# aim-uofa/DiverGen

Hardware: AMD Instinct MI355X
Metric: images/sec (node) Swin-L CenterNet2 LVIS 1024px (higher is better)
Workload: dtype bf16; 1 GPU; CenterNet2 Swin-L-22k-384, 1024x1024, 2 images/GPU, 1453 classes, GPU copy-paste + fwd + bwd + fused clip/AdamW/EMA; configs/DiverGen_swinL.yaml; global_batch=2, parallelism=dp1

## Files before the change

divergen_amd/_lib.py:

```python
import ctypes
import os

import torch

_HERE = os.path.dirname(os.path.abspath(__file__))
LIB_PATH = os.environ.get("DGX_LIB", os.path.join(_HERE, "csrc", "libdgx.so"))
_lib = None

c_p, c_i, c_f, c_i64 = ctypes.c_void_p, ctypes.c_int, ctypes.c_float, ctypes.c_int64


class WgradProblem(ctypes.Structure):
    _fields_ = [("dy", c_p), ("x", c_p), ("gw", c_p), ("M", c_i), ("Nn", c_i), ("Kk", c_i), ("gb", c_p)]


class GemmEpilogue(ctypes.Structure):
    _fields_ = [("mode", c_i), ("c", c_p), ("ldc", c_i64), ("bias", c_p), ("c2", c_p), ("aux", c_p), ("ldaux", c_i64),
                ("residual", c_p), ("out", c_p), ("scale", c_p), ("residual_dtype", c_i),
                ("B", c_i), ("H", c_i), ("W", c_i), ("ws", c_i), ("shift", c_i), ("workspace", c_p), ("workspace_bytes", c_i64), ("relu", c_i)]


class ProfStats(ctypes.Structure):
    _fields_ = [("ms", ctypes.c_double), ("launches", c_i64), ("flops", ctypes.c_double), ("bytes", ctypes.c_double),
                ("captured_launches", c_i64), ("captured_flops", ctypes.c_double), ("captured_bytes", ctypes.c_double)]


class PadItem(ctypes.Structure):
    _fields_ = [("x", c_p), ("xpad", c_p), ("N", c_i), ("H", c_i), ("W", c_i)]


class ConvItem(ctypes.Structure):
    _fields_ = [("xpad", c_p), ("y", c_p), ("N", c_i), ("H", c_i), ("W", c_i)]


class ConvWgradItem(ctypes.Structure):
    _fields_ = [("dypad", c_p), ("xpad", c_p), ("N", c_i), ("H", c_i), ("W", c_i)]


class HeadLevel(ctypes.Structure):
    _fields_ = [("x", c_p), ("dx", c_p), ("scale", c_p), ("rows", c_i)]


class GnItem(ctypes.Structure):
    _fields_ = [("x", c_p), ("dy", c_p), ("out", c_p), ("mean", c_p), ("rstd", c_p), ("scratch", c_p), ("N", c_i), ("HW", c_i)]


class ColsumProblem(ctypes.Structure):
    _fields_ = [("dy", c_p), ("out", c_p), ("M", c_i), ("N", c_i)]


SIGNATURES = {
    "dgx_build_arch": (ctypes.c_char_p, []),
    "dgx_abi_version": (c_i, []),
    "dgx_host_register": (c_i, [c_p, ctypes.c_size_t]),
    "dgx_host_unregister": (c_i, [c_p]),
    "dgx_memcpy_h2d_async": (c_i, [c_p, c_p, ctypes.c_size_t, c_p]),
    "dgx_window_attention_fwd": (c_i, [c_p, c_p, c_i64, c_i64, c_p, c_p, c_p, c_i, c_i, c_i, c_i, c_f, c_p]),
    "dgx_window_attention_bwd": (c_i, [c_p] * 8 + [c_i64, c_i64, c_i, c_i, c_i, c_i, c_f, c_p]),
    "dgx_window_attention_fwd_compact": (c_i, [c_p, c_p, c_p, c_i64, c_i64, c_p, c_p, c_p, c_i, c_i, c_i, c_i, c_i, c_i, c_f, c_p]),
    "dgx_window_attention_bwd_compact": (c_i, [c_p] * 9 + [c_i64, c_i64, c_i, c_i, c_i, c_i, c_i, c_i, c_f, c_p]),
    "dgx_window_gather": (c_i, [c_p, c_p, c_i, c_i, c_i, c_i, c_i, c_i, c_i, c_p]),
    "dgx_window_scatter": (c_i, [c_p, c_p, c_i, c_i, c_i, c_i, c_i, c_i, c_i, c_p]),
    "dgx_roi_align_fwd": (c_i, [c_p, c_p, c_p, c_i, c_i, c_i, c_i, c_i, c_f, c_i, c_i, c_i, c_i, c_i, c_i, c_p]),
    "dgx_roi_align_bwd": (c_i, [c_p, c_p, c_p, c_i, c_i, c_i, c_i, c_i, c_f, c_i, c_i, c_i, c_i, c_i, c_i, c_p]),
    "dgx_roi_pooler_fwd": (c_i, [c_p, c_p, c_p, c_i, c_i, c_p, c_p, c_p, c_i, c_i, c_i, c_i, c_i, c_i, c_i, c_i, c_p]),
    "dgx_roi_pooler_bwd": (c_i, [c_p, c_p, c_p, c_p, c_i, c_i, c_p, c_i, c_i, c_i, c_i, c_i, c_i, c_i, c_i, c_p]),
    "dgx_preprocess_patches": (c_i, [c_p, c_i, c_i, c_p, c_p, c_p, c_i, c_i, c_i, c_p]),
    "dgx_stem_im2col7x7": (c_i, [c_p, c_p, c_i, c_i, c_i, c_p]),
    "dgx_affine_act_fwd": (c_i, [c_p, c_p, c_p, c_p, c_p, c_i64, c_i, c_i, c_p]),
    "dgx_affine_act_bwd": (c_i, [c_p, c_p, c_p, c_p, c_p, c_i64, c_i, c_i, c_p]),
    "dgx_maxpool3x3s2_fwd": (c_i, [c_p, c_p, c_p, c_i, c_i, c_i, c_i, c_p]),
    "dgx_maxpool3x3s2_bwd": (c_i, [c_p, c_p, c_p, c_i, c_i, c_i, c_i, c_p]),
    "dgx_mask_bce_workspace_floats": (c_i64, [c_i64]),
    "dgx_mask_bce": (c_i, [c_p, c_i64, c_i64, c_p, c_i64, c_p, c_p, c_p, c_i, c_p]),
    "dgx_prof_enable": (c_i, [c_i]),
    "dgx_prof_pause": (c_i, [c_i]),
    "dgx_prof_read": (c_i, [c_i, c_p]),
    "dgx_roi_pooler_bwd_gather": (c_i, [c_p, c_p, c_p, c_p, c_i, c_i, c_f, c_i, c_p, c_i, c_i, c_i, c_i, c_i, c_i, c_i, c_p]),
    "dgx_roi_pooler_bwd_gather_accum": (c_i, [c_p, c_p, c_p, c_p, c_i, c_i, c_f, c_i, c_p, c_i, c_i, c_i, c_i, c_i, c_i, c_i, c_f, c_i, c_p]),
    "dgx_mask_crop": (c_i, [c_p, c_p, c_p, c_p, c_i, c_i, c_i, c_i, c_i, c_p]),
    "dgx_nms_sorted": (c_i, [c_p, c_i, c_f, c_p, c_p, c_p, c_p]),
    "dgx_nms_workspace_words": (c_i64, [c_i]),
    "dgx_nms_batched_workspace_words": (c_i64, [c_i, c_i]),
    "dgx_nms_batched": (c_i, [c_p, c_p, c_p, c_i, c_i, c_f, c_i, c_p, c_p, c_i, c_p, c_p]),
    "dgx_iou_match": (c_i, [c_p, c_i, c_p, c_i, c_f, c_p, c_p, c_p, c_p]),
    "dgx_centernet_targets": (c_i, [c_p, c_p, c_i, c_p, c_p, c_p, c_i, c_f, c_f, c_p, c_p, c_p]),
    "dgx_centernet_scores": (c_i, [c_p, c_i, c_i, c_p, c_p, c_i, c_i, c_f, c_p, c_p, c_i, c_p]),
    "dgx_centernet_decode": (c_i, [c_p, c_i, c_i, c_p, c_p, c_i, c_i, c_p, c_i, c_p, c_f, c_p, c_p, c_p, c_i, c_p]),
    "dgx_centernet_head_outputs": (c_i, [c_p, c_i, c_i, c_p, c_p, c_p]),
    "dgx_centernet_head_outputs_bwd_workspace_floats": (c_i64, [c_p, c_i, c_i]),
    "dgx_centernet_head_outputs_bwd": (c_i, [c_p, c_i, c_i, c_p, c_p, c_p, c_p, c_p]),
    "dgx_set_reserved_cus": (None, [c_i]),
    "dgx_get_reserved_cus": (c_i, []),
    "dgx_dev_set": (c_i, [ctypes.c_char_p, c_i]),
    "dgx_gemm_last_form": (c_i, [ctypes.POINTER(c_i)] * 3),
    "dgx_dev_gemm_log": (c_i, [ctypes.c_char_p]),
    "dgx_gather_boxes": (c_i, [c_p, c_p, c_i, c_i, c_p, c_p]),
    "dgx_topk_index_rows": (c_i, [c_p, c_i64, c_i, c_p, c_p, c_p, c_i, c_i, c_p, c_i64, c_p]),
    "dgx_sort_rows_desc": (c_i, [c_p, c_i, c_i, c_p, c_p, c_p]),
    "dgx_centernet_finalize": (c_i, [c_p, c_p, c_p, c_p, c_i, c_i, c_i, c_p, c_p, c_p, c_p]),
    "dgx_roi_label": (c_i, [c_p, c_p, c_i, c_i, c_p, c_p, c_p, c_i, c_f, c_i, c_i, c_i, c_p, c_p, c_p, c_p, c_p, c_p]),
    "dgx_roi_gather": (c_i, [c_i, c_i, c_i, c_p, c_p, c_p, c_p, c_p, c_p, c_p, c_p, c_p, c_f] + [c_p] * 10 + [c_p]),
    "dgx_centernet_label_inds": (c_i, [c_p, c_p, c_i, c_i, c_p, c_p, c_p, c_i, c_p, c_p, c_p]),
    "dgx_copy_paste": (c_i, [c_p, c_p, c_p, c_i, c_i, c_i, c_p, c_p, c_i, c_p, c_p, c_p, c_p, c_p]),
    "dgx_copy_paste_blend": (c_i, [c_p, c_p, c_p, c_i, c_i, c_i, c_p, c_p, c_i, c_p, c_p, c_p, c_p, c_p, c_p]),
    "dgx_copy_paste_blend_ws": (c_i, [c_p, c_p, c_p, c_i, c_i, c_i, c_p, c_p, c_i, c_p, c_p, c_p, c_p, c_p, c_p, ctypes.c_size_t, c_p]),
    "dgx_poisson_blend": (c_i, [c_p, c_p, c_p, c_i, c_i, c_p, ctypes.c_size_t, c_i, c_p]),
    "dgx_poisson_work_bytes": (c_i64, [c_i, c_i, c_i64]),
    "dgx_poisson_frame_unknowns": (c_i64, [c_i, c_i]),
    "dgx_poisson_max_iter": (c_i, [c_i, c_i, c_i64]),
    "dgx_self_copy_paste": (c_i, [c_p, c_p, c_p, c_i, c_i, c_i, c_p, c_p, c_i, c_i, c_i, c_p, c_i, c_i, c_i, c_p, c_p, c_p, c_p, c_p, c_p]),
    "dgx_self_copy_paste_merged": (c_i, [c_p, c_p, c_p, c_i, c_i, c_i, c_p, c_p, c_i, c_i, c_i, c_p, c_i, c_i, c_i, c_p, c_p, c_p, c_p, c_p, c_p]),
    "dgx_self_copy_paste_all": (c_i, [c_p, c_p, c_p, c_i, c_i, c_i, c_p, c_p, c_i, c_i, c_i, c_i, c_i, c_p, c_p, c_p, c_p, c_p, c_p]),
# ... 146 lines not shown
```

divergen_amd/csrc/abi.hip:

```cpp
#include "dgx_common.h"
extern "C" const char* dgx_build_arch(void) { return "gfx950"; }
extern "C" int dgx_abi_version(void) { return 3; }

extern "C" int dgx_host_register(void* p, size_t bytes) {
    if (!p || !bytes) return DGX_ERR_BAD_ARG;
    const hipError_t e = hipHostRegister(p, bytes, hipHostRegisterDefault);
    return e == hipSuccess ? DGX_OK : -(int)e - 1000;
}
extern "C" int dgx_host_unregister(void* p) {
    if (!p) return DGX_ERR_BAD_ARG;
    const hipError_t e = hipHostUnregister(p);
    return e == hipSuccess ? DGX_OK : -(int)e - 1000;
}
extern "C" int dgx_memcpy_h2d_async(void* dst, const void* src, size_t bytes, void* stream) {
    if (!bytes) return DGX_OK;
    if (!dst || !src) return DGX_ERR_BAD_ARG;
    const hipError_t e = hipMemcpyAsync(dst, src, bytes, hipMemcpyHostToDevice, (hipStream_t)stream);
    return e == hipSuccess ? DGX_OK : -(int)e - 1000;
}
```

divergen_amd/csrc/gemm_common.h:

```cpp
#pragma once
#include "dgx_common.h"
#include "gemm_plan.h"
#include "winmap.h"
#include <type_traits>

constexpr int GBK = 64;
static constexpr uint32_t G_OOB = 0x80000000u;

namespace dgxgemm {
struct GMap { int B, H, W, ws, shift, nWh, nWw, compact; };

struct GemmP {
    const uint16_t* A;
    const uint16_t* B;
    int M, N, K, lda, ldb;
    int tiles_n, total, per_xcd;
    int splits, kt_per_split;
    float* ws;
    int mode;
    uint16_t* C;
    int ldc;
    const uint16_t* bias;
    uint16_t* C2;
    const uint16_t* aux;
    int ldaux;
    const void* res;
    void* out;
    const float* scale;
    int res_dtype;
    GMap map;
    int conv_kc, conv_wp;
    int cmap_n, cmap_h, cmap_w;
    int relu;
    int ngrp;
    struct Grp { const uint16_t* A; uint16_t* C; int M, cn, ch, cw, wp, tile0; } grp[6];
};
constexpr int GEMM_MAXG = 6;
}
using dgxgemm::GMap;
using dgxgemm::GemmP;

namespace {

__device__ __forceinline__ void g_load_lds16(uint32_t voff, u32x4 rsrc, uint32_t lds_addr, uint32_t soff) {
    asm volatile("s_mov_b32 m0, %2\n\ts_nop 0\n\tbuffer_load_dwordx4 %0, %1, %3 offen lds" ::"v"(voff), "s"(rsrc), "s"(lds_addr), "s"(soff)
                 : "memory");
}
__device__ __forceinline__ u32x4 g_rsrc(const void* base, uint32_t bytes) {
    const uint64_t a = (uint64_t)base;
    return u32x4{(uint32_t)a, (uint32_t)(a >> 32) & 0xffffu, bytes, 0x00020000u};
}
template <int N> __device__ __forceinline__ void g_vmcnt() { asm volatile("s_waitcnt vmcnt(%0)" ::"n"(N) : "memory"); }
__device__ __forceinline__ void g_lgkm0() { asm volatile("s_waitcnt lgkmcnt(0)" ::: "memory"); }
__device__ __forceinline__ void g_bar() {
    asm volatile("s_barrier" ::: "memory");
    __builtin_amdgcn_sched_barrier(0);
}

template <int MC> __device__ __forceinline__ void g_fix_mode(GemmP& P) {
    if constexpr (MC == 6) { P.mode = 3; P.res_dtype = DGX_F32; }
    else if constexpr (MC == 3) { P.mode = 3; P.res_dtype = DGX_BF16; }
    else if constexpr (MC >= 0) P.mode = MC;
}
template <class F> int g_with_mc(int mc, F&& f) {
    switch (mc) {
        case 1: return f(std::integral_constant<int, 1>{});
        case 2: return f(std::integral_constant<int, 2>{});
        case 3: return f(std::integral_constant<int, 3>{});
        case 4: return f(std::integral_constant<int, 4>{});
        case 5: return f(std::integral_constant<int, 5>{});
        case 6: return f(std::integral_constant<int, 6>{});
        default: return f(std::integral_constant<int, 0>{});
    }
}
inline int g_tail_mc(const GemmP& P) { return dgxplan::tail_mc(P.mode, P.res_dtype == DGX_BF16); }

__device__ __forceinline__ dgxgemm::GemmP::Grp g_group_of_tile(const GemmP& P, int L) {
    dgxgemm::GemmP::Grp q = P.grp[0];
#pragma unroll
    for (int k = 1; k < dgxgemm::GEMM_MAXG; ++k)
        if (k < P.ngrp && L >= P.grp[k].tile0) q = P.grp[k];
    return q;
}
__device__ __forceinline__ void g_enter_group(GemmP& P, const dgxgemm::GemmP::Grp& q) {
    P.A = q.A; P.C = q.C; P.M = q.M;
    P.cmap_n = q.cn; P.cmap_h = q.ch; P.cmap_w = q.cw; P.conv_wp = q.wp;
}
__device__ __forceinline__ uint32_t g_a_voff(const GemmP& P, int m, int lc) {
    int64_t arow = m;
    if (P.conv_kc) {
        const int hw = P.cmap_h * P.cmap_w;
        const int n = m / hw, r = m - n * hw;
        const int y = r / P.cmap_w, x = r - y * P.cmap_w;
        arow = ((int64_t)n * (P.cmap_h + 2) + y + 1) * P.conv_wp + x + 1;
    }
    return m < P.M ? (uint32_t)((arow * P.lda + lc * 8) * 2) : G_OOB;
}
__device__ __forceinline__ uint32_t g_a_soff(const GemmP& P, int kta) {
    uint32_t s = (uint32_t)kta * (GBK * 2);
    if (P.conv_kc) {
        const int tap = kta / P.conv_kc, kc = kta - tap * P.conv_kc;
        s = (uint32_t)((tap / 3) * P.conv_wp + tap % 3) * (uint32_t)(P.lda * 2) + (uint32_t)kc * (GBK * 2);
    }
    return s;
}
__device__ __forceinline__ void g_bias4(const u32x2 raw, float (&bv)[4]) {
    bv[0] = __uint_as_float(raw[0] << 16); bv[1] = __uint_as_float(raw[0] & 0xffff0000u);
    bv[2] = __uint_as_float(raw[1] << 16); bv[3] = __uint_as_float(raw[1] & 0xffff0000u);
}

constexpr float kGInvSqrt2 = 0.70710678118654752440f;
constexpr float kGInvSqrt2Pi = 0.39894228040143267794f;
__device__ __forceinline__ void g_unpack8(const u32x4 r, float (&v)[8]) {
#pragma unroll
    for (int i = 0; i < 4; ++i) { v[2 * i] = __uint_as_float(r[i] << 16); v[2 * i + 1] = __uint_as_float(r[i] & 0xffff0000u); }
}
__device__ __forceinline__ u32x4 g_pack8(const float (&v)[8]) {
    return u32x4{pack_bf2(v[0], v[1]), pack_bf2(v[2], v[3]), pack_bf2(v[4], v[5]), pack_bf2(v[6], v[7])};
}

__device__ __forceinline__ int64_t g_row_token(const GMap& m, int64_t orow, int& b) {
    if (m.ws == 0) {
        b = (int)(orow / ((int64_t)m.H * m.W));
        return orow;
    }
    if (m.compact) return wm_token_of_row(wm_geom(m.H, m.W, m.ws, m.shift), (int)orow, b);
    const int Nw = m.ws * m.ws;
    const int n = (int)(orow % Nw);
    int64_t t = orow / Nw;
    const int wc = (int)(t % m.nWw);
    t /= m.nWw;
    const int wr = (int)(t % m.nWh);
    b = (int)(t / m.nWh);
    int hh = wr * m.ws + n / m.ws + m.shift, ww = wc * m.ws + n % m.ws + m.shift;
    const int Hp = m.nWh * m.ws, Wp = m.nWw * m.ws;
    if (hh >= Hp) hh -= Hp;
    if (ww >= Wp) ww -= Wp;
    return (hh < m.H && ww < m.W) ? ((int64_t)b * m.H + hh) * m.W + ww : -1;
}
// ... 139 lines not shown
```

divergen_amd/csrc/gemm_lw.hip:

```cpp
#include "gemm_common.h"
#include "dev_clock.h"
#include <stdio.h>
#include <stdlib.h>
#include <string.h>

namespace {
constexpr int LW_LDS = 160 * 1024;
template <int BM, int BN, int NSA_, int NSB_> struct LwCfg {
    static constexpr int NSA = NSA_, NSB = NSB_;
    static_assert(NSA >= NSB && NSA - NSB <= 1 && NSB >= 2, "ring depths: NSA == NSB or NSB + 1");
    static constexpr int WMF = BM / 32;
    static constexpr int WNF = BN / 64;
    static constexpr int NLA = BM / 32;
    static constexpr int NLB = BN / 32;
    static constexpr int SA = BM * 128;
    static constexpr int SBb = BN * 128;
    static constexpr int B0 = (NSA - 1) * SA;
    static constexpr int STG0 = B0 + NSB * SBb;
    static constexpr int RING = STG0 + SA;
    static_assert(RING <= LW_LDS, "rings do not fit");
    static constexpr int SROW = BN * 2 + 16;
    static constexpr int TOK0 = LW_LDS - BM * 8;
    static constexpr int STGB = TOK0 - STG0;
    static constexpr int HALF = BM / 2;
    static constexpr int pick_hc() {
        for (int hc = HALF; hc >= 16; hc -= 16)
            if (HALF % hc == 0 && 2 * hc * SROW <= STGB) return hc;
        return 0;
    }
    static constexpr int HC = pick_hc();
    static_assert(HC >= 16, "staging area too small");
    static constexpr int CH = 2 * HC;
    static constexpr int NPASS = HALF / HC;
    static constexpr int FPP = HC / 16;
};
constexpr int LW_THREADS = 768, LW_MFMA_THREADS = 512;

__device__ __forceinline__ void lw_lgkm0() { __builtin_amdgcn_s_waitcnt(0xc07f); }
__device__ __forceinline__ uint32_t lw_sgpr(uint32_t v) { return (uint32_t)__builtin_amdgcn_readfirstlane((int)v); }
template <int PRO, int STEADY, int STEP>
__device__ __forceinline__ void lw_vmcnt_le(int n) {
    if (PRO > STEADY && n >= PRO) g_vmcnt<PRO>();
    else if (STEADY > 0 && n >= STEADY) g_vmcnt<STEADY>();
    else if (STEP > 0 && STEP < STEADY && n >= STEP) g_vmcnt<STEP>();
    else g_vmcnt<0>();
}
struct LwItem { int m0, n0, kt0, NT, split; };
}

template <int BM, int BN, int NSA, int NSB, int MC>
__global__ __launch_bounds__(LW_THREADS) void gemm_lw_kernel(GemmP P0) {
    constexpr int EC = MC == 6 ? 2 : (MC == 3 || MC == 4 || MC == 5) ? 1 : 0;
    if constexpr (MC == 0) { if (P0.mode > 1) __builtin_unreachable(); }
    else g_fix_mode<MC>(P0);
    using Cfg = LwCfg<BM, BN, NSA, NSB>;
    constexpr int WMF = Cfg::WMF, WNF = Cfg::WNF, NLA = Cfg::NLA, NLB = Cfg::NLB, SA = Cfg::SA, SBb = Cfg::SBb, B0 = Cfg::B0;
    constexpr int SROW = Cfg::SROW, STG0 = Cfg::STG0, CH = Cfg::CH, HC = Cfg::HC, NPASS = Cfg::NPASS, FPP = Cfg::FPP, HALF = Cfg::HALF;
    extern __shared__ __attribute__((aligned(1024))) unsigned char lds_raw[];
    const int nwx = (int)(gridDim.x >> 3);
    const int xcd = blockIdx.x & 7;
    const int items = P0.total * P0.splits;
    const int bound = min((xcd + 1) * P0.per_xcd, items);
    const int first = xcd * P0.per_xcd + (int)(blockIdx.x >> 3);
    if (first >= bound) return;
    const int tid = threadIdx.x, l = tid & 63;
    const int w = __builtin_amdgcn_readfirstlane(tid >> 6);
    const int grp = (w >> 2) & 1, wc = w & 3;
    const int c = l & 15, g = l >> 4;
    const int NTK = (P0.K + GBK - 1) / GBK;
    const int ktail = P0.K - (NTK - 1) * GBK;
    const uint32_t lds0 = (uint32_t)(uintptr_t)(DGX_LDS unsigned char*)lds_raw;

    auto locate_item = [&](int L0, GemmP& P, LwItem& it) {
        int L = L0 / P0.splits;
        it.split = L0 - L * P0.splits;
        if (P0.ngrp > 0) {
            L = __builtin_amdgcn_readfirstlane(L);
            const dgxgemm::GemmP::Grp q = g_group_of_tile(P0, L);
            g_enter_group(P, q);
            L -= q.tile0;
        }
        const int tm = L / P0.tiles_n, tn = L - tm * P0.tiles_n;
        it.m0 = tm * BM;
        it.n0 = tn * BN;
        it.kt0 = it.split * P0.kt_per_split;
        it.NT = min(P0.kt_per_split, NTK - it.kt0);
    };
    auto a_slot = [](int s) -> uint32_t { return s == NSA - 1 ? (uint32_t)STG0 : (uint32_t)s * SA; };

    if (w >= 8) {
        const int lw = w - 8;
        const int rsub = l >> 3;
        const int lc = (l & 7) ^ (((lw & 1) << 2) | (rsub >> 1));
        const bool kt_ok = lc * 8 < ktail;
        const uint32_t ldsq = lw_sgpr(lds0 + 1024u * lw);
        GemmP P = P0;
        LwItem it;
        uint32_t voffA[NLA], voffB[NLB];
        u32x4 rA;
        const u32x4 rB = g_rsrc(P0.B, (uint32_t)((int64_t)P0.N * P0.ldb * 2));
        auto setup = [&](int L0) {
            locate_item(L0, P, it);
#pragma unroll
            for (int s = 0; s < NLA; ++s) voffA[s] = g_a_voff(P, it.m0 + 8 * (lw + 4 * s) + rsub, lc);
#pragma unroll
            for (int s = 0; s < NLB; ++s) {
                const int n = it.n0 + 8 * (lw + 4 * s) + rsub;
                voffB[s] = n < P.N ? (uint32_t)(((int64_t)n * P.ldb + lc * 8) * 2) : G_OOB;
            }
            const u32x4 r = g_rsrc(P.A, (uint32_t)((P.conv_kc ? (int64_t)P.cmap_n * (P.cmap_h + 2) * P.conv_wp + 2 * P.conv_wp + 2 : (int64_t)P.M) * P.lda * 2));
            rA = u32x4{lw_sgpr(r[0]), lw_sgpr(r[1]), lw_sgpr(r[2]), lw_sgpr(r[3])};
        };
        auto issue_a = [&](int t) {
            if (t >= it.NT) return;
            const int kta = it.kt0 + t;
            const uint32_t soffA = g_a_soff(P, kta);
            const bool tail = (kta == NTK - 1) && (ktail != GBK) && !kt_ok;
            const uint32_t dst = ldsq + a_slot(t % NSA);
#pragma unroll
            for (int s = 0; s < NLA; ++s) g_load_lds16(tail ? G_OOB : voffA[s], rA, lw_sgpr(dst + 4096u * s), lw_sgpr(soffA));
        };
        auto issue_b = [&](int t) {
            if (t >= it.NT) return;
            const int kta = it.kt0 + t;
            const uint32_t soff = (uint32_t)kta * (GBK * 2);
            const bool tail = (kta == NTK - 1) && (ktail != GBK) && !kt_ok;
            const uint32_t dst = ldsq + B0 + (uint32_t)(t % NSB) * SBb;
#pragma unroll
            for (int s = 0; s < NLB; ++s) g_load_lds16(tail ? G_OOB : voffB[s], rB, lw_sgpr(dst + 4096u * s), lw_sgpr(soff));
        };
        constexpr int STEADY = (NSA > NSB ? NSB - 1 : NSA - 2) * NLA + (NSB - 2) * NLB;
        constexpr int PRO = (NSA - 1) * NLA + (NSB - 1) * NLB;
        static_assert(PRO < 64, "vmcnt is a 6-bit counter");
        auto wait_tile = [&](int tau, int ia, int ib) {
            const int la = min(ia, it.NT - 1), lb = min(ib, it.NT - 1);
            const int ca = max(0, la - (tau + 1) + 1), cb = max(0, lb - (tau + 1) + 1);
            lw_vmcnt_le<PRO, STEADY, NLA>(ca * NLA + cb * NLB);
        };
        auto prologue_1 = [&]() {
// ... 290 lines not shown
```

divergen_amd/csrc/gemm_nt.hip:

```cpp
#include "gemm_common.h"
#include "dev_clock.h"
#include <stdio.h>
#include <string.h>

namespace {
template <int BM, int BN, int NS_> struct GemmCfg {
    static constexpr int NS = NS_;
    static constexpr int WMF = BM / 32;
    static constexpr int WNF = BN / 64;
    static constexpr int NA = BM / 64;
    static constexpr int NB = BN / 64;
    static constexpr int SB = (BM + BN) * 128;
    static constexpr int SROW = BN * 2 + 16;
    static constexpr int EPI = BM * SROW + BM * 8;
    static constexpr int LDS = (NS * SB > EPI ? NS * SB : EPI);
};
}

template <int BM, int BN, int NS, int MINW, int MC = -1>
__global__ __launch_bounds__(512, MINW) void gemm_nt_kernel(GemmP P) {
    g_fix_mode<MC>(P);
    using Cfg = GemmCfg<BM, BN, NS>;
    constexpr int NL = Cfg::NA + Cfg::NB;
    constexpr int WMF = Cfg::WMF, WNF = Cfg::WNF, NA = Cfg::NA, NB = Cfg::NB, SB = Cfg::SB, SROW = Cfg::SROW;
    extern __shared__ __attribute__((aligned(1024))) unsigned char lds_raw[];
    const int L0 = (blockIdx.x & 7) * P.per_xcd + (blockIdx.x >> 3);
    if (L0 >= P.total * P.splits) return;
    int L = L0 / P.splits;
    const int split = L0 - L * P.splits;
    if (P.ngrp > 0) {
        L = __builtin_amdgcn_readfirstlane(L);
        dgxgemm::GemmP::Grp q = P.grp[0];
#pragma unroll
        for (int k = 1; k < dgxgemm::GEMM_MAXG; ++k)
            if (k < P.ngrp && L >= P.grp[k].tile0) q = P.grp[k];
        P.A = q.A; P.C = q.C; P.M = q.M;
        P.cmap_n = q.cn; P.cmap_h = q.ch; P.cmap_w = q.cw; P.conv_wp = q.wp;
        L -= q.tile0;
    }
    DGX_CLK(0);
    DGX_CLK_RT(5);
    const int tm = L / P.tiles_n, tn = L - tm * P.tiles_n;
    const int m0 = tm * BM, n0 = tn * BN;
    const int tid = threadIdx.x, l = tid & 63;
    const int w = __builtin_amdgcn_readfirstlane(tid >> 6);
    const int grp = w >> 2, wc = w & 3;
    const int c = l & 15, g = l >> 4;
    const int NTK = (P.K + GBK - 1) / GBK;
    const int ktail = P.K - (NTK - 1) * GBK;
    const int kt0 = split * P.kt_per_split;
    const int NT = min(P.kt_per_split, NTK - kt0);

    const int rsub = l >> 3;
    const int lc = (l & 7) ^ (((w & 1) << 2) | (rsub >> 1));
    uint32_t voffA[NA], voffB[NB];
#pragma unroll
    for (int s = 0; s < NA; ++s) voffA[s] = g_a_voff(P, m0 + 8 * (w + 8 * s) + rsub, lc);
#pragma unroll
    for (int s = 0; s < NB; ++s) {
        const int n = n0 + 8 * (w + 8 * s) + rsub;
        voffB[s] = n < P.N ? (uint32_t)(((int64_t)n * P.ldb + lc * 8) * 2) : G_OOB;
    }
    const bool kt_ok = lc * 8 < ktail;
    const u32x4 rA = g_rsrc(P.A, (uint32_t)((P.conv_kc ? (int64_t)P.cmap_n * (P.cmap_h + 2) * P.conv_wp + 2 * P.conv_wp + 2 : (int64_t)P.M) * P.lda * 2));
    const u32x4 rB = g_rsrc(P.B, (uint32_t)((int64_t)P.N * P.ldb * 2));
    const uint32_t lds0 = (uint32_t)(uintptr_t)(DGX_LDS unsigned char*)lds_raw;
    const uint32_t ldsw = __builtin_amdgcn_readfirstlane(lds0 + 1024u * w);
    auto issue_one = [&](int k, int t, int stage) {
        const int kta = kt0 + t;
        const uint32_t soff = (uint32_t)kta * (GBK * 2), soffA = g_a_soff(P, kta);
        const uint32_t dst = ldsw + (uint32_t)stage * SB;
        const bool tail = (kta == NTK - 1) && (ktail != GBK) && !kt_ok;
        if (k < NA) g_load_lds16(tail ? G_OOB : voffA[k], rA, dst + 8192u * k, soffA);
        else g_load_lds16(tail ? G_OOB : voffB[k - NA], rB, dst + BM * 128 + 8192u * (k - NA), soff);
    };

    const int swz = (c >> 1) & 7;
    const uint32_t la = (uint32_t)((grp * (BM / 2) + c) * 128 + ((g ^ swz) << 4));
    const uint32_t lb = (uint32_t)((BM + wc * (BN / 4) + c) * 128 + ((g ^ swz) << 4));
    f32x4 acc[WMF][WNF];
#pragma unroll
    for (int i = 0; i < WMF; ++i)
#pragma unroll
        for (int j = 0; j < WNF; ++j) acc[i][j] = f32x4{0.f, 0.f, 0.f, 0.f};
    bf16x8 af[WMF][2], bfr[WNF][2];
    auto load_phase = [&](int stage, int ti, int istage) {
        if (ti >= 0) {
#pragma unroll
            for (int k = 0; k < NL; ++k) issue_one(k, ti, istage);
        }
        DGX_LDS const unsigned char* sa = lds_opaque((const unsigned char*)lds_raw + stage * SB + la);
        DGX_LDS const unsigned char* sa1 = lds_opaque((const unsigned char*)lds_raw + stage * SB + (la ^ 64u));
        DGX_LDS const unsigned char* sb = lds_opaque((const unsigned char*)lds_raw + stage * SB + lb);
        DGX_LDS const unsigned char* sb1 = lds_opaque((const unsigned char*)lds_raw + stage * SB + (lb ^ 64u));
#pragma unroll
        for (int j = 0; j < WNF; ++j) {
            bfr[j][0] = *reinterpret_cast<DGX_LDS const bf16x8*>(sb + 2048 * j);
            bfr[j][1] = *reinterpret_cast<DGX_LDS const bf16x8*>(sb1 + 2048 * j);
        }
#pragma unroll
        for (int i = 0; i < WMF; ++i) {
            af[i][0] = *reinterpret_cast<DGX_LDS const bf16x8*>(sa + 2048 * i);
            af[i][1] = *reinterpret_cast<DGX_LDS const bf16x8*>(sa1 + 2048 * i);
        }
// ... 247 lines not shown
    if (bm == 192 && bn == 192 && ns == 3) return nt_launch_e<192, 192, 3, 2, -1>(P, st);
    if (bm == 128 && bn == 192 && ns == 4) return nt_launch_e<128, 192, 4, 2, -1>(P, st);
    if (bm == 192 && bn == 256 && ns == 2) return nt_launch_e<192, 256, 2, 2, -1>(P, st);
    if (bm == 128 && bn == 256 && ns == 3) return nt_launch_e<128, 256, 3, 2, -1>(P, st);
    if (bm == 256 && bn == 128 && ns == 3) return nt_launch_e<256, 128, 3, 2, -1>(P, st);
    if (bm == 128 && bn == 128 && ns == 4) return nt_launch_e<128, 128, 4, 2, -1>(P, st);
    return DGX_ERR_UNSUPPORTED;
}
}

int gemm_lw_launch(GemmP& P, int bm, int bn, hipStream_t st);
bool dgx_gemm_k192_takes(const GemmP& P);
int dgx_gemm_k192_launch(const GemmP& P, hipStream_t st);

static GemmPlan plan_and_log(const GemmP& P, int64_t ws_bytes) {
    dgxplan::GemmProblem q;
    q.M = P.M; q.N = P.N; q.K = P.K;
    q.mode = P.mode; q.res_bf16 = P.res_dtype == DGX_BF16;
    q.conv = P.conv_kc != 0; q.relu = P.relu != 0;
    q.ngrp = P.ngrp;
    int rows = P.ngrp ? 0 : P.M;
    for (int i = 0; i < P.ngrp; ++i) { q.Ms[i] = P.grp[i].M; rows += P.grp[i].M; }
    q.ws_bytes = P.ws ? ws_bytes : 0;
    q.k192_operands = dgx_gemm_k192_takes(P);
    const GemmPlan pl = dgxplan::plan_gemm(q, g_dev, dgx_get_reserved_cus() / 8);
    if (g_gemm_log) { fprintf(g_gemm_log, "%d %d %d %d %d %d\n", rows, P.N, P.K, P.conv_kc ? 9 : P.mode, pl.bm, pl.bn); fflush(g_gemm_log); }
    return pl;
}
static int launch(GemmP& P, const GemmPlan& pl, hipStream_t st) {
    P.tiles_n = pl.tiles_n; P.total = pl.total; P.per_xcd = pl.per_xcd;
    P.splits = pl.splits; P.kt_per_split = pl.kt_per_split;
    for (int i = 0; i < P.ngrp; ++i) P.grp[i].tile0 = pl.tile0[i];
    const bool k192 = pl.form == dgxplan::FORM_K192;
    const int rc = k192 ? dgx_gemm_k192_launch(P, st) : pl.form == dgxplan::FORM_LW ? gemm_lw_launch(P, pl.bm, pl.bn, st) : gemm_nt_launch(P, pl, st);
    if (rc != DGX_OK) return rc;
    if (k192) g_last = {pl.form, 32, 192, 1};
    else g_last = {pl.form, pl.bm, pl.bn, pl.splits};
    if (!k192 && pl.splits > 1) {
        const int64_t chunks = (int64_t)P.M * (P.N >> 3);
        const int grid = (int)((chunks + 255) / 256 < 4096 ? (chunks + 255) / 256 : 4096);
        hipLaunchKernelGGL(gemm_splitk_fold_kernel, dim3(grid), dim3(256), 0, st, P);
    }
    DGX_LAUNCH_CHECK();
    return DGX_OK;
}

DGX_CLK_READER(dgx_dev_gemm_nt_clocks)
extern "C" int dgx_dev_gemm_log(const char* path) {
    if (g_gemm_log) { fclose(g_gemm_log); g_gemm_log = nullptr; }
    if (path && *path && !(g_gemm_log = fopen(path, "w"))) return DGX_ERR_BAD_ARG;
    return DGX_OK;
}
extern int g_dgx_dev_wgrad_lw;
extern "C" int dgx_dev_set(const char* key, int value) {
    if (!key) return DGX_ERR_BAD_ARG;
    if (!strcmp(key, "gemm_lw")) g_dev.lw = value;
    else if (!strcmp(key, "gemm_2wg")) g_dev.two_wg = value;
    else if (!strcmp(key, "gemm_tile")) { g_dev.tile_bm = value / 1000; g_dev.tile_bn = value % 1000; }
    else if (!strcmp(key, "gemm_splitk")) g_dev.splitk = value;
    else if (!strcmp(key, "gemm_k192")) g_dev.k192 = value;
    else if (!strcmp(key, "wgrad_lw")) g_dgx_dev_wgrad_lw = value;
    else if (!strcmp(key, "reset")) { g_dev = dgxplan::DevKnobs(); g_dgx_dev_wgrad_lw = 1; }
    else return DGX_ERR_BAD_ARG;
    return DGX_OK;
}
extern "C" int dgx_gemm_last_form(int* bm, int* bn, int* splits) {
    if (bm) *bm = g_last.bm;
    if (bn) *bn = g_last.bn;
    if (splits) *splits = g_last.splits;
    return g_last.form;
}

extern "C" int dgx_gemm_bf16_nt(const void* A, const void* B, int M, int N, int K, int64_t lda, int64_t ldb,
                                const dgx_gemm_epilogue* ep, void* stream) {
    if (M <= 0 || N <= 0) return DGX_OK;
    if (!A || !B || !ep || K <= 0 || (K & 7) || (N & 7) || (lda & 7) || (ldb & 7) || lda < K || ldb < K) return DGX_ERR_BAD_ARG;
    if ((int64_t)M * lda * 2 >= (1ll << 31) || (int64_t)N * ldb * 2 >= (1ll << 31)) return DGX_ERR_UNSUPPORTED;
    GemmP P;
    memset((void*)&P, 0, sizeof(P));
    P.A = (const uint16_t*)A; P.B = (const uint16_t*)B;
    P.M = M; P.N = N; P.K = K; P.lda = (int)lda; P.ldb = (int)ldb;
    P.mode = ep->mode;
    P.C = (uint16_t*)ep->c; P.ldc = (int)ep->ldc;
    P.bias = (const uint16_t*)ep->bias;
    P.C2 = (uint16_t*)ep->c2;
    P.aux = (const uint16_t*)ep->aux; P.ldaux = (int)ep->ldaux;
    P.res = ep->residual; P.out = ep->out; P.scale = ep->scale; P.res_dtype = ep->residual_dtype;
    P.ws = (float*)ep->workspace;
    P.relu = (ep->mode <= DGX_EPI_BIAS) ? ep->relu : 0;
    switch (ep->mode) {
        case DGX_EPI_NONE: case DGX_EPI_BIAS:
            if (!ep->c || ep->ldc < N || (ep->ldc & 7)) return DGX_ERR_BAD_ARG;
            if (ep->mode == DGX_EPI_NONE) P.bias = nullptr;
            break;
        case DGX_EPI_BIAS_GELU:
            if (!ep->c || !ep->c2 || ep->ldc < N || (ep->ldc & 7)) return DGX_ERR_BAD_ARG;
            break;
        case DGX_EPI_GELU_GRAD: case DGX_EPI_RELU_GRAD:
            if (!ep->c || !ep->aux || ep->ldc < N || ep->ldaux < N || (ep->ldc & 7) || (ep->ldaux & 7)) return DGX_ERR_BAD_ARG;
            P.bias = nullptr;
            break;
        case DGX_EPI_BIAS_RESIDUAL: {
            const int aws = ep->ws < 0 ? -ep->ws : ep->ws;
            if (!ep->residual || !ep->out || ep->B <= 0 || ep->H <= 0 || ep->W <= 0 || ep->B > 4095 || ep->shift < 0 ||
                (aws > 0 && ep->shift >= aws) || (ep->residual_dtype != DGX_F32 && ep->residual_dtype != DGX_BF16) ||
                (ep->ws < 0 && !wm_compact_ok(ep->H, ep->W, aws, ep->shift)))
                return DGX_ERR_BAD_ARG;
            GMap m = {ep->B, ep->H, ep->W, aws, ep->shift, 0, 0, ep->ws < 0 ? 1 : 0};
            if (aws > 0) { m.nWh = (ep->H + aws - 1) / aws; m.nWw = (ep->W + aws - 1) / aws; }
            const int64_t rows = ep->ws > 0 ? (int64_t)ep->B * m.nWh * m.nWw * aws * aws : (int64_t)ep->B * ep->H * ep->W;
            if (rows != M) return DGX_ERR_BAD_ARG;
            P.map = m;
            break;
        }
        default: return DGX_ERR_BAD_ARG;
    }
    const double mn = (double)M * N, rsz = ep->residual_dtype == DGX_F32 ? 4.0 : 2.0;
    const double obytes = ep->mode == DGX_EPI_BIAS_RESIDUAL ? 2.0 * rsz * mn : (ep->mode >= DGX_EPI_BIAS_GELU ? 4.0 * mn : 2.0 * mn);
    DgxProfScope prof(DGX_PROF_GEMM_NT, stream, 2.0 * mn * K, 2.0 * ((double)M * K + (double)N * K) + obytes);
    return launch(P, plan_and_log(P, ep->workspace_bytes), (hipStream_t)stream);
}

extern "C" int64_t dgx_conv3x3_pad_rows(int N, int H, int W) {
    return (N <= 0 || H <= 0 || W <= 0) ? 0 : (int64_t)N * (H + 2) * (W + 2) + 2 * (int64_t)(W + 3);
}

extern "C" int dgx_conv3x3_gemm_multi(const dgx_conv_item* items, int n, const void* w, const void* bias, int Cin, int Cout, int relu,
                                      void* stream) {
    if (n <= 0) return DGX_OK;
    if (!items || !w || Cin <= 0 || Cout <= 0 || (Cin & 63) || (Cout & 7)) return DGX_ERR_BAD_ARG;
    if (n > dgxgemm::GEMM_MAXG || Cout > 256 || (int64_t)Cout * 9 * Cin * 2 >= (1ll << 31)) return DGX_ERR_UNSUPPORTED;
    GemmP P;
    memset((void*)&P, 0, sizeof(P));
    P.B = (const uint16_t*)w;
    P.N = Cout; P.K = 9 * Cin; P.lda = Cin; P.ldb = 9 * Cin;
    P.mode = bias ? DGX_EPI_BIAS : DGX_EPI_NONE;
    P.ldc = Cout;
    P.bias = (const uint16_t*)bias;
    P.conv_kc = Cin / GBK;
    P.relu = relu;
    P.ngrp = n;
    double fl = 0.0, by = 2.0 * 9.0 * Cin * Cout;
// ... 59 lines not shown
```

divergen_amd/csrc/wgrad256.hip:

```cpp
#include "dgx_common.h"
#include <type_traits>

namespace {
constexpr int T256 = 256;
constexpr int BM256 = 32;
constexpr int NB256 = 4;
constexpr int OPB256 = BM256 * T256 * 2;
constexpr int STB256 = 2 * OPB256;
constexpr int MAXP256 = 12;

struct Prob256 {
    const uint16_t* A;
    const uint16_t* B;
    float* C;
    float* gb;
    float* wsb;
    float* ws;
    int M, Nn, Kk, tiles_k, tiles, S, slab, wg0;
    int ldc;
    int64_t red0;
};
struct Params256 {
    Prob256 p[MAXP256];
    int n, total, per_xcd;
    int interleave;
    float beta;
    int nimg;
    struct Img { const uint16_t* dy; const uint16_t* x; int wp, M, slab0; } img[6];
};

__device__ __forceinline__ void buffer_load_lds16(uint32_t voff, u32x4 rsrc, uint32_t lds_wave_base, uint32_t soff) {
    asm volatile("s_mov_b32 m0, %2\n\ts_nop 0\n\tbuffer_load_dwordx4 %0, %1, %3 offen lds" ::"v"(voff), "s"(rsrc), "s"(lds_wave_base), "s"(soff)
                 : "memory");
}
__device__ __forceinline__ u32x4 make_rsrc(const void* base, uint32_t bytes) {
    const uint64_t a = (uint64_t)base;
    return u32x4{(uint32_t)a, (uint32_t)(a >> 32) & 0xffffu, bytes, 0x00020000u};
}
__device__ __forceinline__ void mfma16_agpr(f32x4& c, bf16x8 a, bf16x8 b) {
    asm("v_mfma_f32_16x16x32_bf16 %0, %1, %2, %0" : "+a"(c) : "v"(a), "v"(b));
}
__device__ __forceinline__ void mfma16_vgpr(f32x4& c, bf16x8 a, bf16x8 b) {
    asm("v_mfma_f32_16x16x32_bf16 %0, %1, %2, %0" : "+v"(c) : "v"(a), "v"(b));
}
template <int N> __device__ __forceinline__ void wait_vmcnt() { asm volatile("s_waitcnt vmcnt(%0)" ::"n"(N) : "memory"); }
}

__global__ __launch_bounds__(256) void wgrad256_partial_kernel(Params256 P) {
    extern __shared__ __attribute__((aligned(1024))) unsigned char lds_raw[];
    const int L = (blockIdx.x & 7) * P.per_xcd + (blockIdx.x >> 3);
    if (L >= P.total) return;
    int pi = 0;
    if (P.interleave) {
        pi = L % P.n;
    } else {
#pragma unroll
        for (int i = 1; i < MAXP256; ++i)
            if (i < P.n && L >= P.p[i].wg0) pi = i;
    }
    Prob256 q = P.p[pi];
    const int local = P.interleave ? L / P.n : L - q.wg0;
    const int s = local / q.tiles, tile = local - s * q.tiles;
    int s_in = s;
    if (P.nimg > 0) {
        const int su = __builtin_amdgcn_readfirstlane(s), tap = __builtin_amdgcn_readfirstlane(pi);
        Params256::Img im = P.img[0];
#pragma unroll
        for (int k = 1; k < 6; ++k)
            if (k < P.nimg && su >= P.img[k].slab0) im = P.img[k];
        q.A = im.dy + (int64_t)(im.wp + 1) * q.Nn;
        q.B = im.x + (int64_t)((tap / 3) * im.wp + tap % 3) * q.Kk;
        q.M = im.M;
        s_in = su - im.slab0;
    }
    const int n0 = (tile / q.tiles_k) * T256, k0 = (tile % q.tiles_k) * T256;
    const int m_begin = s_in * q.slab, m_end = min(q.M, m_begin + q.slab);
    const int nst = (m_end - m_begin + BM256 - 1) / BM256;
    const int tid = threadIdx.x, w = tid >> 6, l = tid & 63, g = l >> 4, c16 = l & 15;
    const int wn = (w >> 1) * 128, wk = (w & 1) * 128;

    const int rip = l >> 5;
    const int lc = (l & 31) ^ (((2 * (w & 1) + rip) & 3) << 1);
    const uint32_t OOB = 0x80000000u;
    const uint32_t vA = (n0 + 8 * lc < q.Nn) ? (uint32_t)(((2 * w + rip) * q.Nn + n0 + 8 * lc) * 2) : OOB;
    const uint32_t vB = (k0 + 8 * lc < q.Kk) ? (uint32_t)(((2 * w + rip) * q.Kk + k0 + 8 * lc) * 2) : OOB;
    const u32x4 rA = make_rsrc(q.A, (uint32_t)((int64_t)m_end * q.Nn * 2));
    const u32x4 rB = make_rsrc(q.B, (uint32_t)((int64_t)m_end * q.Kk * 2));
    const uint32_t lds0 = (uint32_t)(uintptr_t)(DGX_LDS unsigned char*)lds_raw;
    const uint32_t ldsw = __builtin_amdgcn_readfirstlane(lds0 + 1024u * w);
    auto issue1 = [&](int st, int h) {
        const uint32_t row0 = (uint32_t)(m_begin + st * BM256);
        const uint32_t dst = ldsw + (uint32_t)(st & (NB256 - 1)) * STB256;
        const int j = h & 3;
        if (h < 4) buffer_load_lds16(vA, rA, dst + 4096u * j, (row0 + 8 * j) * (uint32_t)(q.Nn * 2));
        else buffer_load_lds16(vB, rB, dst + OPB256 + 4096u * j, (row0 + 8 * j) * (uint32_t)(q.Kk * 2));
    };
    auto issue = [&](int st) {
#pragma unroll
        for (int h = 0; h < 8; ++h) issue1(st, h);
    };

    const int x = c16 >> 2, hi = (c16 >> 1) & 1, lo = c16 & 1;
    DGX_LDS const uint16_t* pfa[2][4];
    DGX_LDS const uint16_t* pfb[2][4];
#pragma unroll
    for (int b = 0; b < 4; ++b) {
        const uint32_t o = (uint32_t)((8 * g + x) * 512 + 32 * (b ^ x) + 16 * hi + 8 * lo);
#pragma unroll
        for (int h2 = 0; h2 < 2; ++h2) {
            pfa[h2][b] = lds_opaque(reinterpret_cast<const uint16_t*>(lds_raw + o + wn * 2 + h2 * 2 * STB256));
            pfb[h2][b] = lds_opaque(reinterpret_cast<const uint16_t*>(lds_raw + OPB256 + o + wk * 2 + h2 * 2 * STB256));
        }
    }

    f32x4 acc[8][8];
#pragma unroll
    for (int i = 0; i < 8; ++i)
#pragma unroll
        for (int j = 0; j < 8; ++j) acc[i][j] = f32x4{0.f, 0.f, 0.f, 0.f};
    const bool do_bias = q.gb != nullptr && (tile % q.tiles_k) == 0;
    f32x4 bacc[4];
#pragma unroll
    for (int i = 0; i < 4; ++i) bacc[i] = f32x4{0.f, 0.f, 0.f, 0.f};
    bf16x8 ones = {(short)0x3F80, (short)0x3F80, (short)0x3F80, (short)0x3F80, (short)0x3F80, (short)0x3F80, (short)0x3F80, (short)0x3F80};
    asm volatile("" : "+v"(ones));
    auto bias_mfmas = [&](const bf16x8 (&af)[8]) {
        if (do_bias) {
            if (w & 1) {
#pragma unroll
// ... 166 lines not shown
    int tiles[MAXP256], maxM = 0;
    for (int i = 0; i < n; ++i) {
        tiles[i] = ((pr[i].Nn + T256 - 1) / T256) * ((pr[i].Kk + T256 - 1) / T256);
        if (pr[i].M > maxM) maxM = pr[i].M;
    }
    int R = BM256;
    for (;; R += BM256) {
        int64_t wgs = 0;
        for (int i = 0; i < n; ++i) wgs += (int64_t)tiles[i] * ((pr[i].M + R - 1) / R);
        if (wgs <= 256 || R >= maxM) break;
    }
    for (int i = 0; i < n; ++i) {
        S[i] = (pr[i].M + R - 1) / R;
        if (S[i] < 1) S[i] = 1;
        int sl = (pr[i].M + S[i] - 1) / S[i];
        slab[i] = (sl + BM256 - 1) / BM256 * BM256;
    }
}

static int64_t ws_floats256(const dgx_wgrad_problem* pr, int n, const int* S, int64_t* off, int64_t* offb = nullptr) {
    int64_t tot = 0;
    for (int i = 0; i < n; ++i) {
        if (off) off[i] = tot;
        if (S[i] > 1) tot += (int64_t)S[i] * pr[i].Nn * pr[i].Kk;
    }
    for (int i = 0; i < n; ++i) {
        if (offb) offb[i] = tot;
        if (S[i] > 1 && pr[i].gb) tot += ((int64_t)S[i] * pr[i].Nn + 3) / 4 * 4;
    }
    return tot;
}

bool wgrad_lw_wants(const dgx_wgrad_problem* pr, int n);
int wgrad_lw_launch(const dgx_wgrad_problem* pr, int n, float beta, hipStream_t st);
constexpr int MAXP_GROUP = 32;

extern "C" int dgx_wgrad_grouped_form(const dgx_wgrad_problem* problems, int n) {
    return problems && n > 0 && n <= MAXP_GROUP && wgrad_lw_wants(problems, n) ? 1 : 0;
}

static int64_t split_workspace_bytes(const dgx_wgrad_problem* problems, int n) {
    if (!problems || n <= 0 || n > MAXP256) return 0;
    int S[MAXP256], slab[MAXP256];
    plan256(problems, n, S, slab);
    return ws_floats256(problems, n, S, nullptr) * 4;
}
extern "C" int64_t dgx_wgrad_grouped_workspace_bytes(const dgx_wgrad_problem* problems, int n) {
    if (!problems || n <= 0 || n > MAXP_GROUP) return 0;
    if (wgrad_lw_wants(problems, n) && n > MAXP256) return 0;
    return split_workspace_bytes(problems, n);
}

static int wgrad_grouped_impl(const dgx_wgrad_problem* problems, const int* ldc, int n, float beta, void* workspace, void* stream);

extern "C" int dgx_linear_wgrad_grouped(const dgx_wgrad_problem* problems, int n, float beta, void* workspace,
                                        void* stream) {
    double fl = 0.0, by = 0.0;
    if (!problems || n <= 0 || n > MAXP_GROUP) return DGX_ERR_BAD_ARG;
    for (int i = 0; i < n; ++i) {
        fl += 2.0 * problems[i].M * problems[i].Nn * problems[i].Kk;
        by += 2.0 * problems[i].M * ((double)problems[i].Nn + problems[i].Kk) + 8.0 * problems[i].Nn * problems[i].Kk;
    }
    DgxProfScope prof(DGX_PROF_WGRAD, stream, fl, by);
    if (wgrad_lw_wants(problems, n)) {
        const int rc = wgrad_lw_launch(problems, n, beta, (hipStream_t)stream);
        if (rc == DGX_OK) { DGX_LAUNCH_CHECK(); return DGX_OK; }
        if (rc != DGX_ERR_UNSUPPORTED || n > MAXP256) return rc;
    }
    return wgrad_grouped_impl(problems, nullptr, n, beta, workspace, stream);
}

extern "C" int64_t dgx_conv3x3_wgrad_workspace_bytes(int N, int H, int W, int Cin, int Cout) {
    dgx_wgrad_problem pr[9];
    const int64_t Mp = (int64_t)N * (H + 2) * (W + 2);
    for (int t = 0; t < 9; ++t) { pr[t].dy = pr[t].x = nullptr; pr[t].gw = nullptr; pr[t].gb = nullptr; pr[t].M = (int)Mp; pr[t].Nn = Cout; pr[t].Kk = Cin; }
    return split_workspace_bytes(pr, 9);
}
extern "C" int dgx_conv3x3_wgrad_bias(const void* dypad, const void* xpad, float* gw, float* gb, int N, int H, int W, int Cin, int Cout,
                                      float beta, void* workspace, void* stream);
extern "C" int dgx_conv3x3_wgrad(const void* dypad, const void* xpad, float* gw, int N, int H, int W, int Cin, int Cout, float beta,
                                 void* workspace, void* stream) {
    return dgx_conv3x3_wgrad_bias(dypad, xpad, gw, nullptr, N, H, W, Cin, Cout, beta, workspace, stream);
}
extern "C" int64_t dgx_conv3x3_wgrad_bias_workspace_bytes(int N, int H, int W, int Cin, int Cout) {
    dgx_wgrad_problem pr[9];
    const int64_t Mp = (int64_t)N * (H + 2) * (W + 2);
    float dummy;
    for (int t = 0; t < 9; ++t) { pr[t].dy = pr[t].x = nullptr; pr[t].gw = nullptr; pr[t].gb = t == 0 ? &dummy : nullptr; pr[t].M = (int)Mp; pr[t].Nn = Cout; pr[t].Kk = Cin; }
    return split_workspace_bytes(pr, 9);
}
extern "C" int dgx_conv3x3_wgrad_bias(const void* dypad, const void* xpad, float* gw, float* gb, int N, int H, int W, int Cin, int Cout,
                                      float beta, void* workspace, void* stream) {
    if (N <= 0 || H <= 0 || W <= 0) return DGX_OK;
    if (!dypad || !xpad || !gw || (Cin & 7) || (Cout & 7)) return DGX_ERR_BAD_ARG;
    const int64_t Mp = (int64_t)N * (H + 2) * (W + 2);
    const int wp = W + 2;
    dgx_wgrad_problem pr[9];
    int ldc[9];
    for (int t = 0; t < 9; ++t) {
        pr[t].dy = (const uint16_t*)dypad + (int64_t)(wp + 1) * Cout;
        pr[t].x = (const uint16_t*)xpad + (int64_t)((t / 3) * wp + t % 3) * Cin;
        pr[t].gw = gw + (int64_t)t * Cin;
        pr[t].gb = t == 0 ? gb : nullptr;
        pr[t].M = (int)Mp; pr[t].Nn = Cout; pr[t].Kk = Cin;
        ldc[t] = 9 * Cin;
    }
    DgxProfScope prof(DGX_PROF_WGRAD, stream, 2.0 * N * H * W * 9.0 * Cin * Cout, 2.0 * Mp * ((double)Cin + Cout) + 8.0 * 9.0 * Cin * Cout);
    return wgrad_grouped_impl(pr, ldc, 9, beta, workspace, stream);
}

static int wgrad_grouped_impl(const dgx_wgrad_problem* problems, const int* ldc, int n, float beta, void* workspace, void* stream) {
    if (n <= 0) return DGX_OK;
    if (!problems || n > MAXP256) return DGX_ERR_BAD_ARG;
    for (int i = 0; i < n; ++i) {
        const dgx_wgrad_problem& p = problems[i];
        if (!p.dy || !p.x || !p.gw || p.M <= 0 || p.Nn <= 0 || p.Kk <= 0 || (p.Nn & 7) || (p.Kk & 7)) return DGX_ERR_BAD_ARG;
        if ((int64_t)p.M * p.Nn * 2 >= (1ll << 31) || (int64_t)p.M * p.Kk * 2 >= (1ll << 31)) return DGX_ERR_UNSUPPORTED;
    }
    int S[MAXP256], slab[MAXP256];
    int64_t off[MAXP256], offb[MAXP256];
    plan256(problems, n, S, slab);
    if (ws_floats256(problems, n, S, off, offb) > 0 && !workspace) return DGX_ERR_BAD_ARG;
    Params256 P;
    P.n = n;
    P.beta = beta;
    P.nimg = 0;
    int wg = 0;
    int64_t red = 0;
    for (int i = 0; i < n; ++i) {
        const dgx_wgrad_problem& p = problems[i];
        Prob256& q = P.p[i];
        q.A = (const uint16_t*)p.dy;
        q.B = (const uint16_t*)p.x;
        q.C = p.gw;
        q.gb = p.gb;
        q.wsb = (float*)workspace + offb[i];
        q.ws = (float*)workspace + off[i];
        q.M = p.M; q.Nn = p.Nn; q.Kk = p.Kk;
        q.ldc = ldc ? ldc[i] : p.Kk;
        q.tiles_k = (p.Kk + T256 - 1) / T256;
        q.S = S[i];
        q.slab = slab[i];
        q.tiles = ((p.Nn + T256 - 1) / T256) * q.tiles_k;
        q.wg0 = wg;
        q.red0 = red;
        wg += q.tiles * S[i];
        if (S[i] > 1) red += (int64_t)p.Nn * p.Kk / 4;
    }
    for (int i = n; i < MAXP256; ++i) P.p[i] = P.p[0];
    hipStream_t st = (hipStream_t)stream;
    const size_t sm = (size_t)NB256 * STB256;
    static bool once = false;
    if (!once) {
        (void)hipFuncSetAttribute((const void*)wgrad256_partial_kernel, hipFuncAttributeMaxDynamicSharedMemorySize, (int)sm);
        once = true;
    }
    P.total = wg;
    P.interleave = 0;
    if (ldc && n > 1) {
        P.interleave = 1;
        for (int i = 1; i < n; ++i)
            if (P.p[i].tiles != P.p[0].tiles || P.p[i].S != P.p[0].S || P.p[i].M != P.p[0].M) P.interleave = 0;
    }
    P.per_xcd = (wg + 7) / 8;
    hipLaunchKernelGGL(wgrad256_partial_kernel, dim3(8 * P.per_xcd), dim3(256), sm, st, P);
    int bias_cb = 1, bias_blocks = 0;
    {
        int maxNn = 0;
        for (int i = 0; i < n; ++i)
            if (S[i] > 1 && problems[i].gb) maxNn = problems[i].Nn > maxNn ? problems[i].Nn : maxNn;
        if (maxNn > 0) { bias_cb = (maxNn + 255) / 256; bias_blocks = bias_cb * n; }
    }
    if (red > 0 || bias_blocks > 0) {
        int maxS = 1;
        for (int i = 0; i < n; ++i) maxS = S[i] > maxS ? S[i] : maxS;
        if (red > 0 && red <= 32768 && maxS >= 16) {
            hipLaunchKernelGGL(wgrad256_reduce_kernel<16>, dim3((int)((red * 16 + 255) / 256) + bias_blocks), dim3(256), 0, st, P, red,
                               bias_blocks, bias_cb);
        } else {
            const int grid = (int)((red + 255) / 256 < 8192 ? (red + 255) / 256 : 8192);
            hipLaunchKernelGGL(wgrad256_reduce_kernel<1>, dim3(grid + bias_blocks), dim3(256), 0, st, P, red, bias_blocks, bias_cb);
        }
    }
    DGX_LAUNCH_CHECK();
    return DGX_OK;
}

static int conv_multi_plan(const dgx_conv_wgrad_item* items, int n, int tiles, int* R_out, int* nsl, int* M) {
    int maxM = 0;
    for (int i = 0; i < n; ++i) {
        M[i] = items[i].N * (items[i].H + 2) * (items[i].W + 2);
// ... 12 lines not shown
}

extern "C" int64_t dgx_conv3x3_wgrad_bias_multi_workspace_bytes(const dgx_conv_wgrad_item* items, int n, int Cin, int Cout) {
    if (!items || n <= 0 || n > 6) return 0;
    if (n == 1) return dgx_conv3x3_wgrad_bias_workspace_bytes(items[0].N, items[0].H, items[0].W, Cin, Cout);
    int R, nsl[6], M[6];
    const int tiles = ((Cout + T256 - 1) / T256) * ((Cin + T256 - 1) / T256);
    const int S = conv_multi_plan(items, n, tiles, &R, nsl, M);
    return ((int64_t)9 * S * Cout * Cin + ((int64_t)S * Cout + 3) / 4 * 4) * 4;
}

extern "C" int dgx_conv3x3_wgrad_bias_multi(const dgx_conv_wgrad_item* items, int n, float* gw, float* gb, int Cin, int Cout, float beta,
                                            void* workspace, void* stream) {
    if (n <= 0) return DGX_OK;
    if (!items || !gw || !workspace || (Cin & 7) || (Cout & 7) || Cin <= 0 || Cout <= 0) return DGX_ERR_BAD_ARG;
    if (n > 6) return DGX_ERR_UNSUPPORTED;
    if (n == 1)
        return dgx_conv3x3_wgrad_bias(items[0].dypad, items[0].xpad, gw, gb, items[0].N, items[0].H, items[0].W, Cin, Cout, beta, workspace,
                                      stream);
    int R, nsl[6], M[6];
    const int tiles_k = (Cin + T256 - 1) / T256, tiles = ((Cout + T256 - 1) / T256) * tiles_k;
    for (int i = 0; i < n; ++i) {
        if (!items[i].dypad || !items[i].xpad || items[i].N <= 0 || items[i].H <= 0 || items[i].W <= 0) return DGX_ERR_BAD_ARG;
        const int64_t rows = (int64_t)items[i].N * (items[i].H + 2) * (items[i].W + 2) + 2 * (int64_t)(items[i].W + 3);
        if (rows * Cout * 2 >= (1ll << 31) || rows * Cin * 2 >= (1ll << 31)) return DGX_ERR_UNSUPPORTED;
    }
    const int S = conv_multi_plan(items, n, tiles, &R, nsl, M);
    Params256 P;
    P.n = 9;
    P.beta = beta;
    P.nimg = n;
    int s0 = 0;
    double fl = 0.0, by = 8.0 * 9.0 * Cin * Cout;
    for (int i = 0; i < n; ++i) {
        P.img[i].dy = (const uint16_t*)items[i].dypad; P.img[i].x = (const uint16_t*)items[i].xpad;
        P.img[i].wp = items[i].W + 2; P.img[i].M = M[i]; P.img[i].slab0 = s0;
        s0 += nsl[i];
        fl += 2.0 * items[i].N * items[i].H * items[i].W * 9.0 * Cin * Cout;
        by += 2.0 * M[i] * ((double)Cin + Cout);
    }
    for (int i = n; i < 6; ++i) P.img[i] = P.img[0];
    float* ws = (float*)workspace;
    const int64_t per = (int64_t)S * Cout * Cin;
    int wg = 0;
    int64_t red = 0;
    for (int t = 0; t < 9; ++t) {
        Prob256& q = P.p[t];
        q.A = P.img[0].dy; q.B = P.img[0].x;
        q.C = gw + (int64_t)t * Cin;
        q.gb = t == 0 ? gb : nullptr;
        q.wsb = ws + 9 * per;
        q.ws = ws + (int64_t)t * per;
        q.M = M[0]; q.Nn = Cout; q.Kk = Cin;
        q.ldc = 9 * Cin;
        q.tiles_k = tiles_k;
        q.S = S;
        q.slab = R;
        q.tiles = tiles;
        q.wg0 = wg;
        q.red0 = red;
        wg += tiles * S;
        red += (int64_t)Cout * Cin / 4;
    }
    for (int i = 9; i < MAXP256; ++i) P.p[i] = P.p[0];
    hipStream_t st = (hipStream_t)stream;
    const size_t sm = (size_t)NB256 * STB256;
    static bool once = false;
    if (!once) {
        (void)hipFuncSetAttribute((const void*)wgrad256_partial_kernel, hipFuncAttributeMaxDynamicSharedMemorySize, (int)sm);
        once = true;
    }
    P.total = wg;
    P.interleave = 1;
    P.per_xcd = (wg + 7) / 8;
    DgxProfScope prof(DGX_PROF_WGRAD, stream, fl, by);
    hipLaunchKernelGGL(wgrad256_partial_kernel, dim3(8 * P.per_xcd), dim3(256), sm, st, P);
    const int bias_cb = (Cout + 255) / 256, bias_blocks = gb ? bias_cb * 9 : 0;
    if (red <= 32768 && S >= 16) {
        hipLaunchKernelGGL(wgrad256_reduce_kernel<16>, dim3((int)((red * 16 + 255) / 256) + bias_blocks), dim3(256), 0, st, P, red, bias_blocks,
                           bias_cb);
    } else {
        const int grid = (int)((red + 255) / 256 < 8192 ? (red + 255) / 256 : 8192);
        hipLaunchKernelGGL(wgrad256_reduce_kernel<1>, dim3(grid + bias_blocks), dim3(256), 0, st, P, red, bias_blocks, bias_cb);
    }
    DGX_LAUNCH_CHECK();
    return DGX_OK;
}
```

divergen_amd/csrc/wgrad_lw.hip:

```cpp
#include "dgx_common.h"
#include <stdlib.h>
#include <string.h>
#include <type_traits>

namespace {
constexpr int WL_TN = 256, WL_TK = 192;
constexpr int WL_BM = 64;
constexpr int WL_GR = 32;
constexpr int WL_GB = WL_GR * 512;
constexpr int WL_NGA = 6, WL_NGB = 4;
constexpr int WL_B0 = WL_NGA * WL_GB;
constexpr int WL_LDS = (WL_NGA + WL_NGB) * WL_GB;
constexpr int WL_MAXP = 32;
constexpr int WL_THREADS = 768;

struct WlProb {
    const uint16_t* A;
    const uint16_t* B;
    float* C;
    float* gb;
    int M, Nn, Kk, ldc, tiles_k, item0;
};
struct WlParams {
    WlProb p[WL_MAXP];
    int item0[WL_MAXP];
    int n, total, per_xcd;
    float beta;
};

__device__ __forceinline__ void wl_load_lds16(uint32_t voff, u32x4 rsrc, uint32_t lds_addr, uint32_t soff) {
    asm volatile("s_mov_b32 m0, %2\n\ts_nop 0\n\tbuffer_load_dwordx4 %0, %1, %3 offen lds" ::"v"(voff), "s"(rsrc), "s"(lds_addr), "s"(soff)
                 : "memory");
}
__device__ __forceinline__ u32x4 wl_rsrc(const void* base, uint32_t bytes) {
    const uint64_t a = (uint64_t)base;
    return u32x4{(uint32_t)__builtin_amdgcn_readfirstlane((int)(uint32_t)a), (uint32_t)__builtin_amdgcn_readfirstlane((int)((uint32_t)(a >> 32) & 0xffffu)),
                 (uint32_t)__builtin_amdgcn_readfirstlane((int)bytes), 0x00020000u};
}
template <int N> __device__ __forceinline__ void wl_vmcnt() { asm volatile("s_waitcnt vmcnt(%0)" ::"n"(N) : "memory"); }
__device__ __forceinline__ void wl_bar() {
    asm volatile("s_barrier" ::: "memory");
    __builtin_amdgcn_sched_barrier(0);
}
__device__ __forceinline__ void wl_lgkm0() { __builtin_amdgcn_s_waitcnt(0xc07f); }
__device__ __forceinline__ uint32_t wl_sgpr(uint32_t v) { return (uint32_t)__builtin_amdgcn_readfirstlane((int)v); }
template <int N> using wl_ic = std::integral_constant<int, N>;
template <int N, int I = 0, typename F> __device__ __forceinline__ void wl_static_for(F&& f) {
    if constexpr (I < N) { f(wl_ic<I>{}); wl_static_for<N, I + 1>(f); }
}
}

__global__ __launch_bounds__(WL_THREADS) void wgrad_lw_kernel(WlParams P) {
    extern __shared__ __attribute__((aligned(1024))) unsigned char lds_raw[];
    const int nwx = (int)(gridDim.x >> 3);
    const int xcd = blockIdx.x & 7;
    const int bound = min((xcd + 1) * P.per_xcd, P.total);
    const int first = xcd * P.per_xcd + (int)(blockIdx.x >> 3);
    if (first >= bound) return;
    const int tid = threadIdx.x, l = tid & 63;
    const int w = __builtin_amdgcn_readfirstlane(tid >> 6);
    const uint32_t lds0 = (uint32_t)(uintptr_t)(DGX_LDS unsigned char*)lds_raw;

    typedef const __attribute__((address_space(4))) WlProb* TabPtr;
    const TabPtr tab = (TabPtr)__builtin_amdgcn_kernarg_segment_ptr();
    auto locate = [&](int L, WlProb& q, int& n0, int& k0) {
        L = __builtin_amdgcn_readfirstlane(L);
        int idx = 0;
#pragma unroll
        for (int i = 1; i < WL_MAXP; ++i)
            if (L >= P.item0[i]) idx = i;
        q.A = tab[idx].A; q.B = tab[idx].B; q.C = tab[idx].C; q.gb = tab[idx].gb;
        q.M = tab[idx].M; q.Nn = tab[idx].Nn; q.Kk = tab[idx].Kk; q.ldc = tab[idx].ldc; q.tiles_k = tab[idx].tiles_k; q.item0 = tab[idx].item0;
        const int t = L - q.item0;
        const int tn = t / q.tiles_k;
        n0 = tn * WL_TN;
        k0 = ((t - tn * q.tiles_k + tn + (tn >> 3)) % q.tiles_k) * WL_TK;
    };
    if (w >= 8) {
        const int lw = w - 8;
        const int rip = l >> 5;
        const int lc0 = (l & 31) ^ (((2 * (lw & 1) + rip) & 3) << 1), lc1 = lc0 ^ 8;
        const uint32_t ldsq = wl_sgpr(lds0 + 1024u * lw);
        const uint32_t OOB = 0x80000000u;
        WlProb q;
        int n0, k0, NH = 0;
        uint32_t va[4], vb[4];
        uint32_t stepA = 0, stepB = 0, sa = 0, sb = 0;
        u32x4 rA, rB;
        auto setup = [&](int L) {
            locate(L, q, n0, k0);
            NH = 2 * ((q.M + WL_BM - 1) / WL_BM);
#pragma unroll
            for (int s = 0; s < 4; ++s) {
                const int lc = (s & 1) ? lc1 : lc0, row = 8 * s + 2 * lw + rip;
                va[s] = (n0 + 8 * lc < q.Nn) ? (uint32_t)((row * q.Nn + n0 + 8 * lc) * 2) : OOB;
                vb[s] = (8 * lc < WL_TK && k0 + 8 * lc < q.Kk) ? (uint32_t)((row * q.Kk + k0 + 8 * lc) * 2) : OOB;
            }
            stepA = (uint32_t)(WL_GR * q.Nn * 2); stepB = (uint32_t)(WL_GR * q.Kk * 2);
            sa = 0; sb = 0;
            rA = wl_rsrc(q.A, (uint32_t)((int64_t)q.M * q.Nn * 2));
            rB = wl_rsrc(q.B, (uint32_t)((int64_t)q.M * q.Kk * 2));
        };
        auto issue_a1 = [&](int s) { wl_load_lds16(va[s], rA, wl_sgpr(ldsq + sa + 4096u * s), 0u); va[s] += stepA; };
        auto issue_b1 = [&](int s) { wl_load_lds16(vb[s], rB, wl_sgpr(ldsq + WL_B0 + sb + 4096u * s), 0u); vb[s] += stepB; };
        auto next_a = [&]() { sa = sa + WL_GB == WL_NGA * WL_GB ? 0u : sa + WL_GB; };
        auto next_b = [&]() { sb = (sb + WL_GB) & (WL_NGB * WL_GB - 1); };
        auto issue_a = [&]() {
#pragma unroll
            for (int s = 0; s < 4; ++s) issue_a1(s);
            next_a();
        };
        auto issue_b = [&]() {
#pragma unroll
            for (int s = 0; s < 4; ++s) issue_b1(s);
            next_b();
        };
        const int g = l >> 4, c16 = l & 15, x = c16 >> 2;
        DGX_LDS const uint16_t* pf[4];
#pragma unroll
        for (int f = 0; f < 4; ++f)
            pf[f] = lds_opaque(reinterpret_cast<const uint16_t*>(lds_raw + (8 * g + x) * 512 + 16 * ((c16 >> 1) & 1) + 8 * (c16 & 1) + 32 * ((4 * lw + f) ^ x ^ ((g & 1) << 2))));
        const bf16x8 ones = {(short)0x3F80, (short)0x3F80, (short)0x3F80, (short)0x3F80, (short)0x3F80, (short)0x3F80, (short)0x3F80, (short)0x3F80};
        f32x4 bacc[4];
        bf16x8 bfrag[4];
#pragma unroll
        for (int f = 0; f < 4; ++f) bacc[f] = f32x4{0.f, 0.f, 0.f, 0.f};
        uint32_t sbias = 0;
        auto bias_read = [&]() {
#pragma unroll
            for (int f = 0; f < 4; ++f) {
                DGX_LDS const uint16_t* p = pf[f] + sbias;
                asm volatile("" : "+v"(p));
                bfrag[f] = tr_frag(p, 0, 4 * 256);
            }
            sbias = sbias + WL_GB / 2 == WL_NGA * WL_GB / 2 ? 0u : sbias + WL_GB / 2;
        };
        auto bias_fold = [&](int f) { bacc[f] = mfma16(ones, bfrag[f], bacc[f]); };
        setup(first);
        for (int L = first; L < bound; L += nwx) {
            const bool do_bias = q.gb != nullptr && k0 == 0;
            issue_a(); issue_b(); issue_a(); issue_b(); issue_a(); issue_b(); issue_a(); issue_b(); issue_a();
            wl_vmcnt<28>();
            wl_bar();
            sbias = 0;
            if (do_bias) bias_read();
            for (int h = 0; h < NH; ++h) {
                if (h < 3) wl_vmcnt<20>(); else wl_vmcnt<16>();
                wl_bar();
                if (do_bias) {
#pragma unroll
                    for (int s = 0; s < 4; ++s) { issue_a1(s); bias_fold(s); }
                    issue_b();
                    next_a();
                    bias_read();
                } else {
                    issue_a();
                    issue_b();
                }
            }
            wl_bar();
            if (do_bias) {
#pragma unroll
                for (int f = 0; f < 4; ++f) {
                    const int n = n0 + 64 * lw + 16 * f + c16;
                    if (g == 0 && n < q.Nn) q.gb[n] = P.beta != 0.f ? P.beta * q.gb[n] + bacc[f][0] : bacc[f][0];
                    bacc[f] = f32x4{0.f, 0.f, 0.f, 0.f};
                }
            }
            if (L + nwx < bound) setup(L + nwx);
        }
        return;
    }

    const int grp = (w >> 2) & 1, wc = w & 3;
    const int g = l >> 4, c16 = l & 15;
    const int x = c16 >> 2, hi = (c16 >> 1) & 1, lo = c16 & 1;
    const uint32_t rowb = (uint32_t)((8 * g + x) * 512 + 16 * hi + 8 * lo);
    const int gb = g & 1;
    DGX_LDS const uint16_t* pa[2][4];
    DGX_LDS const uint16_t* pb[3];
#pragma unroll
    for (int b = 0; b < 4; ++b) {
        const uint32_t o = rowb + 32u * (uint32_t)(b ^ x) + 128u * (uint32_t)(grp ^ gb);
        pa[0][b] = lds_opaque(reinterpret_cast<const uint16_t*>(lds_raw + o));
        pa[1][b] = lds_opaque(reinterpret_cast<const uint16_t*>(lds_raw + o + 4 * WL_GB));
    }
#pragma unroll
    for (int j = 0; j < 3; ++j) pb[j] = lds_opaque(reinterpret_cast<const uint16_t*>(lds_raw + WL_B0 + rowb + 32u * (uint32_t)((3 * wc + j) ^ x ^ (gb << 2))));
    for (int L = first; L < bound; L += nwx) {
        WlProb q;
        int n0, k0;
        locate(L, q, n0, k0);
        const int NH = 2 * ((q.M + WL_BM - 1) / WL_BM);
        f32x4 acc[8][3];
#pragma unroll
        for (int i = 0; i < 8; ++i)
#pragma unroll
            for (int j = 0; j < 3; ++j) acc[i][j] = f32x4{0.f, 0.f, 0.f, 0.f};
        bf16x8 b0[3], b1[3], afr[4];
        constexpr int PRE = 3;
        auto fragA = [&](auto S, auto I) -> bf16x8 {
            constexpr int s_ = decltype(S)::value, i_ = decltype(I)::value;
            constexpr int off = (s_ & 3) * (WL_GB / 2) + 128 * (i_ >> 2);
            return tr_frag(pa[s_ >> 2][i_ & 3], off, off + 4 * 256);
        };
        auto fragB = [&](auto S, auto J) -> bf16x8 {
            constexpr int off = decltype(S)::value * (WL_GB / 2);
            return tr_frag(pb[decltype(J)::value], off, off + 4 * 256);
        };
        auto half = [&](auto U, const bf16x8 (&bc)[3], bf16x8 (&bn)[3]) {
            constexpr int u = decltype(U)::value, sa = u % WL_NGA, sa1 = (u + 1) % WL_NGA, sb1 = (u + 1) % WL_NGB;
            wl_bar();
            __builtin_amdgcn_s_setprio(1);
            wl_static_for<8>([&](auto I) {
                constexpr int i = decltype(I)::value, ip = i + PRE;
                if constexpr (ip < 8) afr[ip & 3] = fragA(wl_ic<sa>{}, wl_ic<ip>{});
                else afr[ip & 3] = fragA(wl_ic<sa1>{}, wl_ic<ip - 8>{});
                if constexpr (i < 3) bn[i] = fragB(wl_ic<sb1>{}, wl_ic<i>{});
#pragma unroll
                for (int j = 0; j < 3; ++j) acc[i][j] = mfma16(bc[j], afr[i & 3], acc[i][j]);
            });
            __builtin_amdgcn_sched_group_barrier(0x100, 4, 0); __builtin_amdgcn_sched_group_barrier(0x008, 3, 0);
            __builtin_amdgcn_sched_group_barrier(0x100, 4, 0); __builtin_amdgcn_sched_group_barrier(0x008, 3, 0);
            __builtin_amdgcn_sched_group_barrier(0x100, 4, 0); __builtin_amdgcn_sched_group_barrier(0x008, 3, 0);
            __builtin_amdgcn_sched_group_barrier(0x100, 2, 0); __builtin_amdgcn_sched_group_barrier(0x008, 3, 0);
            __builtin_amdgcn_sched_group_barrier(0x100, 2, 0); __builtin_amdgcn_sched_group_barrier(0x008, 3, 0);
            __builtin_amdgcn_sched_group_barrier(0x100, 2, 0); __builtin_amdgcn_sched_group_barrier(0x008, 3, 0);
            __builtin_amdgcn_sched_group_barrier(0x100, 2, 0); __builtin_amdgcn_sched_group_barrier(0x008, 3, 0);
            __builtin_amdgcn_sched_group_barrier(0x100, 2, 0); __builtin_amdgcn_sched_group_barrier(0x008, 3, 0);
            __builtin_amdgcn_s_setprio(0);
        };
        wl_bar();
        wl_static_for<3>([&](auto J) { b0[decltype(J)::value] = fragB(wl_ic<0>{}, J); });
        wl_static_for<PRE>([&](auto I) { afr[decltype(I)::value] = fragA(wl_ic<0>{}, I); });
        for (int h = 0; h < NH; h += 12) {
            half(wl_ic<0>{}, b0, b1); half(wl_ic<1>{}, b1, b0);
            if (h + 2 >= NH) break;
            half(wl_ic<2>{}, b0, b1); half(wl_ic<3>{}, b1, b0);
            if (h + 4 >= NH) break;
            half(wl_ic<4>{}, b0, b1); half(wl_ic<5>{}, b1, b0);
            if (h + 6 >= NH) break;
            half(wl_ic<6>{}, b0, b1); half(wl_ic<7>{}, b1, b0);
            if (h + 8 >= NH) break;
            half(wl_ic<8>{}, b0, b1); half(wl_ic<9>{}, b1, b0);
            if (h + 10 >= NH) break;
            half(wl_ic<10>{}, b0, b1); half(wl_ic<11>{}, b1, b0);
        }
        wl_bar();
        const float beta = P.beta;
#pragma unroll
        for (int i = 0; i < 8; ++i) {
            const int n = n0 + 128 * (i >> 2) + 64 * grp + 16 * (i & 3) + c16;
#pragma unroll
            for (int j = 0; j < 3; ++j) {
                const int k = k0 + wc * 48 + 16 * j + 4 * g;
                if (n < q.Nn && k < q.Kk) {
                    f32x4* o = reinterpret_cast<f32x4*>(q.C + (int64_t)n * q.ldc + k);
                    f32x4 v = acc[i][j];
                    if (beta != 0.f) { const f32x4 c = *o; v[0] += beta * c[0]; v[1] += beta * c[1]; v[2] += beta * c[2]; v[3] += beta * c[3]; }
                    *o = v;
                }
            }
        }
    }
}

int wgrad_lw_launch(const dgx_wgrad_problem* pr, int n, float beta, hipStream_t st) {
    if (n <= 0 || n > WL_MAXP) return DGX_ERR_UNSUPPORTED;
    WlParams P;
    memset((void*)&P, 0, sizeof(P));
    int items = 0;
    for (int i = 0; i < n; ++i) {
        const dgx_wgrad_problem& p = pr[i];
        if (!p.dy || !p.x || !p.gw || p.M <= 0 || (p.Nn & 7) || (p.Kk & 7)) return DGX_ERR_BAD_ARG;
        if ((int64_t)p.M * p.Nn * 2 >= (1ll << 31) || (int64_t)p.M * p.Kk * 2 >= (1ll << 31)) return DGX_ERR_UNSUPPORTED;
        WlProb& q = P.p[i];
        q.A = (const uint16_t*)p.dy; q.B = (const uint16_t*)p.x; q.C = p.gw; q.gb = p.gb;
        q.M = p.M; q.Nn = p.Nn; q.Kk = p.Kk; q.ldc = p.Kk;
        q.tiles_k = (p.Kk + WL_TK - 1) / WL_TK;
        q.item0 = items;
        items += ((p.Nn + WL_TN - 1) / WL_TN) * q.tiles_k;
    }
    for (int i = 0; i < WL_MAXP; ++i) P.item0[i] = i < n ? P.p[i].item0 : 0x7fffffff;
    P.n = n; P.total = items; P.beta = beta;
    P.per_xcd = (items + 7) / 8;
    static bool once = false;
    if (!once) {
        if (hipFuncSetAttribute((const void*)wgrad_lw_kernel, hipFuncAttributeMaxDynamicSharedMemorySize, WL_LDS) != hipSuccess) return DGX_ERR_UNSUPPORTED;
        once = true;
    }
    extern int dgx_get_reserved_cus(void);
    const int avail = 32 - dgx_get_reserved_cus() / 8;
    const int wgx = P.per_xcd < avail ? P.per_xcd : avail;
    hipLaunchKernelGGL(wgrad_lw_kernel, dim3(8 * wgx), dim3(WL_THREADS), WL_LDS, st, P);
    return DGX_OK;
}

int g_dgx_dev_wgrad_lw = 1;
bool wgrad_lw_wants(const dgx_wgrad_problem* pr, int n) {
    const int mode = g_dgx_dev_wgrad_lw;
    if (!mode || n <= 0 || n > WL_MAXP) return false;
    int items = 0;
    for (int i = 0; i < n; ++i) {
        if (pr[i].M < 1024) return false;
        items += ((pr[i].Nn + WL_TN - 1) / WL_TN) * ((pr[i].Kk + WL_TK - 1) / WL_TK);
    }
    if (mode == 2) return true;
    if (items < 192) return false;
    const int rounds = (items + 255) / 256;
    return (double)items / (256.0 * rounds) >= 0.74;
}
```

divergen_amd/csrc/window_attention.hip:

```cpp
#include "dgx_common.h"
#include <type_traits>
#include <map>
#include <mutex>
#include <utility>
#include "winmap.h"
#if defined(__HIP_DEVICE_COMPILE__) && !defined(__gfx950__)
#error "window_attention.hip orders the bias-gradient slot hand-over by store COMPLETION (sc1 stores acknowledged at the device coherence point; see flush_head): verified for gfx950 only"
#endif
typedef float wa_f32x2 __attribute__((ext_vector_type(2)));

template <int WS> struct WinCfg;
template <> struct WinCfg<12> { static constexpr int N = 144, NT = 9, NTK = 10, RS = 168, TBL = 529; };
template <> struct WinCfg<7>  { static constexpr int N = 49,  NT = 4, NTK = 4,  RS = 72,  TBL = 169; };

__device__ __forceinline__ bf16x8 ld_frag_global(const uint16_t* p, bool ok) {
    bf16x8 z = {0, 0, 0, 0, 0, 0, 0, 0};
    return ok ? *reinterpret_cast<const bf16x8*>(p) : z;
}

template <int N, int NP, int RS>
__device__ __forceinline__ void stage_transposed(uint16_t* T, const uint16_t* src, int64_t row_stride,
                                                 int tid, int nthreads) {
    constexpr int HALF = NP / 2;
    for (int u = tid; u < HALF * 4; u += nthreads) {
        const int c = u / HALF, m = u - c * HALF;
        const int r0 = 2 * m, r1 = r0 + 1;
        bf16x8 v0 = ld_frag_global(src + (int64_t)r0 * row_stride + 8 * c, r0 < N);
        bf16x8 v1 = ld_frag_global(src + (int64_t)r1 * row_stride + 8 * c, r1 < N);
#pragma unroll
        for (int i = 0; i < 8; ++i) {
            uint32_t w = (uint32_t)(uint16_t)v0[i] | ((uint32_t)(uint16_t)v1[i] << 16);
            *reinterpret_cast<uint32_t*>(&T[(8 * c + i) * RS + r0]) = w;
        }
    }
}

template <int RS>
__device__ __forceinline__ bf16x8 ld_frag_T(const uint16_t* T, int row, int t, int g) {
    const uint2 a = *reinterpret_cast<const uint2*>(&T[row * RS + 32 * t + 4 * g]);
    const uint2 b = *reinterpret_cast<const uint2*>(&T[row * RS + 32 * t + 16 + 4 * g]);
    u32x4 v = {a.x, a.y, b.x, b.y};
    return __builtin_bit_cast(bf16x8, v);
}

template <int N, int NP, int RR>
__device__ __forceinline__ void stage_rows(uint16_t* img, const uint16_t* src, int64_t row_stride, int tid, int nthreads) {
    for (int u = tid; u < NP * 4; u += nthreads) {
        const int r = u >> 2, c = u & 3;
        *reinterpret_cast<bf16x8*>(&img[r * RR + 8 * c]) = ld_frag_global(src + (int64_t)r * row_stride + 8 * c, r < N);
    }
}

__device__ __forceinline__ void block_to_window_head(int bid, int nH, int& b, int& h) {
    const int xcd = bid & 7, slot = bid >> 3;
    b = (slot / nH) * 8 + xcd;
    h = slot % nH;
}

struct AttnGeom {
    int H, W, shift;
    int T, P;
    const uint16_t* bias;
    const uint16_t* zeros;
};
template <int WS>
__device__ __forceinline__ int attn_row(const AttnGeom& G, const WmGeom& g, const WmWindow& w, int img, int wr, int wc, int n) {
    const int i = n / WS, j = n - i * WS;
    int before;
    const bool real = wm_token_real(g, w, wr, wc, i, j, before);
    const int wi = wr * g.nWw + wc;
    return real ? img * (G.H * G.W) + w.base + before : -(1 + img * G.P + (wi * (WS * WS) - w.base) + (n - before));
}

#define DGX_LOG2E 1.4426950408889634f
#define DGX_LN2 0.6931471805599453f
template <int WS, bool MASKED, bool COMPACT = false>
__global__ __launch_bounds__(WinCfg<WS>::NT * 64) void win_attn_fwd_kernel(
    const uint16_t* __restrict__ qkv, const float* __restrict__ table, const int8_t* __restrict__ region,
    uint16_t* __restrict__ out, float* __restrict__ lse, int B_, int nW, int nH, float scale, int64_t t_sh, int64_t t_si,
    AttnGeom G = AttnGeom{0, 0, 0, 0, 0, nullptr, nullptr}) {
    using Cf = WinCfg<WS>;
    constexpr int N = Cf::N, NT = Cf::NT, NTK = Cf::NTK, NP = NTK * 16, RS = Cf::RS, TBL = Cf::TBL;
    constexpr int RR = WS == 12 ? 48 : 40;
    __shared__ __attribute__((aligned(16))) uint16_t Vs[NP * RR];
    __shared__ __attribute__((aligned(16))) uint16_t Ks[NP * RR];
    __shared__ float tbl[TBL];
    __shared__ __attribute__((aligned(16))) int koff_s[NP];
    __shared__ __attribute__((aligned(16))) int kreg_s[NP];
    static_assert(TBL <= NT * 64 && NP <= NT * 64 && NP * 4 <= 2 * NT * 64, "one prologue load per thread and array");

    int b, h;
    block_to_window_head(blockIdx.x, nH, b, h);
    if (b >= B_) return;
    const int C = nH * 32;
    const int64_t rowst = 3 * (int64_t)C;
    const uint16_t* base = qkv + (int64_t)b * N * rowst + h * 32;
    const int tid = threadIdx.x, nthreads = NT * 64;
    const int w = tid >> 6, l = tid & 63, g = l >> 4, c16 = l & 15;
    const int qi = 16 * w + c16;
    const bool qok = qi < N;
    WmGeom wg;
    WmWindow ww;
    int img = 0, wr = 0, wc = 0;
    if (COMPACT) {
        wg = wm_geom(G.H, G.W, WS, G.shift);
        img = b / nW;
        const int wi = b - img * nW;
        wr = wi / wg.nWw;
        wc = wi - wr * wg.nWw;
        ww = wm_window(wg, wr, wc);
    }
    const bool wfull = COMPACT && ww.rh == WS && ww.rw == WS;
    auto row_of = [&](int n) -> int {
        if (wfull) return img * (G.H * G.W) + ww.base + n;
        return attn_row<WS>(G, wg, ww, img, wr, wc, n);
    };
    auto row_ptr = [&](int n) -> const uint16_t* {
        if (!COMPACT) return base + (int64_t)n * rowst;
        const int row = row_of(n < N ? n : 0);
        return (row >= 0 ? qkv + (int64_t)row * rowst : G.bias) + h * 32;
    };

    const int8_t* reg = region + (int64_t)(b % nW) * N;
    const float tv = tid < TBL ? table[h * t_sh + tid * t_si] : 0.f;
    const int kr_in = (MASKED && tid < N) ? (int)reg[tid] : -1;
    const int rq = (MASKED && qok) ? (int)reg[qi] : 0;
    const int u0 = tid, u1 = tid + nthreads;
    const uint16_t* r0 = row_ptr(u0 >> 2);
    const uint16_t* r1 = row_ptr(u1 >> 2);
    const bf16x8 k0 = ld_frag_global(r0 + C + 8 * (u0 & 3), (u0 >> 2) < N);
    const bf16x8 v0 = ld_frag_global(r0 + 2 * C + 8 * (u0 & 3), (u0 >> 2) < N);
    const bool two = u1 < NP * 4;
    const bf16x8 k1 = ld_frag_global(r1 + C + 8 * (u1 & 3), two && (u1 >> 2) < N);
    const bf16x8 v1 = ld_frag_global(r1 + 2 * C + 8 * (u1 & 3), two && (u1 >> 2) < N);
    const int q_row = COMPACT ? row_of(qok ? qi : 0) : 0;
    const bf16x8 qf = ld_frag_global(COMPACT ? (q_row >= 0 ? qkv + (int64_t)q_row * rowst : G.bias) + h * 32 + 8 * g : base + (int64_t)qi * rowst + 8 * g, qok);
    if (tid < TBL) tbl[tid] = tv * DGX_LOG2E;
    if (tid < NP) {
        const int yk = tid / WS;
        koff_s[tid] = tid < N ? yk * (2 * WS - 1) + (tid - yk * WS) : 0;
        kreg_s[tid] = kr_in;
    }
    if (u0 < NP * 4) {
        *reinterpret_cast<bf16x8*>(&Ks[(u0 >> 2) * RR + 8 * (u0 & 3)]) = k0;
        *reinterpret_cast<bf16x8*>(&Vs[(u0 >> 2) * RR + 8 * (u0 & 3)]) = v0;
    }
    if (two) {
        *reinterpret_cast<bf16x8*>(&Ks[(u1 >> 2) * RR + 8 * (u1 & 3)]) = k1;
        *reinterpret_cast<bf16x8*>(&Vs[(u1 >> 2) * RR + 8 * (u1 & 3)]) = v1;
    }
    __syncthreads();

    const int yq = qi / WS, xq = qi - yq * WS;
    const int base_q = qok ? (yq + WS - 1) * (2 * WS - 1) + (xq + WS - 1) : (WS - 1) * (2 * WS - 1) + (WS - 1);
    const float scale2 = scale * DGX_LOG2E;
    DGX_LDS const float* tbl_q = lds_opaque(tbl + base_q);
    DGX_LDS const int* koff_g = lds_opaque(koff_s + 4 * g);
    DGX_LDS const int* kreg_g = lds_opaque(kreg_s + 4 * g);

    float p[NTK][4];
    float mx = -INFINITY;
#pragma unroll
    for (int kt = 0; kt < NTK; ++kt) {
        const bf16x8 kf = *reinterpret_cast<const bf16x8*>(&Ks[(16 * kt + c16) * RR + 8 * g]);
        f32x4 z = {0.f, 0.f, 0.f, 0.f};
        const f32x4 acc = mfma16(kf, qf, z);
        const i32x4 ko = *reinterpret_cast<DGX_LDS const i32x4*>(koff_g + 16 * kt);
        i32x4 kr4 = {0, 0, 0, 0};
        if (MASKED) kr4 = *reinterpret_cast<DGX_LDS const i32x4*>(kreg_g + 16 * kt);
#pragma unroll
        for (int r = 0; r < 4; ++r) {
            float s = __builtin_fmaf(acc[r], scale2, tbl_q[-ko[r]]);
            if (MASKED) s += kr4[r] != rq ? -100.0f * DGX_LOG2E : 0.0f;
            if (NP != N && 16 * kt + 4 * g + r >= N) s = -INFINITY;
            p[kt][r] = s;
// ... 119 lines not shown
    DGX_LDS const int* reg_g = reinterpret_cast<DGX_LDS const int*>(lse_g) + 3 * NP;
    DGX_LDS uint16_t* ds_w = lds_opaque(dSt + key * RD + 4 * g);

    const uint32_t st_qk_c = (uint32_t)(srow * (int)rowst + 8 * sc);
    const uint32_t st_o_c = (uint32_t)(srow * C + 8 * sc);
    const uint32_t row4_c = (uint32_t)((kok ? key : 0) * (int)rowst + 4 * g);
    auto compact_row = [&](int b, int n) -> int {
        const WmGeom wg = wm_geom(G.H, G.W, WS, G.shift);
        const int img = b / nW, wi = b - img * nW, wr = wi / wg.nWw, wc = wi - wr * wg.nWw;
        const WmWindow ww = wm_window(wg, wr, wc);
        if (ww.rh == WS && ww.rw == WS) return img * (G.H * G.W) + ww.base + n;
        return attn_row<WS>(G, wg, ww, img, wr, wc, n);
    };
    auto issue = [&](int b, int h, BwdPrefetch& P) {
        if (COMPACT) {
            const int row = compact_row(b, stager ? srow : 0);
            const uint16_t* qp = (row >= 0 ? qkv + (int64_t)row * rowst : G.bias) + h * 32 + 8 * sc;
            const uint16_t* dp = row >= 0 ? dout + (int64_t)row * C + h * 32 + 8 * sc : G.zeros + 8 * sc;
            const uint16_t* op = row >= 0 ? out + (int64_t)row * C + h * 32 + 8 * sc : G.zeros + 8 * sc;
            if (stager) {
                P.q = *reinterpret_cast<const bf16x8*>(qp);
                P.k = *reinterpret_cast<const bf16x8*>(qp + C);
                P.v = *reinterpret_cast<const bf16x8*>(qp + 2 * C);
                P.d = *reinterpret_cast<const bf16x8*>(dp);
                P.o = *reinterpret_cast<const bf16x8*>(op);
                P.lse = (lse + ((int64_t)b * nH + h) * N)[(uint32_t)srow];
                P.reg = (int)(region + (MASKED ? (int64_t)(b % nW) * N : 0))[(uint32_t)srow];
            }
            return;
        }
        const uint16_t* base = qkv + (int64_t)b * N * rowst + h * 32;
        const uint16_t* dob = dout + (int64_t)b * N * C + h * 32;
        const uint16_t* ob = out + (int64_t)b * N * C + h * 32;
        uint32_t st_qk = st_qk_c, st_o = st_o_c;
        asm volatile("" : "+v"(st_qk), "+v"(st_o));
        if (stager) {
            P.q = *reinterpret_cast<const bf16x8*>(base + st_qk);
            P.k = *reinterpret_cast<const bf16x8*>(base + C + st_qk);
            P.v = *reinterpret_cast<const bf16x8*>(base + 2 * C + st_qk);
            P.d = *reinterpret_cast<const bf16x8*>(dob + st_o);
            P.o = *reinterpret_cast<const bf16x8*>(ob + st_o);
            P.lse = (lse + ((int64_t)b * nH + h) * N)[(uint32_t)srow];
            P.reg = (int)(region + (int64_t)(b % nW) * N)[(uint32_t)srow];
        }
    };

    BwdPrefetch P;
    {
        const bf16x8 z = {0, 0, 0, 0, 0, 0, 0, 0};
        P.q = P.d = P.o = P.k = P.v = z;
        P.lse = INFINITY;
        P.reg = 0;
    }
    if (count > 0) issue(b, h, P);
    auto load_head = [&](int hh) {
        constexpr int NTHR = (NT + (HELP ? 3 : 0)) * 64, KT = (TBL + NTHR - 1) / NTHR;
        float tv[KT];
#pragma unroll
        for (int k = 0; k < KT; ++k) {
            const int i = tid + k * NTHR;
            tv[k] = table[hh * dt_sh + (i < TBL ? i : 0) * dt_si];
        }
#pragma unroll
        for (int k = 0; k < KT; ++k) {
            const int i = tid + k * NTHR;
            if (i < TBL) { tbl[i] = tv[k] * DGX_LOG2E; tblacc[i] = 0.f; }
        }
        if (PK) {
            __syncthreads();
            for (int i = tid; i < 4 * TBLS; i += nthreads) {
                const int sft = i / TBLS, j = i - sft * TBLS + sft;
                tbl4[i] = j < TBL ? tbl[j] : 0.f;
            }
        }
    };
    load_head(h);
    auto zero_pads = [&]() {
        for (int i = tid; i < (NP - N) * RR; i += nthreads) { Qs[N * RR + i] = 0; dOs[N * RR + i] = 0; Ks[N * RR + i] = 0; Vs[N * RR + i] = 0; }
        for (int i = tid; i < (NP - N) * RD; i += nthreads) dSt[N * RD + i] = 0;
    };
    zero_pads();
    for (int i = tid; i < NP; i += nthreads) {
        const int yq = i / WS;
        qoff_s[i] = i < N ? yq * (2 * WS - 1) + (i - yq * WS) : 0;
        if (i >= N) {
            if (PK) { lse_s[2 * i] = -INFINITY; lse_s[2 * i + 1] = 0.f; }
            else { lse_s[i] = -INFINITY; delta_s[i] = 0.f; }
            reg_s[i] = 0;
        }
    }
    const int yk = key / WS, xk = key - yk * WS;
    const int kbase = kok ? (WS - 1) * (2 * WS - 1) + (WS - 1) - (yk * (2 * WS - 1) + xk) : 0;
    const float kneg = kok ? 0.0f : -INFINITY;
    const float scale2 = scale * DGX_LOG2E, inv_scale = 1.0f / scale;
    DGX_LDS const float* tbl_k = lds_opaque(tbl + kbase);
    DGX_LDS const float* bptr[NT];
#pragma unroll
    for (int qt = 0; qt < NT; ++qt) {
        const int q0 = 16 * qt + 4 * g, y0 = q0 / WS;
        const int idx0 = kbase + y0 * (2 * WS - 1) + (q0 - y0 * WS);
        bptr[qt] = lds_opaque(tbl4 + (idx0 & 3) * TBLS + (idx0 & ~3));
    }
    float dbias[NT][4];
#pragma unroll
    for (int i = 0; i < NT; ++i)
#pragma unroll
        for (int r = 0; r < 4; ++r) dbias[i][r] = 0.f;
// ... 37 lines not shown
                for (int r = 0; r < 4; ++r) {
                    const int q = 16 * qt + 4 * g + r;
                    if (q < N) M[krow + 16 * qt + r] = dbias[qt][r];
                    dbias[qt][r] = 0.f;
                }
            }
        }
        __syncthreads();
        const int lrun0 = left > 0 ? (hh * left) / upl : 0;
        const int nlrun = left > 0 ? ((hh + 1) * left - 1) / upl - lrun0 + 1 : 0;
        const int slot = (int)blockIdx.x < main_wgs ? (int)blockIdx.x / nH : q_runs + ((int)blockIdx.x - main_wgs - lrun0);
        float* mine = part_ws + ((int64_t)hh * slots_per_head + slot) * TBLP;
        for (int i = tid; i < TBL; i += nthreads) {
            const int iy = i / (2 * WS - 1), dy = iy - (WS - 1), dx = i - iy * (2 * WS - 1) - (WS - 1);
            const int yk0 = dy < 0 ? -dy : 0, yk1 = dy > 0 ? WS - dy : WS, xk0 = dx < 0 ? -dx : 0, xk1 = dx > 0 ? WS - dx : WS;
            float sum = 0.f;
            for (int yk = yk0; yk < yk1; ++yk) {
                DGX_LDS const float* row = M + (yk * WS) * LDM + (yk + dy) * WS + dx;
                for (int xk = xk0; xk < xk1; ++xk) sum += row[xk * (LDM + 1)];
            }
            __hip_atomic_store(mine + i, sum, __ATOMIC_RELAXED, __HIP_MEMORY_SCOPE_AGENT);
        }
        asm volatile("s_waitcnt vmcnt(0)" ::: "memory");
        __syncthreads();
        if (tid == 0) last_s = __hip_atomic_fetch_add(&head_cnt[hh], 1, __ATOMIC_RELAXED, __HIP_MEMORY_SCOPE_AGENT) == q_runs + nlrun - 1;
        __syncthreads();
        if (last_s) {
            const float* p0 = part_ws + (int64_t)hh * slots_per_head * TBLP;
            const int ns = q_runs + nlrun;
            for (int i = tid; i < TBL; i += nthreads) {
                float sum = dtable[hh * dt_sh + i * dt_si];
                for (int s0 = 0; s0 < ns; s0 += 16) {
                    float v[16];
#pragma unroll
                    for (int k = 0; k < 16; ++k)
                        v[k] = __hip_atomic_load(p0 + (s0 + k < ns ? s0 + k : s0) * TBLP + i, __ATOMIC_RELAXED, __HIP_MEMORY_SCOPE_AGENT);
#pragma unroll
                    for (int k = 0; k < 16; ++k) sum += s0 + k < ns ? v[k] : 0.f;
                }
                dtable[hh * dt_sh + i * dt_si] = sum;
            }
            if (tid == 0) __hip_atomic_store(&head_cnt[hh], 0, __ATOMIC_RELAXED, __HIP_MEMORY_SCOPE_AGENT);
        }
    };
    if (count > 0) stage();
    int done = 0;
    while (done < count) {
    const int seg = min(count - done, hi - b);
    for (int u = 0; u < seg; ++u) {
        const bool more = done + u + 1 < count;
        const bool wrap = u + 1 == seg;
        const int bn = b + 1 == hi ? lo : b + 1, hn = b + 1 == hi ? h + 1 : h;
        __syncthreads();
        if (more) issue(bn, hn, P);
        const bf16x8 kf = *reinterpret_cast<const bf16x8*>(&Ks[(kok ? key : 0) * RR + 8 * g]);
        const bf16x8 vf = *reinterpret_cast<const bf16x8*>(&Vs[(kok ? key : 0) * RR + 8 * g]);
        const int rk = MASKED ? reg_s[kok ? key : 0] : 0;

        f32x4 dV[2] = {{0.f, 0.f, 0.f, 0.f}, {0.f, 0.f, 0.f, 0.f}};
        f32x4 dK[2] = {{0.f, 0.f, 0.f, 0.f}, {0.f, 0.f, 0.f, 0.f}};
        constexpr int TSPLIT = 3;
        bool mixed = false;
        if (MASKED) {
            const int r0 = reg_s[0];
            bool diff = false;
            for (int i = l; i < N; i += 64) diff = diff || reg_s[i] != r0;
            mixed = __builtin_amdgcn_readfirstlane((int)(__ballot(diff) != 0ull)) != 0;
        }
        const bool MK = MASKED && mixed;
#pragma unroll
        for (int t = 0; t < NTK / 2; ++t) {
            if (HELP && (t < TSPLIT ? helper : shared)) continue;
            uint32_t ppk[2][2], dpk[2][2];
#pragma unroll
            for (int hh = 0; hh < 2; ++hh) {
                const int qt = 2 * t + hh;
                float pv[4] = {0.f, 0.f, 0.f, 0.f}, dsv[4] = {0.f, 0.f, 0.f, 0.f};
                if (qt < NT) {
                    const bf16x8 qa = *reinterpret_cast<DGX_LDS const bf16x8*>(q_row + 16 * qt * RR);
                    const bf16x8 da = *reinterpret_cast<DGX_LDS const bf16x8*>(do_row + 16 * qt * RR);
                    f32x4 lv, dl, bv = {0.f, 0.f, 0.f, 0.f};
                    i32x4 ov = {0, 0, 0, 0}, rv = {0, 0, 0, 0};
                    if constexpr (PK) {
                        const wa_f32x2 ld = *reinterpret_cast<DGX_LDS const wa_f32x2*>(ld_lane + 32 * qt);
                        lv = f32x4{quad_bcast<0>(ld.x), quad_bcast<1>(ld.x), quad_bcast<2>(ld.x), quad_bcast<3>(ld.x)};
                        dl = f32x4{quad_bcast<0>(ld.y), quad_bcast<1>(ld.y), quad_bcast<2>(ld.y), quad_bcast<3>(ld.y)};
                        bv = *reinterpret_cast<DGX_LDS const f32x4*>(bptr[qt]);
                        if (MK) {
                            const int rq1 = reg_lane[16 * qt];
                            rv = i32x4{quad_bcast<0>(rq1), quad_bcast<1>(rq1), quad_bcast<2>(rq1), quad_bcast<3>(rq1)};
                        }
                    } else {
                        lv = *reinterpret_cast<DGX_LDS const f32x4*>(lse_g + 16 * qt);
                        dl = *reinterpret_cast<DGX_LDS const f32x4*>(delta_g + 16 * qt);
                        ov = *reinterpret_cast<DGX_LDS const i32x4*>(qoff_g + 16 * qt);
                        if (MK) rv = *reinterpret_cast<DGX_LDS const i32x4*>(reg_g + 16 * qt);
                    }
                    const f32x4 s = mfma16(qa, kf, lv);
                    const f32x4 dp = mfma16(da, vf, dl);
#pragma unroll
                    for (int r = 0; r < 4; ++r) {
                        float sv = __builtin_fmaf(s[r], scale2, PK ? bv[r] : tbl_k[ov[r]]);
                        if (N % 16 != 0) sv += kneg;
                        if (MK) sv += rv[r] != rk ? -100.0f * DGX_LOG2E : 0.0f;
                        pv[r] = __builtin_amdgcn_exp2f(sv);
                        dsv[r] = pv[r] * dp[r];
                        dbias[qt < NT ? qt : 0][r] += dsv[r];
// ... 93 lines not shown
    std::lock_guard<std::mutex> lock(mu);
    int device = 0;
    if (hipGetDevice(&device) != hipSuccess) return nullptr;
    BwdTableWs& w = pool[std::make_pair(device, st)];
    hipStreamCaptureStatus cap = hipStreamCaptureStatusNone;
    const bool capturing = hipStreamIsCapturing(st, &cap) == hipSuccess && cap != hipStreamCaptureStatusNone;
    if (w.part && w.floats >= floats && w.heads >= heads) {
        if (w.dirty || capturing) {
            if (hipMemsetAsync(w.cnt, 0, (size_t)w.heads * 4, st) != hipSuccess) return nullptr;
            if (!capturing) w.dirty = false;
        }
        return &w;
    }
    if (w.part && capturing) return nullptr;
    hipStreamCaptureMode mode = hipStreamCaptureModeRelaxed;
    if (capturing && hipThreadExchangeStreamCaptureMode(&mode) != hipSuccess) return nullptr;
    if (w.part) { (void)hipStreamSynchronize(st); (void)hipFree(w.part); (void)hipFree(w.cnt); w.part = nullptr; w.cnt = nullptr; }
    const int64_t nf = floats > (int64_t)300 * 532 ? floats : (int64_t)300 * 532;
    const int nh = heads > 64 ? heads : 64;
    bool ok = hipMalloc((void**)&w.part, (size_t)nf * 4) == hipSuccess;
    if (!ok) w.part = nullptr;
    if (ok && hipMalloc((void**)&w.cnt, (size_t)nh * 4) != hipSuccess) { (void)hipFree(w.part); w.part = nullptr; w.cnt = nullptr; ok = false; }
    if (capturing) (void)hipThreadExchangeStreamCaptureMode(&mode);
    if (!ok) return nullptr;
    if (hipMemsetAsync(w.cnt, 0, (size_t)nh * 4, st) != hipSuccess) return nullptr;
    w.floats = nf; w.heads = nh;
    w.dirty = capturing;
    return &w;
}

static const int8_t* zero_region() {
    static int8_t* z = nullptr;
    if (!z) {
        if (hipMalloc((void**)&z, 256) != hipSuccess) return nullptr;
        (void)hipMemset(z, 0, 256);
    }
    return z;
}

static int attn_geom(AttnGeom& G, int B_, int& nW, int ws, int B, int H, int W, int shift, const void* qkv_bias, int nH) {
    if (B <= 0 || H <= 0 || W <= 0 || shift < 0 || shift >= ws || !qkv_bias || !wm_compact_ok(H, W, ws, shift)) return DGX_ERR_BAD_ARG;
    const WmGeom g = wm_geom(H, W, ws, shift);
    nW = g.nWh * g.nWw;
    if ((int64_t)B * nW != B_) return DGX_ERR_BAD_ARG;
    const int64_t Tw = (int64_t)B_ * ws * ws;
    if (Tw * 3 * nH * 32 >= ((int64_t)1 << 32)) return DGX_ERR_UNSUPPORTED;
    G.H = H; G.W = W; G.shift = shift;
    G.T = B * H * W;
    G.P = nW * ws * ws - H * W;
    G.bias = (const uint16_t*)qkv_bias;
    return DGX_OK;
}

static int attn_fwd_launch(const void* qkv, const float* table, int64_t table_stride_head, int64_t table_stride_index, const int8_t* region,
                           void* out, float* lse, int B_, int nW, int nH, int ws, float scale, const AttnGeom* geom, void* stream) {
    if (B_ <= 0) return DGX_OK;
    if (!qkv || !table || !out || !lse || nH <= 0 || nW <= 0 || (region && B_ % nW)) return DGX_ERR_BAD_ARG;
    hipStream_t st = (hipStream_t)stream;
    const bool masked = region != nullptr;
    if (!region) { region = zero_region(); if (!geom) nW = 1; if (!region) return DGX_ERR_BAD_ARG; }
    const int grid = ((B_ + 7) / 8) * 8 * nH;
    const double heads = (double)B_ * nH, ntok = (double)ws * ws;
    DgxProfScope prof(DGX_PROF_ATTN_FWD, stream, heads * 2.0 * 2.0 * ntok * ntok * 32.0, heads * ntok * (32.0 * 2.0 * 4.0 + 4.0));
    AttnGeom G = geom ? *geom : AttnGeom{0, 0, 0, 0, 0, nullptr, nullptr};
#define FWD_LAUNCH(WSV, MK, CP) hipLaunchKernelGGL((win_attn_fwd_kernel<WSV, MK, CP>), dim3(grid), dim3(WinCfg<WSV>::NT * 64), 0, st, \
                                                  (const uint16_t*)qkv, table, region, (uint16_t*)out, lse, B_, nW, nH, scale, \
                                                  table_stride_head, table_stride_index, G)
#define FWD_LAUNCH_C(WSV, MK) do { if (geom) FWD_LAUNCH(WSV, MK, true); else FWD_LAUNCH(WSV, MK, false); } while (0)
    if (ws == 12) { if (masked) FWD_LAUNCH_C(12, true); else FWD_LAUNCH_C(12, false); }
    else if (ws == 7) { if (masked) FWD_LAUNCH_C(7, true); else FWD_LAUNCH_C(7, false); }
#undef FWD_LAUNCH_C
#undef FWD_LAUNCH
    else
        return DGX_ERR_UNSUPPORTED;
    DGX_LAUNCH_CHECK();
    return DGX_OK;
}

extern "C" int dgx_window_attention_fwd(const void* qkv, const float* table, int64_t table_stride_head,
                                        int64_t table_stride_index, const int8_t* region, void* out, float* lse, int B_,
                                        int nW, int nH, int ws, float scale, void* stream) {
    return attn_fwd_launch(qkv, table, table_stride_head, table_stride_index, region, out, lse, B_, nW, nH, ws, scale, nullptr, stream);
}

extern "C" int dgx_window_attention_fwd_compact(const void* qkv, const void* qkv_bias, const float* table, int64_t table_stride_head,
                                                int64_t table_stride_index, const int8_t* region, void* out, float* lse, int B, int H, int W,
                                                int nH, int ws, int shift, float scale, void* stream) {
    if (ws != 12 && ws != 7) return DGX_ERR_UNSUPPORTED;
    AttnGeom G = {0, 0, 0, 0, 0, nullptr, nullptr};
    int nW = 0;
    const int nWh = (H + ws - 1) / ws, nWw = (W + ws - 1) / ws;
    const int B_ = B * nWh * nWw;
    if (int rc = attn_geom(G, B_, nW, ws, B, H, W, shift, qkv_bias, nH)) return rc;
    return attn_fwd_launch(qkv, table, table_stride_head, table_stride_index, region, out, lse, B_, nW, nH, ws, scale, &G, stream);
}

static int attn_bwd_launch(const void* qkv, const float* table, const int8_t* region, const void* out,
                           const float* lse, const void* dout, void* dqkv, float* dtable,
                           int64_t dtable_stride_head, int64_t dtable_stride_index, int B_, int nW, int nH,
                           int ws, float scale, const AttnGeom* geom, void* stream) {
    if (B_ <= 0) return DGX_OK;
    if (!qkv || !table || !out || !lse || !dout || !dqkv || !dtable || nH <= 0 || nW <= 0 || (region && B_ % nW))
        return DGX_ERR_BAD_ARG;
    hipStream_t st = (hipStream_t)stream;
    const bool masked = region != nullptr;
    if (!region) { region = zero_region(); if (!geom) nW = 1; if (!region) return DGX_ERR_BAD_ARG; }
    AttnGeom G = geom ? *geom : AttnGeom{0, 0, 0, 0, 0, nullptr, nullptr};
    if (geom) { G.zeros = (const uint16_t*)zero_region(); if (!G.zeros) return DGX_ERR_BAD_ARG; }
    extern int dgx_get_reserved_cus(void);
    const int cus = 256 - dgx_get_reserved_cus();
    const int64_t total = (int64_t)B_ * nH;
    if (total > 0x7fffffff) return DGX_ERR_UNSUPPORTED;
    int upw = (int)((total + cus - 1) / cus);
    if (upw > B_) upw = B_;
    const int left = B_ % upw, main_wgs = (B_ / upw) * nH;
    int upl = upw;
    if (left > 0 && cus > main_wgs) {
        upl = (nH * left + (cus - main_wgs) - 1) / (cus - main_wgs);
        if (upl > upw) upl = upw;
    }
    const int grid = main_wgs + (nH * left + upl - 1) / upl;
    const double heads = (double)B_ * nH, ntok = (double)ws * ws;
    DgxProfScope prof(DGX_PROF_ATTN_BWD, stream, heads * 5.0 * 2.0 * ntok * ntok * 32.0, heads * ntok * (32.0 * 2.0 * 8.0 + 4.0));
    const int64_t tblp = ((2 * ws - 1) * (2 * ws - 1) + 3) / 4 * 4;
    BwdTableWs* tw = bwd_table_ws(st, (int64_t)nH * (B_ / upw + (left > 0 ? (left + upl - 1) / upl + 1 : 0)) * tblp, nH);
    if (!tw) return DGX_ERR_UNSUPPORTED;
#define BWD_ARGS (const uint16_t*)qkv, table, region, (const uint16_t*)out, lse, (const uint16_t*)dout, (uint16_t*)dqkv, dtable, B_, nW, nH, \
                 scale, upw, upl, tw->part, tw->cnt, dtable_stride_head, dtable_stride_index, G
    if (ws == 12) {
        static bool once = false;
        const size_t sm = bwd_smem_bytes<12>(true);
        if (!once) {
            (void)hipFuncSetAttribute((const void*)win_attn_bwd_kernel<12, true, true>, hipFuncAttributeMaxDynamicSharedMemorySize, (int)sm);
            (void)hipFuncSetAttribute((const void*)win_attn_bwd_kernel<12, false, true>, hipFuncAttributeMaxDynamicSharedMemorySize, (int)sm);
            (void)hipFuncSetAttribute((const void*)win_attn_bwd_kernel<12, true, true, true>, hipFuncAttributeMaxDynamicSharedMemorySize, (int)sm);
            (void)hipFuncSetAttribute((const void*)win_attn_bwd_kernel<12, false, true, true>, hipFuncAttributeMaxDynamicSharedMemorySize, (int)sm);
            once = true;
        }
#define BWD12(MK, CP) hipLaunchKernelGGL((win_attn_bwd_kernel<12, MK, true, CP>), dim3(grid), dim3((WinCfg<12>::NT + 3) * 64), sm, st, BWD_ARGS)
        if (masked) { if (geom) BWD12(true, true); else BWD12(true, false); }
        else { if (geom) BWD12(false, true); else BWD12(false, false); }
#undef BWD12
    } else if (ws == 7) {
        const size_t sm = bwd_smem_bytes<7>();
#define BWD7(MK, CP) hipLaunchKernelGGL((win_attn_bwd_kernel<7, MK, false, CP>), dim3(grid), dim3(WinCfg<7>::NT * 64), sm, st, BWD_ARGS)
        if (masked) { if (geom) BWD7(true, true); else BWD7(true, false); }
        else { if (geom) BWD7(false, true); else BWD7(false, false); }
#undef BWD7
    } else {
        return DGX_ERR_UNSUPPORTED;
    }
#undef BWD_ARGS
    if (hipError_t e = hipGetLastError(); e != hipSuccess) {
        tw->dirty = true;
        return -(int)e - 1000;
    }
    return DGX_OK;
}

extern "C" int dgx_window_attention_bwd(const void* qkv, const float* table, const int8_t* region, const void* out,
                                        const float* lse, const void* dout, void* dqkv, float* dtable,
                                        int64_t dtable_stride_head, int64_t dtable_stride_index, int B_, int nW, int nH,
                                        int ws, float scale, void* stream) {
    return attn_bwd_launch(qkv, table, region, out, lse, dout, dqkv, dtable, dtable_stride_head, dtable_stride_index, B_, nW, nH, ws, scale,
                           nullptr, stream);
}

extern "C" int dgx_window_attention_bwd_compact(const void* qkv, const void* qkv_bias, const float* table, const int8_t* region, const void* out,
                                                const float* lse, const void* dout, void* dqkv, float* dtable, int64_t dtable_stride_head,
                                                int64_t dtable_stride_index, int B, int H, int W, int nH, int ws, int shift, float scale,
                                                void* stream) {
    if (ws != 12 && ws != 7) return DGX_ERR_UNSUPPORTED;
    AttnGeom G = {0, 0, 0, 0, 0, nullptr, nullptr};
    int nW = 0;
    const int nWh = (H + ws - 1) / ws, nWw = (W + ws - 1) / ws;
    const int B_ = B * nWh * nWw;
    if (int rc = attn_geom(G, B_, nW, ws, B, H, W, shift, qkv_bias, nH)) return rc;
    return attn_bwd_launch(qkv, table, region, out, lse, dout, dqkv, dtable, dtable_stride_head, dtable_stride_index, B_, nW, nH, ws, scale,
                           &G, stream);
}
```

divergen_amd/layers/gemm_ops.py:

```python
import ctypes

import torch

from .. import _lib as L

BF16 = torch.bfloat16
EPI_NONE, EPI_BIAS, EPI_BIAS_GELU, EPI_BIAS_RESIDUAL, EPI_GELU_GRAD, EPI_RELU_GRAD = 0, 1, 2, 3, 4, 5


def _check2(a, b):
    if a.dtype != BF16 or b.dtype != BF16:
        raise L.DgxError("dgx_gemm_bf16_nt takes bfloat16 operands")
    if a.dim() != 2 or b.dim() != 2 or a.shape[1] != b.shape[1]:
        raise L.DgxError("gemm_nt: a (M, K) x b (N, K): got %s, %s" % (tuple(a.shape), tuple(b.shape)))
    if a.stride(1) != 1 or b.stride(1) != 1:
        raise L.DgxError("gemm_nt: operands must be K-contiguous")


_WS = {}
WS_BYTES = 64 << 20


def _workspace(dev):
    key = (dev, L.stream())
    ws = _WS.get(key)
    if ws is None:
        ws = _WS[key] = torch.empty(WS_BYTES, dtype=torch.uint8, device=dev)
    return ws


def _launch(a, b, ep):
    M, K = a.shape
    N = b.shape[0]
    if M * N * 8 <= WS_BYTES:
        ws = _workspace(a.device)
        ep.workspace, ep.workspace_bytes = ws.data_ptr(), WS_BYTES
    L.check(L.lib().dgx_gemm_bf16_nt(a.data_ptr(), b.data_ptr(), M, N, K, a.stride(0), b.stride(0), ctypes.byref(ep), L.stream()),
            "dgx_gemm_bf16_nt")


def _dev_ptr(t):
    if t is None:
        return None
    if not t.is_cuda:
        raise L.DgxError("libdgx ops need GPU (ROCm) tensors; got a %s tensor -- no CPU fallback exists" % t.device)
    return t.data_ptr()


def gemm_nt(a, b, bias=None, out=None):
    _check2(a, b)
    _dev_ptr(a), _dev_ptr(b)
    M, N = a.shape[0], b.shape[0]
    c = out if out is not None else torch.empty(M, N, dtype=BF16, device=a.device)
    ep = L.GemmEpilogue()
    ep.mode = EPI_BIAS if bias is not None else EPI_NONE
    ep.c, ep.ldc, ep.bias = c.data_ptr(), c.stride(0), _dev_ptr(bias)
    _launch(a, b, ep)
    return c


def gemm_nt_act(a, b, bias=None, relu=False):
    _check2(a, b)
    M, N = a.shape[0], b.shape[0]
    c = torch.empty(M, N, dtype=BF16, device=a.device)
    ep = L.GemmEpilogue()
    ep.mode = EPI_BIAS if bias is not None else EPI_NONE
    ep.c, ep.ldc, ep.bias, ep.relu = c.data_ptr(), N, _dev_ptr(bias), int(bool(relu))
    _launch(a, b, ep)
    return c


def gemm_bias_gelu(a, b, bias):
    _check2(a, b)
    M, N = a.shape[0], b.shape[0]
    f1 = torch.empty(M, N, dtype=BF16, device=a.device)
    act = torch.empty(M, N, dtype=BF16, device=a.device)
    ep = L.GemmEpilogue()
    ep.mode = EPI_BIAS_GELU
    ep.c, ep.ldc, ep.bias, ep.c2 = f1.data_ptr(), N, _dev_ptr(bias), act.data_ptr()
    _launch(a, b, ep)
    return f1, act


def gemm_gelu_grad(a, b, f1):
    _check2(a, b)
    M, N = a.shape[0], b.shape[0]
    assert f1.shape == (M, N) and f1.dtype == BF16 and f1.is_contiguous()
    c = torch.empty(M, N, dtype=BF16, device=a.device)
    ep = L.GemmEpilogue()
    ep.mode = EPI_GELU_GRAD
    ep.c, ep.ldc, ep.aux, ep.ldaux = c.data_ptr(), N, f1.data_ptr(), N
    _launch(a, b, ep)
    return c


def gemm_relu_grad(a, b, act):
    _check2(a, b)
    M, N = a.shape[0], b.shape[0]
    assert act.shape == (M, N) and act.dtype == BF16 and act.is_contiguous()
    c = torch.empty(M, N, dtype=BF16, device=a.device)
    ep = L.GemmEpilogue()
    ep.mode = EPI_RELU_GRAD
    ep.c, ep.ldc, ep.aux, ep.ldaux = c.data_ptr(), N, act.data_ptr(), N
    _launch(a, b, ep)
    return c


def gemm_bias_residual(a, b, bias, res, scale, B, H, W, ws, shift):
    _check2(a, b)
    N = b.shape[0]
    res = res.contiguous()
    assert res.shape[-1] == N and res.numel() == B * H * W * N
    out = torch.empty_like(res)
    ep = L.GemmEpilogue()
    ep.mode = EPI_BIAS_RESIDUAL
    ep.bias, ep.residual, ep.out, ep.scale = _dev_ptr(bias), res.data_ptr(), out.data_ptr(), _dev_ptr(scale)
    ep.residual_dtype = L.dtype_code(res)
    ep.B, ep.H, ep.W, ep.ws, ep.shift = B, H, W, ws, shift
    _launch(a, b, ep)
    return out


def dev_time_us(a, b, bias=None, iters=30, mode=None):
    _check2(a, b)
    M, N = a.shape[0], b.shape[0]
    c = torch.empty(M, N, dtype=BF16, device=a.device)
    ep = L.GemmEpilogue()
    ep.mode = (EPI_BIAS if bias is not None else EPI_NONE) if mode is None else mode
    ep.c, ep.ldc, ep.bias = c.data_ptr(), N, _dev_ptr(bias)
    if mode in (EPI_BIAS_GELU, EPI_GELU_GRAD):
        extra = torch.randn(M, N, device=a.device).to(BF16)
        ep.c2, ep.aux, ep.ldaux = extra.data_ptr(), extra.data_ptr(), N
    fn = L.lib().dgx_dev_gemm_time_us
    fn.restype = ctypes.c_float
    fn.argtypes = [L.c_p, L.c_p, L.c_i, L.c_i, L.c_i, L.c_i64, L.c_i64, ctypes.POINTER(L.GemmEpilogue), L.c_i, L.c_p]
    return float(fn(a.data_ptr(), b.data_ptr(), M, N, a.shape[1], a.stride(0), b.stride(0), ctypes.byref(ep), iters, L.stream()))
```

divergen_amd/layers/linear_ops.py:

```python
import torch
import torch.nn as nn

from .. import _lib as L

BF16 = torch.bfloat16


def pad8(n):
    return (n + 7) // 8 * 8


def wgrad_into(g2, dy2, x2, beta=1.0, gb=None):
    M, Nn = dy2.shape
    Kk = x2.shape[1]
    if not (dy2.is_cuda and Nn % 8 == 0 and Kk % 8 == 0 and g2.is_contiguous() and dy2.dtype == BF16 and x2.dtype == BF16
            and M * max(Nn, Kk) * 2 < (1 << 31)):
        raise L.DgxError("wgrad_into: dy %s %s x %s %s -- libdgx takes bf16 GPU operands with widths that are multiples of 8"
                         % (tuple(dy2.shape), dy2.dtype, tuple(x2.shape), x2.dtype))
    wgrad_grouped([(g2, dy2.contiguous(), x2.contiguous(), gb)], beta)


def _wgrad_array(problems):
    n = len(problems)
    arr = (L.WgradProblem * n)()
    for i, pr in enumerate(problems):
        g2, dy2, x2 = pr[:3]
        gb = pr[3] if len(pr) > 3 else None
        assert g2.is_contiguous() and dy2.is_contiguous() and x2.is_contiguous()
        assert dy2.dtype == BF16 and x2.dtype == BF16 and g2.dtype == torch.float32
        assert gb is None or (gb.dtype == torch.float32 and gb.is_contiguous() and gb.numel() == dy2.shape[1])
        arr[i].dy, arr[i].x, arr[i].gw = dy2.data_ptr(), x2.data_ptr(), g2.data_ptr()
        arr[i].gb = gb.data_ptr() if gb is not None else None
        arr[i].M, arr[i].Nn, arr[i].Kk = dy2.shape[0], dy2.shape[1], x2.shape[1]
    return arr


def wgrad_group_form(problems):
    n = len(problems)
    return 0 if n == 0 or n > 32 else int(L.lib().dgx_wgrad_grouped_form(_wgrad_array(problems), n))


def wgrad_grouped(problems, beta=1.0):
    n = len(problems)
    arr = _wgrad_array(problems)
    lib = L.lib()
    nbytes = int(lib.dgx_wgrad_grouped_workspace_bytes(arr, n))
    ws = torch.empty(max(nbytes, 16), dtype=torch.uint8, device=problems[0][1].device)
    L.check(lib.dgx_linear_wgrad_grouped(arr, n, float(beta), L.ptr(ws), L.stream()), "dgx_linear_wgrad_grouped")


_READY_SUSPENDED = [False]
SEGMENT_MODES = {}


class suspend_ready:

    def __enter__(self):
        self.prev = _READY_SUSPENDED[0]
        _READY_SUSPENDED[0] = True

    def __exit__(self, *a):
        _READY_SUSPENDED[0] = self.prev


def notify_ready(p):
    r = getattr(p, "_dgx_ready", None)
    if r is not None and not _READY_SUSPENDED[0] and not (p.is_cuda and torch.cuda.is_current_stream_capturing()):
        r()


def shadow(p):
    s = getattr(p, "_dgx16", None)
    return s if s is not None else p.detach().to(BF16)


def shadow_t(p):
    s = getattr(p, "_dgx16t", None)
    if s is not None:
        return s
    w = shadow(p)
    return w.reshape(w.shape[0], -1).t().contiguous()


def shadow_padded(p):
    s = getattr(p, "_dgx16g", None)
    if s is None:
# ... 193 lines not shown
```

divergen_amd/layers/swin_block.py:

```python
import torch

from .. import _lib as L
from . import gemm_ops as G
from .linear_ops import BF16, notify_ready, shadow, shadow_t, wgrad_group_form, wgrad_grouped


def arena_resident(params):
    return all(p.is_leaf and getattr(p, "_dgx16", None) is not None and p.grad is not None
               and p.grad.dtype == torch.float32 for p in params)


def _ready(*params):
    for p in params:
        notify_ready(p)


def colsum_into(gb, dy2, beta=1.0):
    M, N = dy2.shape
    lib = L.lib()
    ws = torch.empty(max(int(lib.dgx_colsum_workspace_bytes(M, N)), 4), dtype=torch.uint8, device=dy2.device)
    L.check(lib.dgx_colsum_bf16(L.ptr(dy2), L.ptr(gb), M, N, float(beta), L.ptr(ws), L.stream()), "dgx_colsum_bf16")


def colsum_grouped(problems, beta=1.0):
    n = len(problems)
    arr = (L.ColsumProblem * n)()
    for i, (gb, dy2) in enumerate(problems):
        arr[i].dy, arr[i].out, arr[i].M, arr[i].N = dy2.data_ptr(), gb.data_ptr(), dy2.shape[0], dy2.shape[1]
    lib = L.lib()
    ws = torch.empty(max(int(lib.dgx_colsum_grouped_workspace_bytes(arr, n)), 4), dtype=torch.uint8, device=problems[0][1].device)
    L.check(lib.dgx_colsum_grouped(arr, n, float(beta), L.ptr(ws), L.stream()), "dgx_colsum_grouped")


import os
_PAIR = 3
_PENDING = []
_PENDING_LW = []
_CB_QUEUED = [False]
_ROUND, _MAXP = 256, 12
_LW_MIN_M = 4096
_LW_ITEMS, _LW_MAXP = 1000, 32


def _lw_items(g):
    return (-(-g.shape[0] // 256)) * (-(-g.shape[1] // 192))


def _tiles(g):
    return (-(-g.shape[0] // 256)) * (-(-g.shape[1] // 256))


def _launch(items):
    members = [q for (g, d, x_, b, w), _ in items for q in ((w,) if b is None else (w, b))]
    slot = getattr(members[0], "_dgx_arena_slot", None)
    first = slot is not None and all(getattr(q, "_dgx_arena_slot", (None,))[0] is slot[0] for q in members) and slot[0].claim_first_write(members)
    wgrad_grouped([(g, d, x_, b.grad if b is not None else None) for (g, d, x_, b, w), _ in items], beta=0.0 if first else 1.0)
    for (g, d, x_, b, w), _ in items:
        _ready(w) if b is None else _ready(w, b)


def flush_wgrads(final=True):
    if final:
        _CB_QUEUED[0] = False
        _flush_ln()
        _flush_lw()
    while _PENDING:
        if not final and sum(t for _, t in _PENDING) < _ROUND:
            break
        pick, rest, s = [], [], 0
        for it in _PENDING:
            if len(pick) < _MAXP and (s + it[1] <= _ROUND or not pick):
                pick.append(it)
                s += it[1]
            else:
                rest.append(it)
        _PENDING[:] = rest
        _launch(pick)


def reset_pending():
    if _PENDING or _PENDING_LW or _PENDING_LN:
        import warnings
        warnings.warn("divergen_amd: %d pending weight gradients dropped (LayerNorm parameter folds included; an earlier backward pass did not finish)"
                      % (len(_PENDING) + len(_PENDING_LW) + len(_PENDING_LN)))
        del _PENDING[:]
        del _PENDING_LW[:]
        del _PENDING_LN[:]
    _CB_QUEUED[0] = False


_PENDING_LN = []
_PENDING_LN_KEY = [None]


def _flush_ln():
    if not _PENDING_LN:
        return
    import ctypes
    n = len(_PENDING_LN)
    T, C = _PENDING_LN_KEY[0]
    arr = lambda vals: (ctypes.c_void_p * n)(*vals)
    L.check(L.lib().dgx_layernorm_param_reduce_n(arr([p.data_ptr() for p, _, _ in _PENDING_LN]), arr([w.grad.data_ptr() for _, w, _ in _PENDING_LN]),
                                                 arr([b.grad.data_ptr() for _, _, b in _PENDING_LN]), n, T, C, L.stream()),
            "dgx_layernorm_param_reduce_n")
    for _, w, b in _PENDING_LN:
        _ready(w, b)
    del _PENDING_LN[:]


def _defer_ln_reduce(part, norms, T, C):
    n2w, n2b, n1w, n1b = norms
    if _PENDING_LN and _PENDING_LN_KEY[0] != (T, C):
        _flush_ln()
    if any(w is n2w or w is n1w for _, w, _ in _PENDING_LN):
        _flush_ln()
    _PENDING_LN_KEY[0] = (T, C)
    _PENDING_LN.append((part[0], n2w, n2b))
    _PENDING_LN.append((part[1], n1w, n1b))
    if len(_PENDING_LN) >= 16:
        _flush_ln()


def _flush_lw():
    if not _PENDING_LW:
        return
    items = [[p, _tiles(p[0])] for p in _PENDING_LW]
    del _PENDING_LW[:]
    if wgrad_group_form([(g, d, x_, b.grad if b is not None else None) for (g, d, x_, b, w), _ in items]):
        _launch(items)
    else:
        _flush_all()
        _PENDING.extend(items)
        _flush_all()


def _queue_callback():
    if (_PENDING or _PENDING_LW or _PENDING_LN) and not _CB_QUEUED[0]:
        _CB_QUEUED[0] = True
        torch.autograd.Variable._execution_engine.queue_callback(flush_wgrads)


def _defer_wgrads(wgrads, params):
    blk = sum(_tiles(p[0]) for p in wgrads)
    M = wgrads[0][1].shape[0]
    if _PENDING_LW and _PENDING_LW[0][1].shape[0] != M:
        _flush_lw()
    if _LW_MIN_M and min(p[1].shape[0] for p in wgrads) >= _LW_MIN_M and sum(_lw_items(p[0]) for p in wgrads) >= 128 and wgrads[0][1].is_cuda:
        if len(_PENDING_LW) + len(wgrads) > _LW_MAXP:
            _flush_lw()
        _PENDING_LW.extend(wgrads)
        if sum(_lw_items(p[0]) for p in _PENDING_LW) >= _LW_ITEMS or len(_PENDING_LW) + len(wgrads) > _LW_MAXP:
            _flush_lw()
        _queue_callback()
        return
    if _PENDING and _PENDING[0][0][1].shape[0] != M:
        _flush_all()
    if _PAIR >= 3 and 2 * blk <= _ROUND:
        _PENDING.extend([p, _tiles(p[0])] for p in wgrads)
        flush_wgrads(final=False)
    else:
        _PENDING.extend([p, 0] for p in wgrads)
        if len(_PENDING) // 4 >= min(_PAIR, 2):
            _flush_all()
    _queue_callback()


def _flush_all():
    while _PENDING:
        items = _PENDING[:_MAXP]
        del _PENDING[:_MAXP]
        _launch(items)


def _linear_bwd(dy2, x2, weight, bias, wgrads, gelu_of=None):
    wgrads.append((weight.grad.view(weight.shape[0], -1), dy2, x2, bias, weight))
    wt = shadow_t(weight)
    return G.gemm_gelu_grad(dy2, wt, gelu_of) if gelu_of is not None else G.gemm_nt(dy2, wt)


_HANDOVER = [None]


def _take_handover(g, s2):
    h, _HANDOVER[0] = _HANDOVER[0], None
    if h is None or h[0].data_ptr() != g.data_ptr() or h[0].shape != g.shape or h[0].dtype != g.dtype:
        return None
    same_scale = (h[1] is None and s2 is None) or (h[1] is not None and s2 is not None and h[1].data_ptr() == s2.data_ptr())
    return h[2] if same_scale else None


COMPACT = True


def compact_ok(H, W, ws, shift):
    nWh, nWw = -(-H // ws), -(-W // ws)
    return COMPACT and (nWh * ws != H or nWw * ws != W) and H >= shift and W >= shift


class _SwinBlockFn(torch.autograd.Function):
    @staticmethod
    def forward(ctx, x, region, s1, s2, cfg, prev_scale, n1w, n1b, qw, qb, table, pw, pb, n2w, n2b, w1, b1, w2, b2):
        ctx.prev_scale = prev_scale
        B, H, W, ws, shift, nH, scale, eps1, eps2 = cfg
        lib, st, dev = L.lib(), L.stream(), x.device
        x = x.contiguous()
        C = x.shape[-1]
        T = B * H * W
        code = L.dtype_code(x)
        nW = (-(-H // ws)) * (-(-W // ws))
        B_, N = B * nW, ws * ws
        Tw = B_ * N
        f32 = torch.float32
        compact = compact_ok(H, W, ws, shift)
        wsm = -ws if compact else ws
        Tr = T if compact else Tw
        xw = torch.empty(Tw, C, dtype=BF16, device=dev)
        mean1 = torch.empty(T, dtype=f32, device=dev)
        rstd1 = torch.empty(T, dtype=f32, device=dev)
        L.check(lib.dgx_layernorm_fwd(x.data_ptr(), n1w.data_ptr(), n1b.data_ptr(), xw.data_ptr(), mean1.data_ptr(),
                                      rstd1.data_ptr(), T, C, eps1, B, H, W, wsm, shift, code, st), "dgx_layernorm_fwd")
        qkv = G.gemm_nt(xw[:Tr], shadow(qw), shadow(qb))
        tbl = table.detach()
        o = torch.empty(Tr, C, dtype=BF16, device=dev)
        lse = torch.empty(B_, nH, N, dtype=f32, device=dev)
        if compact:
            L.check(lib.dgx_window_attention_fwd_compact(qkv.data_ptr(), shadow(qb).data_ptr(), tbl.data_ptr(), tbl.stride(1), tbl.stride(0),
                                                         L.ptr(region), o.data_ptr(), lse.data_ptr(), B, H, W, nH, ws, shift, scale, st),
                    "dgx_window_attention_fwd_compact")
        else:
            L.check(lib.dgx_window_attention_fwd(qkv.data_ptr(), tbl.data_ptr(), tbl.stride(1), tbl.stride(0), L.ptr(region),
                                                 o.data_ptr(), lse.data_ptr(), B_, nW, nH, ws, scale, st), "dgx_window_attention_fwd")
        x1 = G.gemm_bias_residual(o, shadow(pw), shadow(pb), x.view(B, H * W, C), s1, B, H, W, wsm, shift).view(x.shape)
        h2 = torch.empty(T, C, dtype=BF16, device=dev)
        mean2 = torch.empty(T, dtype=f32, device=dev)
        rstd2 = torch.empty(T, dtype=f32, device=dev)
        L.check(lib.dgx_layernorm_fwd(x1.data_ptr(), n2w.data_ptr(), n2b.data_ptr(), h2.data_ptr(), mean2.data_ptr(),
                                      rstd2.data_ptr(), T, C, eps2, 0, 0, 0, 0, 0, code, st), "dgx_layernorm_fwd")
        f1, a = G.gemm_bias_gelu(h2, shadow(w1), shadow(b1))
        out = G.gemm_bias_residual(a, shadow(w2), shadow(b2), x1.view(B, H * W, C), s2, B, H, W, 0, 0).view(x.shape)
        ctx.save_for_backward(x, mean1, rstd1, xw, qkv, region, o, lse, x1, mean2, rstd2, h2, f1, a, s1, s2)
        ctx.params = (n1w, n1b, qw, qb, table, pw, pb, n2w, n2b, w1, b1, w2, b2)
        ctx.cfg = cfg
        return out

    @staticmethod
    def backward(ctx, g):
        x, mean1, rstd1, xw, qkv, region, o, lse, x1, mean2, rstd2, h2, f1, a, s1, s2 = ctx.saved_tensors
        n1w, n1b, qw, qb, table, pw, pb, n2w, n2b, w1, b1, w2, b2 = ctx.params
        B, H, W, ws, shift, nH, scale, eps1, eps2 = ctx.cfg
        lib, st, dev = L.lib(), L.stream(), g.device
        g = g.contiguous()
        C = x.shape[-1]
        T = B * H * W
        code = L.dtype_code(x)
        nW = (-(-H // ws)) * (-(-W // ws))
        B_, N = B * nW, ws * ws
        Tw = B_ * N
        df2 = _take_handover(g, s2)
        if df2 is None:
            if s2 is None and g.dtype == BF16:
                df2 = g.view(T, C)
            else:
                df2 = torch.empty(T, C, dtype=BF16, device=dev)
                L.check(lib.dgx_residual_bwd(g.data_ptr(), L.ptr(s2), df2.data_ptr(), B, H, W, C, 0, 0, code, st), "dgx_residual_bwd")
        wgrads = []
        df1 = _linear_bwd(df2, a, w2, b2, wgrads, gelu_of=f1)
        dh2 = _linear_bwd(df1, h2, w1, b1, wgrads)
        nblk = lib.dgx_layernorm_bwd_blocks(T)
        part = torch.empty(2, nblk * 2 * C, dtype=torch.float32, device=dev)
        compact = compact_ok(H, W, ws, shift)
        wsm = -ws if compact else ws
        Tr = T if compact else Tw
        dx1 = torch.empty_like(x)
        dpr = torch.empty(Tr, C, dtype=BF16, device=dev)
        L.check(lib.dgx_layernorm_bwd_emit(dh2.data_ptr(), x1.data_ptr(), mean2.data_ptr(), rstd2.data_ptr(), n2w.data_ptr(),
                                           g.data_ptr(), dx1.data_ptr(), None, None, part[0].data_ptr(),
                                           T, C, 0, 0, 0, 0, 0, code, dpr.data_ptr(), L.ptr(s1), B, H, W, wsm, shift, st),
                "dgx_layernorm_bwd_emit")
        do = _linear_bwd(dpr, o, pw, pb, wgrads)
        dqkv = torch.empty(Tw, qkv.shape[1], dtype=BF16, device=dev)
        assert table.grad.stride() == table.stride()
        if compact:
            L.check(lib.dgx_window_attention_bwd_compact(qkv.data_ptr(), shadow(qb).data_ptr(), table.data_ptr(), L.ptr(region), o.data_ptr(),
                                                         lse.data_ptr(), do.data_ptr(), dqkv.data_ptr(), table.grad.data_ptr(), table.stride(1),
                                                         table.stride(0), B, H, W, nH, ws, shift, scale, st), "dgx_window_attention_bwd_compact")
            _ready(table)
            wgrads.append((qw.grad.view(qw.shape[0], -1), dqkv, xw, qb, qw))
            dxw = G.gemm_nt(dqkv[:T], shadow_t(qw))
        else:
            L.check(lib.dgx_window_attention_bwd(qkv.data_ptr(), table.data_ptr(), L.ptr(region), o.data_ptr(), lse.data_ptr(),
                                                 do.data_ptr(), dqkv.data_ptr(), table.grad.data_ptr(), table.stride(1), table.stride(0),
                                                 B_, nW, nH, ws, scale, st), "dgx_window_attention_bwd")
            _ready(table)
            dxw = _linear_bwd(dqkv, xw, qw, qb, wgrads)
        prev = ctx.prev_scale
        if prev and (prev[0] is not None or dx1.dtype != BF16):
            scaled = torch.empty(T, C, dtype=BF16, device=dev)
            L.check(lib.dgx_layernorm_bwd_emit(dxw.data_ptr(), x.data_ptr(), mean1.data_ptr(), rstd1.data_ptr(), n1w.data_ptr(),
                                               dx1.data_ptr(), dx1.data_ptr(), None, None, part[1].data_ptr(),
                                               T, C, B, H, W, wsm, shift, code, scaled.data_ptr(), L.ptr(prev[0]), B, H, W, 0, 0, st),
                    "dgx_layernorm_bwd_emit")
            _HANDOVER[0] = (dx1, prev[0], scaled)
        else:
            L.check(lib.dgx_layernorm_bwd(dxw.data_ptr(), x.data_ptr(), mean1.data_ptr(), rstd1.data_ptr(), n1w.data_ptr(),
                                          dx1.data_ptr(), dx1.data_ptr(), None, None, part[1].data_ptr(),
                                          T, C, B, H, W, wsm, shift, code, st), "dgx_layernorm_bwd")
        _defer_ln_reduce(part, (n2w, n2b, n1w, n1b), T, C)
        _defer_wgrads(wgrads, (w2, w1, pw, qw, b2, b1, pb, qb))
        return (dx1,) + (None,) * 18


def swin_block(x, region, s1, s2, cfg, params):
    prev = getattr(x, "_dgx_next_scale", None)
    with torch.autocast("cuda", enabled=False):
        out = _SwinBlockFn.apply(x, region, s1, s2, cfg, prev, *params)
    out._dgx_next_scale = (s2,)
    return out
```

include/divergen_hip.h:

```cpp
#ifndef DIVERGEN_HIP_H
#define DIVERGEN_HIP_H

#include <stddef.h>
#include <stdint.h>

#ifdef __cplusplus
extern "C" {
#endif

#define DGX_OK 0
#define DGX_ERR_BAD_ARG (-1)
#define DGX_ERR_UNSUPPORTED (-2)
#define DGX_F32 0
#define DGX_BF16 1

const char* dgx_build_arch(void);
int dgx_abi_version(void);

int dgx_host_register(void* p, size_t bytes);
int dgx_host_unregister(void* p);
int dgx_memcpy_h2d_async(void* dst, const void* src, size_t bytes, void* stream);

int dgx_window_attention_fwd(const void* qkv, const float* table, int64_t table_stride_head,
                             int64_t table_stride_index, const int8_t* region, void* out, float* lse, int B_,
                             int nW, int nH, int ws, float scale, void* stream);

int dgx_window_attention_bwd(const void* qkv, const float* table, const int8_t* region,
                             const void* out, const float* lse, const void* dout,
                             void* dqkv, float* dtable, int64_t dtable_stride_head,
                             int64_t dtable_stride_index, int B_, int nW, int nH, int ws, float scale,
                             void* stream);

int dgx_window_attention_fwd_compact(const void* qkv, const void* qkv_bias, const float* table, int64_t table_stride_head,
                                     int64_t table_stride_index, const int8_t* region, void* out, float* lse, int B, int H,
                                     int W, int nH, int ws, int shift, float scale, void* stream);
int dgx_window_attention_bwd_compact(const void* qkv, const void* qkv_bias, const float* table, const int8_t* region,
                                     const void* out, const float* lse, const void* dout, void* dqkv, float* dtable,
                                     int64_t dtable_stride_head, int64_t dtable_stride_index, int B, int H, int W, int nH,
                                     int ws, int shift, float scale, void* stream);

int dgx_window_gather(const void* x, void* xw, int B, int H, int W, int C, int ws, int shift,
                      int dtype, void* stream);
int dgx_window_scatter(const void* xw, void* x, int B, int H, int W, int C, int ws, int shift,
                       int dtype, void* stream);

int dgx_roi_align_fwd(const void* feat, const float* rois, void* out, int N, int H, int W, int C,
                      int R, float spatial_scale, int ph, int pw, int sampling_ratio, int aligned,
                      int out_nhwc, int dtype, void* stream);
int dgx_roi_align_bwd(const void* grad_out, const float* rois, float* grad_feat, int N, int H,
                      int W, int C, int R, float spatial_scale, int ph, int pw, int sampling_ratio,
                      int aligned, int out_nhwc, int dtype, void* stream);

int dgx_roi_pooler_fwd(const void* const* feats, const int* Hs, const int* Ws, int num_levels,
                       int min_level, const float* rois, void* out, int32_t* levels_out, int N,
                       int C, int R, int ph, int pw, int sampling_ratio, int out_nhwc, int dtype,
                       void* stream);
int dgx_roi_pooler_bwd(const void* grad_out, float* const* grad_feats, const int* Hs, const int* Ws,
                       int num_levels, int min_level, const float* rois, int N, int C, int R, int ph,
                       int pw, int sampling_ratio, int out_nhwc, int dtype, void* stream);

int dgx_roi_pooler_bwd_gather(const void* grad_out, void* const* grad_feats, const int* Hs, const int* Ws,
                              int num_levels, int min_level, float spatial_scale, int aligned, const float* rois,
                              int N, int C, int R, int ph, int pw, int sampling_ratio, int dtype, void* stream);
int dgx_roi_pooler_bwd_gather_accum(const void* grad_out, void* const* grad_feats, const int* Hs, const int* Ws,
                                    int num_levels, int min_level, float spatial_scale, int aligned, const float* rois,
                                    int N, int C, int R, int ph, int pw, int sampling_ratio, int accumulate, float grad_scale,
                                    int dtype, void* stream);

int dgx_mask_crop(const uint8_t* masks, const float* boxes, const int32_t* mask_idx, uint8_t* out,
                  int M, int H, int W, int R, int S, void* stream);

int dgx_nms_sorted(const float* boxes, int n, float iou_thr, uint64_t* mask, uint8_t* keep,
                   int32_t* num_keep, void* stream);
int64_t dgx_nms_workspace_words(int n);

int64_t dgx_nms_batched_workspace_words(int B, int K);
int dgx_nms_batched(const float* boxes, const float* scores, const int32_t* n_valid, int B, int K,
                    float iou_thr, int max_keep, uint64_t* mask, int32_t* keep_idx, int cap,
                    int32_t* num_keep, void* stream);

int dgx_iou_match(const float* gt, int M, const float* props, int N, float thr,
                  int64_t* matched_idx, int8_t* matched_label, float* max_iou, void* stream);

int dgx_centernet_scores(const void* const* hm_levels, int hm_pixel_stride, int hm_channel, const int32_t* level_hw,
                         const int32_t* strides, int L, int B, float thr, float* scores, int32_t* n_valid, int dtype, void* stream);
int dgx_centernet_decode(const void* const* reg_levels, int reg_pixel_stride, int reg_channel, const int32_t* level_hw,
                         const int32_t* strides, int L, int B, const int64_t* cand_idx, int Kc, const float* scores, float thr,
                         float* boxes, float* out_scores, int32_t* n_valid, int dtype, void* stream);
int dgx_gather_boxes(const float* boxes, const int64_t* order, int B, int K, float* out, void* stream);
int dgx_topk_index_rows(const float* scores, int64_t row_stride, int B, const int32_t* level_off, const int32_t* level_n,
                        const int32_t* level_n_host, int nlev, int k, int64_t* out, int64_t out_row_stride, void* stream);
int dgx_sort_rows_desc(const float* in, int B, int K, float* out_vals, int64_t* out_order, void* stream);
// ... 84 lines not shown
int dgx_im2col3x3(const void* x, void* col, int N, int H, int W, int C, int stride, int dtype,
                  void* stream);
int dgx_col2im3x3(const void* dcol, void* dx, int N, int H, int W, int C, int stride, int dtype,
                  void* stream);

int64_t dgx_wgrad_workspace_bytes(int M, int Nn, int Kk);
int dgx_linear_wgrad(const void* dy, const void* x, float* gw, int M, int Nn, int Kk, float beta,
                     void* workspace, void* stream);

int dgx_layernorm_fwd(const void* x, const float* gamma, const float* beta, void* y_bf16, float* mean,
                      float* rstd, int64_t T, int C, float eps, int B, int H, int W, int ws, int shift,
                      int x_dtype, void* stream);
int dgx_layernorm_bwd_blocks(int64_t T);
int dgx_layernorm_bwd(const void* dy_bf16, const void* x, const float* mean, const float* rstd,
                      const float* gamma, const void* dres, void* dx, float* dgamma, float* dbeta, float* part,
                      int64_t T, int C, int B, int H, int W, int ws, int shift, int x_dtype, void* stream);
int dgx_layernorm_bwd_emit(const void* dy_bf16, const void* x, const float* mean, const float* rstd, const float* gamma,
                           const void* dres, void* dx, float* dgamma, float* dbeta, float* part, int64_t T, int C, int B, int H,
                           int W, int ws, int shift, int x_dtype, void* emit_bf16, const float* emit_scale, int eB, int eH,
                           int eW, int ews, int eshift, void* stream);
int dgx_layernorm_param_reduce2(const float* part_a, float* dgamma_a, float* dbeta_a, const float* part_b, float* dgamma_b,
                                float* dbeta_b, int64_t T, int C, void* stream);
int dgx_layernorm_param_reduce_n(const float* const* parts, float* const* dgammas, float* const* dbetas, int n, int64_t T, int C,
                                 void* stream);
int dgx_layernorm_f32out_fwd(const void* x, const float* gamma, const float* beta, float* y, float* mean,
                             float* rstd, int64_t T, int C, float eps, int x_dtype, void* stream);
int dgx_layernorm_f32out_bwd(const float* dy, const void* x, const float* mean, const float* rstd,
                             const float* gamma, void* dx, float* dgamma, float* dbeta, float* part, int64_t T,
                             int C, int x_dtype, void* stream);
int dgx_patch_merge_ln_fwd(const void* x, const float* gamma, const float* beta, void* y_bf16, float* mean,
                           float* rstd, int B, int H, int W, int C0, float eps, int x_dtype, void* stream);
int dgx_patch_merge_ln_bwd(const void* dy_bf16, const void* x, const float* mean, const float* rstd,
                           const float* gamma, void* dx, float* dgamma, float* dbeta, float* part, int B, int H,
                           int W, int C0, int x_dtype, void* stream);

int dgx_l2norm_rows_fwd(const void* x, void* y_bf16, float* rnorm, int64_t R, int D, float t, int x_dtype, void* stream);
int dgx_l2norm_rows_bwd(const void* g_bf16, const void* x, const float* rnorm, void* dx_bf16, int64_t R, int D, float t,
                        int x_dtype, void* stream);

int dgx_residual_fwd(const void* x, const void* y_bf16, const float* scale, void* out, int B, int H, int W,
                     int C, int ws, int shift, int x_dtype, void* stream);
int dgx_residual_bwd(const void* g, const float* scale, void* dy_bf16, int B, int H, int W, int C, int ws,
                     int shift, int g_dtype, void* stream);

int dgx_upsample2x_add_fwd(const void* lat, const void* top, void* out, int N, int H, int W, int C, int dtype, void* stream);
int dgx_upsample2x_add_bwd(const void* g, void* gtop, int N, int H, int W, int C, int dtype, void* stream);

typedef struct dgx_wgrad_problem {
    const void* dy;
    const void* x;
    float* gw;
    int M, Nn, Kk;
    float* gb;
} dgx_wgrad_problem;
int64_t dgx_wgrad_grouped_workspace_bytes(const dgx_wgrad_problem* problems, int n);
int dgx_linear_wgrad_grouped(const dgx_wgrad_problem* problems, int n, float beta, void* workspace,
                             void* stream);
int dgx_wgrad_grouped_form(const dgx_wgrad_problem* problems, int n);

int64_t dgx_colsum_workspace_bytes(int M, int N);
int dgx_colsum_bf16(const void* dy_bf16, float* out, int M, int N, float beta, void* workspace, void* stream);
typedef struct dgx_colsum_problem {
    const void* dy;
    float* out;
    int M, N;
} dgx_colsum_problem;
int64_t dgx_colsum_grouped_workspace_bytes(const dgx_colsum_problem* problems, int n);
int dgx_colsum_grouped(const dgx_colsum_problem* problems, int n, float beta, void* workspace, void* stream);

int64_t dgx_groupnorm_scratch_floats(int N, int HW, int G);
int dgx_groupnorm_fwd(const void* x, const float* gamma, const float* beta, void* y, float* mean, float* rstd,
                      float* scratch, int N, int HW, int C, int G, float eps, int relu, void* stream);
int dgx_groupnorm_bwd(const void* x, const void* dy, const float* mean, const float* rstd, const float* gamma,
                      const float* beta, void* dx, float* dgamma, float* dbeta, float* part, int N, int HW,
                      int C, int G, int relu, void* stream);
typedef struct dgx_gn_item {
    const void* x;
    const void* dy;
    void* out;
    float* mean;
    float* rstd;
    float* scratch;
    int N, HW;
} dgx_gn_item;
int dgx_groupnorm_fwd_multi(const dgx_gn_item* items, int n, const float* gamma, const float* beta, int C, int G, float eps, int relu,
                            void* stream);
int dgx_groupnorm_bwd_multi(const dgx_gn_item* items, int n, const float* gamma, const float* beta, float* dgamma, float* dbeta, int C,
                            int G, int relu, void* stream);

int dgx_detic_losses(const void* logits, const void* deltas, const int64_t* gt_classes, const float* class_w,
                     const float* prop, const float* gtb, const int64_t* src, int R, int C, float wx, float wy,
                     float ww, float wh, void* dlogits, float* dsign, float* out16, float* part, int dtype,
                     void* stream);
int dgx_detic_losses_strided(const void* logits, int64_t ld_logits, const void* deltas, int64_t ld_deltas,
                             const int64_t* gt_classes, const float* class_w, const float* prop, const float* gtb,
                             const int64_t* src, int R, int C, float wx, float wy, float ww, float wh, void* dlogits,
                             int64_t ld_dlogits, int grad_cols, float* dsign, float* out16, float* part, int dtype,
                             void* stream);
int dgx_detic_grad_scale(void* dy, int64_t ld, int rows, int C, const float* out16, const float* g_cls, const float* g_box,
                         int dtype, void* stream);

int dgx_fed_class_mask(const int64_t* gt_classes, int R, const float* prob, const float* expo, int C, int K, uint8_t* mask,
                       void* stream);

int dgx_cascade_refine(const float* prop, const void* deltas, const uint8_t* valid_in, int B, const int* row0,
                       const int* gt0, const float* img_h, const float* img_w, const float* gt_boxes,
                       const int64_t* gt_classes, const int64_t* gt_src, float iou_thr, int num_classes, float wx,
                       float wy, float ww, float wh, float scale_clamp, float* boxes, uint8_t* valid_out,
                       int64_t* out_cls, float* out_gtb, int64_t* out_src, int32_t* num_fg, int dtype, void* stream);

int dgx_gelu_fwd(const void* x, void* y, int64_t n, void* stream);
int64_t dgx_gelu_bwd_workspace_bytes(int M, int N);
int dgx_gelu_bwd_colsum(const void* dy, const void* x, void* dx, float* bias_grad, int M, int N, float beta,
                        void* workspace, void* stream);

int dgx_centernet_losses_blocks(int M);
int dgx_centernet_losses(const float* reg_pred, const float* reg_targets, const float* hms, const float* logit,
                         const int64_t* pos_idx, const uint8_t* pos_cared, int M, int C, int P, int not_norm_reg,
                         float beta, float gamma, float sigmoid_clamp, float ignore_high_fp, float pos_mul,
                         float neg_mul, float* g_reg, float* g_neg, float* g_pos, float* out8, float* part,
                         void* stream);

int dgx_paste_masks(const float* masks, const float* boxes, uint8_t* out, int N, int S, int H, int W,
                    float threshold, void* stream);
int dgx_paste_rle(const float* masks, const float* boxes, int32_t* counts, int32_t* nruns, int N, int S, int H,
                  int W, float threshold, int cap, void* stream);
int dgx_rle_encode(const uint8_t* bits, int32_t* counts, int32_t* nruns, int N, int H, int W, int cap, void* stream);
int64_t dgx_rle_to_string(const int32_t* counts, int64_t n, char* out, int64_t cap);

int dgx_grad_bank_update(float* bank, const float* grad, int64_t n, float a, float b, void* stream);
int64_t dgx_grad_sim_workspace_bytes(int64_t n);
int dgx_grad_sim(const float* g1, const float* g2, int64_t n, double* out3, float* out4, void* workspace,
                 void* stream);


#define DGX_EPI_NONE 0
#define DGX_EPI_BIAS 1
#define DGX_EPI_BIAS_GELU 2
#define DGX_EPI_BIAS_RESIDUAL 3
#define DGX_EPI_GELU_GRAD 4
#define DGX_EPI_RELU_GRAD 5
typedef struct dgx_gemm_epilogue {
    int mode;
    void* c;
    int64_t ldc;
    const void* bias;
    void* c2;
    const void* aux;
    int64_t ldaux;
    const void* residual;
    void* out;
    const float* scale;
    int residual_dtype;
    int B, H, W, ws, shift;
    void* workspace;
    int64_t workspace_bytes;
    int relu;
} dgx_gemm_epilogue;
int dgx_gemm_bf16_nt(const void* A, const void* B, int M, int N, int K, int64_t lda, int64_t ldb,
                     const dgx_gemm_epilogue* epilogue, void* stream);
void dgx_set_reserved_cus(int n);
int dgx_get_reserved_cus(void);
int dgx_dev_set(const char* key, int value);
int dgx_gemm_last_form(int* bm, int* bn, int* splits);
int dgx_dev_gemm_log(const char* path);


int dgx_transpose_bf16_grouped(const void* src, void* dst, const void* jobs, int njobs, int64_t total_tiles, void* stream);


int64_t dgx_conv3x3_pad_rows(int N, int H, int W);
int dgx_conv3x3_pad(const void* x, void* xpad, int N, int H, int W, int C, void* stream);
typedef struct dgx_pad_item { const void* x; void* xpad; int N, H, W; } dgx_pad_item;
int dgx_conv3x3_pad_multi(const dgx_pad_item* items, int n, int C, void* stream);
int dgx_deconv2x2_shuffle(const void* y2, void* out, int N, int H, int W, int Cout, void* stream);
int dgx_deconv2x2_unshuffle_relu_grad(const void* gy, const void* yout, void* g2, int N, int H, int W, int Cout, void* stream);
typedef struct dgx_conv_item { const void* xpad; void* y; int N, H, W; } dgx_conv_item;
int dgx_conv3x3_gemm_multi(const dgx_conv_item* items, int n, const void* w, const void* bias, int Cin, int Cout, int relu, void* stream);
typedef struct dgx_conv_wgrad_item { const void* dypad; const void* xpad; int N, H, W; } dgx_conv_wgrad_item;
int64_t dgx_conv3x3_wgrad_bias_multi_workspace_bytes(const dgx_conv_wgrad_item* items, int n, int Cin, int Cout);
int dgx_conv3x3_wgrad_bias_multi(const dgx_conv_wgrad_item* items, int n, float* gw, float* gb, int Cin, int Cout, float beta,
                                 void* workspace, void* stream);
int dgx_conv3x3_pad_relu_grad(const void* g, const void* y, void* gpad, int N, int H, int W, int C, void* stream);
int dgx_conv3x3_gemm(const void* xpad, const void* w, const void* bias, void* y, int N, int H, int W, int Cin, int Cout,
                     int relu, void* workspace, int64_t workspace_bytes, void* stream);
int64_t dgx_conv3x3_wgrad_workspace_bytes(int N, int H, int W, int Cin, int Cout);
int dgx_conv3x3_wgrad(const void* dypad, const void* xpad, float* gw, int N, int H, int W, int Cin, int Cout, float beta,
                      void* workspace, void* stream);
int64_t dgx_conv3x3_wgrad_bias_workspace_bytes(int N, int H, int W, int Cin, int Cout);
int dgx_conv3x3_wgrad_bias(const void* dypad, const void* xpad, float* gw, float* gb, int N, int H, int W, int Cin, int Cout,
                           float beta, void* workspace, void* stream);


int dgx_preprocess_patches(const uint8_t* img, int h, int w, const float* mean, const float* stdv, void* rows, int Hp, int Wp,
                           int patch, void* stream);

int dgx_stem_im2col7x7(const float* x_nchw, void* rows_bf16, int N, int H, int W, void* stream);
int dgx_affine_act_fwd(const void* x, const float* scale, const float* shift, const void* residual, void* y, int64_t rows, int C,
                       int relu, void* stream);
int dgx_affine_act_bwd(const void* dy, const void* y, const float* scale, void* dx, void* dres, int64_t rows, int C, int relu,
                       void* stream);
int dgx_maxpool3x3s2_fwd(const void* x, void* y, void* idx_u8, int N, int H, int W, int C, void* stream);
int dgx_maxpool3x3s2_bwd(const void* dy, const void* idx_u8, void* dx, int N, int H, int W, int C, void* stream);

int64_t dgx_mask_bce_workspace_floats(int64_t n);
int dgx_mask_bce(const void* logits, int64_t row_stride, int64_t inner, const uint8_t* gt, int64_t n, void* grad, float* out,
                 float* workspace, int dtype, void* stream);

#define DGX_PROF_GEMM_NT 0
#define DGX_PROF_WGRAD 1
// ... 19 lines not shown
```

Before: 80.44 images/s.

## Skip GEMM, attention and wgrad work for drop-path-zeroed samples in Swin blocks

Threads the per-sample stochastic-depth scale (s1/s2) through as a row gate into the window-attention forward and backward kernels, the bf16 NT GEMM (both the regular and LW variants) and the grouped wgrad kernels. Output tiles and reduction ranges whose rows belong to a sample with zero scale are skipped, since that branch is multiplied by zero anyway. The GEMM also reorders M-panels so kept and dropped images are interleaved, to balance work across CUs. This adds ABI changes, extra per-tile gate checks, and correctness risk if gating is applied where the zero-scale assumption does not hold.

```diff
diff --git a/divergen_amd/_lib.py b/divergen_amd/_lib.py
--- a/divergen_amd/_lib.py
+++ b/divergen_amd/_lib.py
@@ -11,13 +11,15 @@
 
 
 class WgradProblem(ctypes.Structure):
-    _fields_ = [("dy", c_p), ("x", c_p), ("gw", c_p), ("M", c_i), ("Nn", c_i), ("Kk", c_i), ("gb", c_p)]
+    _fields_ = [("dy", c_p), ("x", c_p), ("gw", c_p), ("M", c_i), ("Nn", c_i), ("Kk", c_i), ("gb", c_p),
+                ("gate", c_p), ("gate_rows", c_i), ("gate_n", c_i)]
 
 
 class GemmEpilogue(ctypes.Structure):
     _fields_ = [("mode", c_i), ("c", c_p), ("ldc", c_i64), ("bias", c_p), ("c2", c_p), ("aux", c_p), ("ldaux", c_i64),
                 ("residual", c_p), ("out", c_p), ("scale", c_p), ("residual_dtype", c_i),
-                ("B", c_i), ("H", c_i), ("W", c_i), ("ws", c_i), ("shift", c_i), ("workspace", c_p), ("workspace_bytes", c_i64), ("relu", c_i)]
+                ("B", c_i), ("H", c_i), ("W", c_i), ("ws", c_i), ("shift", c_i), ("workspace", c_p), ("workspace_bytes", c_i64), ("relu", c_i),
+                ("gate", c_p), ("gate_rows", c_i), ("gate_n", c_i)]
 
 
 class ProfStats(ctypes.Structure):
@@ -59,6 +61,10 @@
     "dgx_window_attention_bwd": (c_i, [c_p] * 8 + [c_i64, c_i64, c_i, c_i, c_i, c_i, c_f, c_p]),
     "dgx_window_attention_fwd_compact": (c_i, [c_p, c_p, c_p, c_i64, c_i64, c_p, c_p, c_p, c_i, c_i, c_i, c_i, c_i, c_i, c_f, c_p]),
     "dgx_window_attention_bwd_compact": (c_i, [c_p] * 9 + [c_i64, c_i64, c_i, c_i, c_i, c_i, c_i, c_i, c_f, c_p]),
+    "dgx_window_attention_fwd_gated": (c_i, [c_p, c_p, c_i64, c_i64, c_p, c_p, c_p, c_i, c_i, c_i, c_i, c_f, c_p, c_p]),
+    "dgx_window_attention_bwd_gated": (c_i, [c_p] * 8 + [c_i64, c_i64, c_i, c_i, c_i, c_i, c_f, c_p, c_p]),
+    "dgx_window_attention_fwd_compact_gated": (c_i, [c_p, c_p, c_p, c_i64, c_i64, c_p, c_p, c_p, c_i, c_i, c_i, c_i, c_i, c_i, c_f, c_p, c_p]),
+    "dgx_window_attention_bwd_compact_gated": (c_i, [c_p] * 9 + [c_i64, c_i64, c_i, c_i, c_i, c_i, c_i, c_i, c_f, c_p, c_p]),
     "dgx_window_gather": (c_i, [c_p, c_p, c_i, c_i, c_i, c_i, c_i, c_i, c_i, c_p]),
     "dgx_window_scatter": (c_i, [c_p, c_p, c_i, c_i, c_i, c_i, c_i, c_i, c_i, c_p]),
     "dgx_roi_align_fwd": (c_i, [c_p, c_p, c_p, c_i, c_i, c_i, c_i, c_i, c_f, c_i, c_i, c_i, c_i, c_i, c_i, c_p]),
diff --git a/divergen_amd/csrc/abi.hip b/divergen_amd/csrc/abi.hip
--- a/divergen_amd/csrc/abi.hip
+++ b/divergen_amd/csrc/abi.hip
@@ -1,6 +1,6 @@
 #include "dgx_common.h"
 extern "C" const char* dgx_build_arch(void) { return "gfx950"; }
-extern "C" int dgx_abi_version(void) { return 3; }
+extern "C" int dgx_abi_version(void) { return 4; }
 
 extern "C" int dgx_host_register(void* p, size_t bytes) {
     if (!p || !bytes) return DGX_ERR_BAD_ARG;
diff --git a/divergen_amd/csrc/gemm_common.h b/divergen_amd/csrc/gemm_common.h
--- a/divergen_amd/csrc/gemm_common.h
+++ b/divergen_amd/csrc/gemm_common.h
@@ -34,6 +34,8 @@
     int relu;
     int ngrp;
     struct Grp { const uint16_t* A; uint16_t* C; int M, cn, ch, cw, wp, tile0; } grp[6];
+    const float* gate;
+    int gate_rows, gate_n;
 };
 constexpr int GEMM_MAXG = 6;
 }
@@ -85,6 +87,48 @@
 __device__ __forceinline__ void g_enter_group(GemmP& P, const dgxgemm::GemmP::Grp& q) {
     P.A = q.A; P.C = q.C; P.M = q.M;
     P.cmap_n = q.cn; P.cmap_h = q.ch; P.cmap_w = q.cw; P.conv_wp = q.wp;
+}
+__device__ __forceinline__ bool g_tile_gated(const GemmP& P, int m0, int bm) {
+    if (!P.gate) return false;
+    const int m1 = min(m0 + bm, P.M) - 1;
+    const int i0 = __builtin_amdgcn_readfirstlane(m0 / P.gate_rows), i1 = __builtin_amdgcn_readfirstlane(m1 / P.gate_rows);
+    if (i0 != i1 || i0 >= P.gate_n) return false;
+    return P.gate[i0] == 0.0f;
+}
+struct GGateOrder { uint32_t kept; int lp8, lr, n; };
+__device__ __forceinline__ GGateOrder g_gate_order(const GemmP& P, int bm) {
+    GGateOrder o = {0u, 0, 0, 0};
+    if (!P.gate) return o;
+    const int tiles_m = P.total / P.tiles_n, n = P.gate_n;
+    const int P8 = tiles_m >> 3, R = P.gate_rows / bm;
+    if (n > 8 || (tiles_m & 7) || P.gate_rows % bm || n * P.gate_rows != P.M || (P8 & (P8 - 1)) || (R & (R - 1))) return o;
+    uint32_t m = 0;
+#pragma unroll
+    for (int i = 0; i < 8; ++i)
+        if (i < n && P.gate[i] != 0.0f) m |= 1u << i;
+    if (m == 0 || m == (1u << n) - 1u) return o;
+    o.kept = (uint32_t)__builtin_amdgcn_readfirstlane((int)m);
+    o.lp8 = __builtin_amdgcn_readfirstlane(__builtin_ctz((unsigned)P8));
+    o.lr = __builtin_amdgcn_readfirstlane(__builtin_ctz((unsigned)R));
+    o.n = __builtin_amdgcn_readfirstlane(n);
+    return o;
+}
+__device__ __forceinline__ int g_gate_panel(const GGateOrder& o, int tm) {
+    if (!o.kept) return tm;
+    tm = __builtin_amdgcn_readfirstlane(tm);
+    const int x = tm >> o.lp8, q = ((tm & ((1 << o.lp8) - 1)) << 3) + x;
+    const int slot = q >> o.lr, r = q & ((1 << o.lr) - 1);
+    const int nk = __builtin_popcount(o.kept);
+    int img = 0, kk = 0, dd = nk;
+#pragma unroll
+    for (int i = 0; i < 8; ++i)
+        if (i < o.n) {
+            const int kept = (int)((o.kept >> i) & 1u);
+            if ((kept ? kk : dd) == slot) img = i;
+            kk += kept;
+            dd += 1 - kept;
+        }
+    return (img << o.lr) + r;
 }
 __device__ __forceinline__ uint32_t g_a_voff(const GemmP& P, int m, int lc) {
     int64_t arow = m;
diff --git a/divergen_amd/csrc/gemm_lw.hip b/divergen_amd/csrc/gemm_lw.hip
--- a/divergen_amd/csrc/gemm_lw.hip
+++ b/divergen_amd/csrc/gemm_lw.hip
@@ -71,6 +71,7 @@
     const int ktail = P0.K - (NTK - 1) * GBK;
     const uint32_t lds0 = (uint32_t)(uintptr_t)(DGX_LDS unsigned char*)lds_raw;
 
+    const GGateOrder gorder = g_gate_order(P0, BM);
     auto locate_item = [&](int L0, GemmP& P, LwItem& it) {
         int L = L0 / P0.splits;
         it.split = L0 - L * P0.splits;
@@ -81,10 +82,10 @@
             L -= q.tile0;
         }
         const int tm = L / P0.tiles_n, tn = L - tm * P0.tiles_n;
-        it.m0 = tm * BM;
+        it.m0 = g_gate_panel(gorder, tm) * BM;
         it.n0 = tn * BN;
         it.kt0 = it.split * P0.kt_per_split;
-        it.NT = min(P0.kt_per_split, NTK - it.kt0);
+        it.NT = g_tile_gated(P, __builtin_amdgcn_readfirstlane(it.m0), BM) ? 0 : min(P0.kt_per_split, NTK - it.kt0);
     };
     auto a_slot = [](int s) -> uint32_t { return s == NSA - 1 ? (uint32_t)STG0 : (uint32_t)s * SA; };
 
diff --git a/divergen_amd/csrc/gemm_nt.hip b/divergen_amd/csrc/gemm_nt.hip
--- a/divergen_amd/csrc/gemm_nt.hip
+++ b/divergen_amd/csrc/gemm_nt.hip
@@ -41,7 +41,7 @@
     DGX_CLK(0);
     DGX_CLK_RT(5);
     const int tm = L / P.tiles_n, tn = L - tm * P.tiles_n;
-    const int m0 = tm * BM, n0 = tn * BN;
+    const int m0 = g_gate_panel(g_gate_order(P, BM), tm) * BM, n0 = tn * BN;
     const int tid = threadIdx.x, l = tid & 63;
     const int w = __builtin_amdgcn_readfirstlane(tid >> 6);
     const int grp = w >> 2, wc = w & 3;
@@ -49,7 +49,7 @@
     const int NTK = (P.K + GBK - 1) / GBK;
     const int ktail = P.K - (NTK - 1) * GBK;
     const int kt0 = split * P.kt_per_split;
-    const int NT = min(P.kt_per_split, NTK - kt0);
+    const int NT = g_tile_gated(P, __builtin_amdgcn_readfirstlane(m0), BM) ? 0 : min(P.kt_per_split, NTK - kt0);
 
     const int rsub = l >> 3;
     const int lc = (l & 7) ^ (((w & 1) << 2) | (rsub >> 1));
@@ -403,6 +403,7 @@
     return DGX_OK;
 }
 extern int g_dgx_dev_wgrad_lw;
+int g_dgx_dev_row_gate = 1;
 extern "C" int dgx_dev_set(const char* key, int value) {
     if (!key) return DGX_ERR_BAD_ARG;
     if (!strcmp(key, "gemm_lw")) g_dev.lw = value;
@@ -411,7 +412,8 @@
     else if (!strcmp(key, "gemm_splitk")) g_dev.splitk = value;
     else if (!strcmp(key, "gemm_k192")) g_dev.k192 = value;
     else if (!strcmp(key, "wgrad_lw")) g_dgx_dev_wgrad_lw = value;
-    else if (!strcmp(key, "reset")) { g_dev = dgxplan::DevKnobs(); g_dgx_dev_wgrad_lw = 1; }
+    else if (!strcmp(key, "row_gate")) g_dgx_dev_row_gate = value;
+    else if (!strcmp(key, "reset")) { g_dev = dgxplan::DevKnobs(); g_dgx_dev_wgrad_lw = 1; g_dgx_dev_row_gate = 1; }
     else return DGX_ERR_BAD_ARG;
     return DGX_OK;
 }
@@ -439,6 +441,10 @@
     P.res = ep->residual; P.out = ep->out; P.scale = ep->scale; P.res_dtype = ep->residual_dtype;
     P.ws = (float*)ep->workspace;
     P.relu = (ep->mode <= DGX_EPI_BIAS) ? ep->relu : 0;
+    if (ep->gate) {
+        if (ep->gate_rows <= 0 || ep->gate_n <= 0) return DGX_ERR_BAD_ARG;
+        if (g_dgx_dev_row_gate) { P.gate = ep->gate; P.gate_rows = ep->gate_rows; P.gate_n = ep->gate_n; }
+    }
     switch (ep->mode) {
         case DGX_EPI_NONE: case DGX_EPI_BIAS:
             if (!ep->c || ep->ldc < N || (ep->ldc & 7)) return DGX_ERR_BAD_ARG;
diff --git a/divergen_amd/csrc/wgrad256.hip b/divergen_amd/csrc/wgrad256.hip
--- a/divergen_amd/csrc/wgrad256.hip
+++ b/divergen_amd/csrc/wgrad256.hip
@@ -19,6 +19,8 @@
     int M, Nn, Kk, tiles_k, tiles, S, slab, wg0;
     int ldc;
     int64_t red0;
+    const float* gate;
+    int gate_rows, gate_n;
 };
 struct Params256 {
     Prob256 p[MAXP256];
@@ -74,7 +76,26 @@
         s_in = su - im.slab0;
     }
     const int n0 = (tile / q.tiles_k) * T256, k0 = (tile % q.tiles_k) * T256;
-    const int m_begin = s_in * q.slab, m_end = min(q.M, m_begin + q.slab);
+    int m_begin = s_in * q.slab, m_end = min(q.M, m_begin + q.slab);
+    if (q.gate) {
+        const int rows = q.gate_rows, lim = q.gate_n * rows;
+        for (int guard = 0; guard < 64 && m_begin < m_end && m_begin < lim; ++guard) {
+            const int i = __builtin_amdgcn_readfirstlane(m_begin / rows);
+            if (q.gate[i] != 0.0f) break;
+            const int skip = ((i + 1) * rows - m_begin) / BM256;
+            if (skip <= 0) break;
+            m_begin = min(m_end, m_begin + skip * BM256);
+        }
+        for (int guard = 0; guard < 64 && m_begin < m_end && m_end <= lim; ++guard) {
+            const int i = __builtin_amdgcn_readfirstlane((m_end - 1) / rows);
+            if (q.gate[i] != 0.0f) break;
+            const int first = max(i * rows, m_begin), a = m_begin + (first - m_begin + BM256 - 1) / BM256 * BM256;
+            if (a >= m_end) break;
+            m_end = a;
+        }
+        m_begin = __builtin_amdgcn_readfirstlane(m_begin);
+        m_end = __builtin_amdgcn_readfirstlane(m_end);
+    }
     const int nst = (m_end - m_begin + BM256 - 1) / BM256;
     const int tid = threadIdx.x, w = tid >> 6, l = tid & 63, g = l >> 4, c16 = l & 15;
     const int wn = (w >> 1) * 128, wk = (w & 1) * 128;
@@ -347,6 +368,7 @@
 }
 
 static int wgrad_grouped_impl(const dgx_wgrad_problem* problems, const int* ldc, int n, float beta, void* workspace, void* stream);
+extern int g_dgx_dev_row_gate;
 
 extern "C" int dgx_linear_wgrad_grouped(const dgx_wgrad_problem* problems, int n, float beta, void* workspace,
                                         void* stream) {
@@ -366,7 +388,7 @@
 }
 
 extern "C" int64_t dgx_conv3x3_wgrad_workspace_bytes(int N, int H, int W, int Cin, int Cout) {
-    dgx_wgrad_problem pr[9];
+    dgx_wgrad_problem pr[9] = {};
     const int64_t Mp = (int64_t)N * (H + 2) * (W + 2);
     for (int t = 0; t < 9; ++t) { pr[t].dy = pr[t].x = nullptr; pr[t].gw = nullptr; pr[t].gb = nullptr; pr[t].M = (int)Mp; pr[t].Nn = Cout; pr[t].Kk = Cin; }
     return split_workspace_bytes(pr, 9);
@@ -378,7 +400,7 @@
     return dgx_conv3x3_wgrad_bias(dypad, xpad, gw, nullptr, N, H, W, Cin, Cout, beta, workspace, stream);
 }
 extern "C" int64_t dgx_conv3x3_wgrad_bias_workspace_bytes(int N, int H, int W, int Cin, int Cout) {
-    dgx_wgrad_problem pr[9];
+    dgx_wgrad_problem pr[9] = {};
     const int64_t Mp = (int64_t)N * (H + 2) * (W + 2);
     float dummy;
     for (int t = 0; t < 9; ++t) { pr[t].dy = pr[t].x = nullptr; pr[t].gw = nullptr; pr[t].gb = t == 0 ? &dummy : nullptr; pr[t].M = (int)Mp; pr[t].Nn = Cout; pr[t].Kk = Cin; }
@@ -390,7 +412,7 @@
     if (!dypad || !xpad || !gw || (Cin & 7) || (Cout & 7)) return DGX_ERR_BAD_ARG;
     const int64_t Mp = (int64_t)N * (H + 2) * (W + 2);
     const int wp = W + 2;
-    dgx_wgrad_problem pr[9];
+    dgx_wgrad_problem pr[9] = {};
     int ldc[9];
     for (int t = 0; t < 9; ++t) {
         pr[t].dy = (const uint16_t*)dypad + (int64_t)(wp + 1) * Cout;
@@ -432,6 +454,11 @@
         q.wsb = (float*)workspace + offb[i];
         q.ws = (float*)workspace + off[i];
         q.M = p.M; q.Nn = p.Nn; q.Kk = p.Kk;
+        q.gate = nullptr; q.gate_rows = 0; q.gate_n = 0;
+        if (p.gate && !ldc) {
+            if (p.gate_rows <= 0 || p.gate_n <= 0 || (int64_t)p.gate_rows * p.gate_n > p.M) return DGX_ERR_BAD_ARG;
+            if (g_dgx_dev_row_gate) { q.gate = p.gate; q.gate_rows = p.gate_rows; q.gate_n = p.gate_n; }
+        }
         q.ldc = ldc ? ldc[i] : p.Kk;
         q.tiles_k = (p.Kk + T256 - 1) / T256;
         q.S = S[i];
@@ -550,6 +577,7 @@
         q.wsb = ws + 9 * per;
         q.ws = ws + (int64_t)t * per;
         q.M = M[0]; q.Nn = Cout; q.Kk = Cin;
+        q.gate = nullptr; q.gate_rows = 0; q.gate_n = 0;
         q.ldc = 9 * Cin;
         q.tiles_k = tiles_k;
         q.S = S;
diff --git a/divergen_amd/csrc/wgrad_lw.hip b/divergen_amd/csrc/wgrad_lw.hip
--- a/divergen_amd/csrc/wgrad_lw.hip
+++ b/divergen_amd/csrc/wgrad_lw.hip
@@ -20,7 +20,11 @@
     float* C;
     float* gb;
     int M, Nn, Kk, ldc, tiles_k, item0;
+    const float* gate;
+    int gate_rows, gate_n;
 };
+struct WlSpan { int lo, hi, hole_at, hole_rows, NH; };
+constexpr int WL_GATE_SCAN = 64;
 struct WlParams {
     WlProb p[WL_MAXP];
     int item0[WL_MAXP];
@@ -73,8 +77,37 @@
         q.M = tab[idx].M; q.Nn = tab[idx].Nn; q.Kk = tab[idx].Kk; q.ldc = tab[idx].ldc; q.tiles_k = tab[idx].tiles_k; q.item0 = tab[idx].item0;
         const int t = L - q.item0;
         const int tn = t / q.tiles_k;
+        q.gate = tab[idx].gate; q.gate_rows = tab[idx].gate_rows; q.gate_n = tab[idx].gate_n;
         n0 = tn * WL_TN;
         k0 = ((t - tn * q.tiles_k + tn + (tn >> 3)) % q.tiles_k) * WL_TK;
+    };
+    auto span_of = [&](const WlProb& q, WlSpan& sp) {
+        sp.lo = 0; sp.hi = q.M; sp.hole_at = -1; sp.hole_rows = 0;
+        if (q.gate) {
+            const int rows = q.gate_rows, n = min(q.gate_n, WL_GATE_SCAN);
+            const bool all = n == q.gate_n && n * rows == q.M;
+            int i = 0, j = n;
+            while (i < n && q.gate[i] == 0.0f) ++i;
+            if (all) {
+                while (j > i && q.gate[j - 1] == 0.0f) --j;
+                sp.hi = min(q.M, (j * rows + WL_BM - 1) / WL_BM * WL_BM);
+            }
+            sp.lo = (i * rows) / WL_BM * WL_BM;
+            if (all && i >= j) sp.lo = sp.hi = 0;
+            int k = i + 1;
+            while (k < j && q.gate[k] != 0.0f) ++k;
+            if (k < j) {
+                int e = k;
+                while (e < j && q.gate[e] == 0.0f) ++e;
+                const int hs = (k * rows + WL_BM - 1) / WL_BM * WL_BM, he = (e * rows) / WL_BM * WL_BM;
+                if (he > hs) { sp.hole_at = 2 * ((hs - sp.lo) / WL_BM); sp.hole_rows = he - hs; }
+            }
+        }
+        const int len = sp.hi - sp.lo - sp.hole_rows;
+        sp.NH = len > 0 ? 2 * ((len + WL_BM - 1) / WL_BM) : 0;
+        sp.lo = __builtin_amdgcn_readfirstlane(sp.lo); sp.hi = __builtin_amdgcn_readfirstlane(sp.hi);
+        sp.hole_at = __builtin_amdgcn_readfirstlane(sp.hole_at); sp.hole_rows = __builtin_amdgcn_readfirstlane(sp.hole_rows);
+        sp.NH = __builtin_amdgcn_readfirstlane(sp.NH);
     };
     if (w >= 8) {
         const int lw = w - 8;
@@ -84,27 +117,45 @@
         const uint32_t OOB = 0x80000000u;
         WlProb q;
         int n0, k0, NH = 0;
+        int ga = 0, gb_ = 0, hole_at = -1;
+        uint32_t jumpA = 0, jumpB = 0;
         uint32_t va[4], vb[4];
         uint32_t stepA = 0, stepB = 0, sa = 0, sb = 0;
         u32x4 rA, rB;
         auto setup = [&](int L) {
             locate(L, q, n0, k0);
-            NH = 2 * ((q.M + WL_BM - 1) / WL_BM);
+            WlSpan sp;
+            span_of(q, sp);
+            NH = sp.NH;
+            ga = 0; gb_ = 0; hole_at = sp.hole_at;
+            jumpA = (uint32_t)(sp.hole_rows * q.Nn * 2); jumpB = (uint32_t)(sp.hole_rows * q.Kk * 2);
 #pragma unroll
             for (int s = 0; s < 4; ++s) {
-                const int lc = (s & 1) ? lc1 : lc0, row = 8 * s + 2 * lw + rip;
+                const int lc = (s & 1) ? lc1 : lc0, row = sp.lo + 8 * s + 2 * lw + rip;
                 va[s] = (n0 + 8 * lc < q.Nn) ? (uint32_t)((row * q.Nn + n0 + 8 * lc) * 2) : OOB;
                 vb[s] = (8 * lc < WL_TK && k0 + 8 * lc < q.Kk) ? (uint32_t)((row * q.Kk + k0 + 8 * lc) * 2) : OOB;
             }
             stepA = (uint32_t)(WL_GR * q.Nn * 2); stepB = (uint32_t)(WL_GR * q.Kk * 2);
             sa = 0; sb = 0;
-            rA = wl_rsrc(q.A, (uint32_t)((int64_t)q.M * q.Nn * 2));
-            rB = wl_rsrc(q.B, (uint32_t)((int64_t)q.M * q.Kk * 2));
+            rA = wl_rsrc(q.A, (uint32_t)((int64_t)sp.hi * q.Nn * 2));
+            rB = wl_rsrc(q.B, (uint32_t)((int64_t)sp.hi * q.Kk * 2));
         };
         auto issue_a1 = [&](int s) { wl_load_lds16(va[s], rA, wl_sgpr(ldsq + sa + 4096u * s), 0u); va[s] += stepA; };
         auto issue_b1 = [&](int s) { wl_load_lds16(vb[s], rB, wl_sgpr(ldsq + WL_B0 + sb + 4096u * s), 0u); vb[s] += stepB; };
-        auto next_a = [&]() { sa = sa + WL_GB == WL_NGA * WL_GB ? 0u : sa + WL_GB; };
-        auto next_b = [&]() { sb = (sb + WL_GB) & (WL_NGB * WL_GB - 1); };
+        auto next_a = [&]() {
+            sa = sa + WL_GB == WL_NGA * WL_GB ? 0u : sa + WL_GB;
+            if (++ga == hole_at) {
+#pragma unroll
+                for (int s = 0; s < 4; ++s) va[s] += jumpA;
+            }
+        };
+        auto next_b = [&]() {
+            sb = (sb + WL_GB) & (WL_NGB * WL_GB - 1);
+            if (++gb_ == hole_at) {
+#pragma unroll
+                for (int s = 0; s < 4; ++s) vb[s] += jumpB;
+            }
+        };
         auto issue_a = [&]() {
 #pragma unroll
             for (int s = 0; s < 4; ++s) issue_a1(s);
@@ -191,7 +242,9 @@
         WlProb q;
         int n0, k0;
         locate(L, q, n0, k0);
-        const int NH = 2 * ((q.M + WL_BM - 1) / WL_BM);
+        WlSpan sp;
+        span_of(q, sp);
+        const int NH = sp.NH;
         f32x4 acc[8][3];
 #pragma unroll
         for (int i = 0; i < 8; ++i)
@@ -265,6 +318,7 @@
     }
 }
 
+extern int g_dgx_dev_row_gate;
 int wgrad_lw_launch(const dgx_wgrad_problem* pr, int n, float beta, hipStream_t st) {
     if (n <= 0 || n > WL_MAXP) return DGX_ERR_UNSUPPORTED;
     WlParams P;
@@ -277,6 +331,10 @@
         WlProb& q = P.p[i];
         q.A = (const uint16_t*)p.dy; q.B = (const uint16_t*)p.x; q.C = p.gw; q.gb = p.gb;
         q.M = p.M; q.Nn = p.Nn; q.Kk = p.Kk; q.ldc = p.Kk;
+        if (p.gate) {
+            if (p.gate_rows <= 0 || p.gate_n <= 0 || (int64_t)p.gate_rows * p.gate_n > p.M) return DGX_ERR_BAD_ARG;
+            if (g_dgx_dev_row_gate) { q.gate = p.gate; q.gate_rows = p.gate_rows; q.gate_n = p.gate_n; }
+        }
         q.tiles_k = (p.Kk + WL_TK - 1) / WL_TK;
         q.item0 = items;
         items += ((p.Nn + WL_TN - 1) / WL_TN) * q.tiles_k;
diff --git a/divergen_amd/csrc/window_attention.hip b/divergen_amd/csrc/window_attention.hip
--- a/divergen_amd/csrc/window_attention.hip
+++ b/divergen_amd/csrc/window_attention.hip
@@ -62,7 +62,12 @@
     int T, P;
     const uint16_t* bias;
     const uint16_t* zeros;
+    const float* gate;
+    int gate_wpi;
 };
+__device__ __forceinline__ bool attn_gated(const AttnGeom& G, int b) {
+    return G.gate && G.gate[__builtin_amdgcn_readfirstlane(b / G.gate_wpi)] == 0.0f;
+}
 template <int WS>
 __device__ __forceinline__ int attn_row(const AttnGeom& G, const WmGeom& g, const WmWindow& w, int img, int wr, int wc, int n) {
     const int i = n / WS, j = n - i * WS;
@@ -121,6 +126,18 @@
         return (row >= 0 ? qkv + (int64_t)row * rowst : G.bias) + h * 32;
     };
 
+    if (attn_gated(G, b)) {
+        if (qok) {
+            const int64_t zrow = COMPACT ? (int64_t)row_of(qi) : (int64_t)b * N + qi;
+            if (zrow >= 0) {
+                uint16_t* orow = out + zrow * C + h * 32 + 4 * g;
+                *reinterpret_cast<u32x2*>(orow) = u32x2{0u, 0u};
+                *reinterpret_cast<u32x2*>(orow + 16) = u32x2{0u, 0u};
+            }
+            if (g == 0) lse[((int64_t)b * nH + h) * N + qi] = 0.f;
+        }
+        return;
+    }
     const int8_t* reg = region + (int64_t)(b % nW) * N;
     const float tv = tid < TBL ? table[h * t_sh + tid * t_si] : 0.f;
     const int kr_in = (MASKED && tid < N) ? (int)reg[tid] : -1;
@@ -346,7 +363,18 @@
         P.lse = INFINITY;
         P.reg = 0;
     }
-    if (count > 0) issue(b, h, P);
+    uint32_t dropped = 0;
+    if (G.gate) {
+        const int nimg = min(B_ / G.gate_wpi, 32);
+        for (int i = 0; i < nimg; ++i) dropped |= (G.gate[i] == 0.0f ? 1u : 0u) << i;
+        dropped = (uint32_t)__builtin_amdgcn_readfirstlane((int)dropped);
+    }
+    auto unit_gated = [&](int bb) -> bool {
+        if (!dropped) return false;
+        const int img = __builtin_amdgcn_readfirstlane(bb / G.gate_wpi);
+        return img < 32 && ((dropped >> img) & 1u);
+    };
+    if (count > 0 && !unit_gated(b)) issue(b, h, P);
     auto load_head = [&](int hh) {
         constexpr int NTHR = (NT + (HELP ? 3 : 0)) * 64, KT = (TBL + NTHR - 1) / NTHR;
         float tv[KT];
@@ -490,7 +518,24 @@
         const bool wrap = u + 1 == seg;
         const int bn = b + 1 == hi ? lo : b + 1, hn = b + 1 == hi ? h + 1 : h;
         __syncthreads();
-        if (more) issue(bn, hn, P);
+        if (more && !unit_gated(bn)) issue(bn, hn, P);
+        if (unit_gated(b)) {
+            uint16_t* zqb = dqkv + (COMPACT ? (int64_t)0 : (int64_t)b * N * rowst) + h * 32;
+            uint32_t zrow4 = row4_c;
+            if (COMPACT) {
+                const int row = compact_row(b, kok ? key : 0);
+                zrow4 = (uint32_t)(row >= 0 ? row : G.T - 1 - row) * (uint32_t)rowst + 4 * g;
+            }
+            if (!helper && kok) {
+#pragma unroll
+                for (int part = 0; part < 3; ++part)
+#pragma unroll
+                    for (int dt = 0; dt < 2; ++dt) *reinterpret_cast<u32x2*>(zqb + part * C + zrow4 + 16 * dt) = u32x2{0u, 0u};
+            }
+            if (more && !wrap) stage();
+            if (!wrap) { b = bn; h = hn; }
+            continue;
+        }
         const bf16x8 kf = *reinterpret_cast<const bf16x8*>(&Ks[(kok ? key : 0) * RR + 8 * g]);
         const bf16x8 vf = *reinterpret_cast<const bf16x8*>(&Vs[(kok ? key : 0) * RR + 8 * g]);
         const int rk = MASKED ? reg_s[kok ? key : 0] : 0;
@@ -690,17 +735,27 @@
     return DGX_OK;
 }
 
+extern int g_dgx_dev_row_gate;
+static int attn_set_gate(AttnGeom& G, const float* gate, int B_, int nW) {
+    if (!gate) return DGX_OK;
+    if (nW <= 0 || B_ % nW) return DGX_ERR_BAD_ARG;
+    if (g_dgx_dev_row_gate) { G.gate = gate; G.gate_wpi = nW; }
+    return DGX_OK;
+}
+
 static int attn_fwd_launch(const void* qkv, const float* table, int64_t table_stride_head, int64_t table_stride_index, const int8_t* region,
-                           void* out, float* lse, int B_, int nW, int nH, int ws, float scale, const AttnGeom* geom, void* stream) {
+                           void* out, float* lse, int B_, int nW, int nH, int ws, float scale, const AttnGeom* geom, void* stream,
+                           const float* gate = nullptr) {
     if (B_ <= 0) return DGX_OK;
     if (!qkv || !table || !out || !lse || nH <= 0 || nW <= 0 || (region && B_ % nW)) return DGX_ERR_BAD_ARG;
+    AttnGeom G = geom ? *geom : AttnGeom{0, 0, 0, 0, 0, nullptr, nullptr};
+    if (int rc = attn_set_gate(G, gate, B_, nW)) return rc;
     hipStream_t st = (hipStream_t)stream;
     const bool masked = region != nullptr;
     if (!region) { region = zero_region(); if (!geom) nW = 1; if (!region) return DGX_ERR_BAD_ARG; }
     const int grid = ((B_ + 7) / 8) * 8 * nH;
     const double heads = (double)B_ * nH, ntok = (double)ws * ws;
     DgxProfScope prof(DGX_PROF_ATTN_FWD, stream, heads * 2.0 * 2.0 * ntok * ntok * 32.0, heads * ntok * (32.0 * 2.0 * 4.0 + 4.0));
-    AttnGeom G = geom ? *geom : AttnGeom{0, 0, 0, 0, 0, nullptr, nullptr};
 #define FWD_LAUNCH(WSV, MK, CP) hipLaunchKernelGGL((win_attn_fwd_kernel<WSV, MK, CP>), dim3(grid), dim3(WinCfg<WSV>::NT * 64), 0, st, \
                                                   (const uint16_t*)qkv, table, region, (uint16_t*)out, lse, B_, nW, nH, scale, \
                                                   table_stride_head, table_stride_index, G)
@@ -736,14 +791,15 @@
 static int attn_bwd_launch(const void* qkv, const float* table, const int8_t* region, const void* out,
                            const float* lse, const void* dout, void* dqkv, float* dtable,
                            int64_t dtable_stride_head, int64_t dtable_stride_index, int B_, int nW, int nH,
-                           int ws, float scale, const AttnGeom* geom, void* stream) {
+                           int ws, float scale, const AttnGeom* geom, void* stream, const float* gate = nullptr) {
     if (B_ <= 0) return DGX_OK;
     if (!qkv || !table || !out || !lse || !dout || !dqkv || !dtable || nH <= 0 || nW <= 0 || (region && B_ % nW))
         return DGX_ERR_BAD_ARG;
+    AttnGeom G = geom ? *geom : AttnGeom{0, 0, 0, 0, 0, nullptr, nullptr};
+    if (int rc = attn_set_gate(G, gate, B_, nW)) return rc;
     hipStream_t st = (hipStream_t)stream;
     const bool masked = region != nullptr;
     if (!region) { region = zero_region(); if (!geom) nW = 1; if (!region) return DGX_ERR_BAD_ARG; }
-    AttnGeom G = geom ? *geom : AttnGeom{0, 0, 0, 0, 0, nullptr, nullptr};
     if (geom) { G.zeros = (const uint16_t*)zero_region(); if (!G.zeros) return DGX_ERR_BAD_ARG; }
     extern int dgx_get_reserved_cus(void);
     const int cus = 256 - dgx_get_reserved_cus();
@@ -817,3 +873,40 @@
     return attn_bwd_launch(qkv, table, region, out, lse, dout, dqkv, dtable, dtable_stride_head, dtable_stride_index, B_, nW, nH, ws, scale,
                            &G, stream);
 }
+
+extern "C" int dgx_window_attention_fwd_gated(const void* qkv, const float* table, int64_t table_stride_head, int64_t table_stride_index,
+                                              const int8_t* region, void* out, float* lse, int B_, int nW, int nH, int ws, float scale,
+                                              void* stream, const float* gate) {
+    return attn_fwd_launch(qkv, table, table_stride_head, table_stride_index, region, out, lse, B_, nW, nH, ws, scale, nullptr, stream, gate);
+}
+extern "C" int dgx_window_attention_bwd_gated(const void* qkv, const float* table, const int8_t* region, const void* out, const float* lse,
+                                              const void* dout, void* dqkv, float* dtable, int64_t dtable_stride_head,
+                                              int64_t dtable_stride_index, int B_, int nW, int nH, int ws, float scale, void* stream,
+                                              const float* gate) {
+    return attn_bwd_launch(qkv, table, region, out, lse, dout, dqkv, dtable, dtable_stride_head, dtable_stride_index, B_, nW, nH, ws, scale,
+                           nullptr, stream, gate);
+}
+extern "C" int dgx_window_attention_fwd_compact_gated(const void* qkv, const void* qkv_bias, const float* table, int64_t table_stride_head,
+                                                      int64_t table_stride_index, const int8_t* region, void* out, float* lse, int B, int H,
+                                                      int W, int nH, int ws, int shift, float scale, void* stream, const float* gate) {
+    if (ws != 12 && ws != 7) return DGX_ERR_UNSUPPORTED;
+    AttnGeom G = {0, 0, 0, 0, 0, nullptr, nullptr};
+    int nW = 0;
+    const int nWh = (H + ws - 1) / ws, nWw = (W + ws - 1) / ws;
+    const int B_ = B * nWh * nWw;
+    if (int rc = attn_geom(G, B_, nW, ws, B, H, W, shift, qkv_bias, nH)) return rc;
+    return attn_fwd_launch(qkv, table, table_stride_head, table_stride_index, region, out, lse, B_, nW, nH, ws, scale, &G, stream, gate);
+}
+extern "C" int dgx_window_attention_bwd_compact_gated(const void* qkv, const void* qkv_bias, const float* table, const int8_t* region,
+                                                      const void* out, const float* lse, const void* dout, void* dqkv, float* dtable,
+                                                      int64_t dtable_stride_head, int64_t dtable_stride_index, int B, int H, int W, int nH,
+                                                      int ws, int shift, float scale, void* stream, const float* gate) {
+    if (ws != 12 && ws != 7) return DGX_ERR_UNSUPPORTED;
+    AttnGeom G = {0, 0, 0, 0, 0, nullptr, nullptr};
+    int nW = 0;
+    const int nWh = (H + ws - 1) / ws, nWw = (W + ws - 1) / ws;
+    const int B_ = B * nWh * nWw;
+    if (int rc = attn_geom(G, B_, nW, ws, B, H, W, shift, qkv_bias, nH)) return rc;
+    return attn_bwd_launch(qkv, table, region, out, lse, dout, dqkv, dtable, dtable_stride_head, dtable_stride_index, B_, nW, nH, ws, scale,
+                           &G, stream, gate);
+}
diff --git a/divergen_amd/layers/gemm_ops.py b/divergen_amd/layers/gemm_ops.py
--- a/divergen_amd/layers/gemm_ops.py
+++ b/divergen_amd/layers/gemm_ops.py
@@ -47,7 +47,12 @@
     return t.data_ptr()
 
 
-def gemm_nt(a, b, bias=None, out=None):
+def _set_gate(ep, gate):
+    if gate is not None and gate[0] is not None:
+        ep.gate, ep.gate_rows, ep.gate_n = _dev_ptr(gate[0]), int(gate[1]), gate[0].numel()
+
+
+def gemm_nt(a, b, bias=None, out=None, gate=None):
     _check2(a, b)
     _dev_ptr(a), _dev_ptr(b)
     M, N = a.shape[0], b.shape[0]
@@ -55,6 +60,7 @@
     ep = L.GemmEpilogue()
     ep.mode = EPI_BIAS if bias is not None else EPI_NONE
     ep.c, ep.ldc, ep.bias = c.data_ptr(), c.stride(0), _dev_ptr(bias)
+    _set_gate(ep, gate)
     _launch(a, b, ep)
     return c
 
@@ -70,7 +76,7 @@
     return c
 
 
-def gemm_bias_gelu(a, b, bias):
+def gemm_bias_gelu(a, b, bias, gate=None):
     _check2(a, b)
     M, N = a.shape[0], b.shape[0]
     f1 = torch.empty(M, N, dtype=BF16, device=a.device)
@@ -78,11 +84,12 @@
     ep = L.GemmEpilogue()
     ep.mode = EPI_BIAS_GELU
     ep.c, ep.ldc, ep.bias, ep.c2 = f1.data_ptr(), N, _dev_ptr(bias), act.data_ptr()
+    _set_gate(ep, gate)
     _launch(a, b, ep)
     return f1, act
 
 
-def gemm_gelu_grad(a, b, f1):
+def gemm_gelu_grad(a, b, f1, gate=None):
     _check2(a, b)
     M, N = a.shape[0], b.shape[0]
     assert f1.shape == (M, N) and f1.dtype == BF16 and f1.is_contiguous()
@@ -90,6 +97,7 @@
     ep = L.GemmEpilogue()
     ep.mode = EPI_GELU_GRAD
     ep.c, ep.ldc, ep.aux, ep.ldaux = c.data_ptr(), N, f1.data_ptr(), N
+    _set_gate(ep, gate)
     _launch(a, b, ep)
     return c
 
@@ -106,7 +114,7 @@
     return c
 
 
-def gemm_bias_residual(a, b, bias, res, scale, B, H, W, ws, shift):
+def gemm_bias_residual(a, b, bias, res, scale, B, H, W, ws, shift, gated=False):
     _check2(a, b)
     N = b.shape[0]
     res = res.contiguous()
@@ -117,6 +125,9 @@
     ep.bias, ep.residual, ep.out, ep.scale = _dev_ptr(bias), res.data_ptr(), out.data_ptr(), _dev_ptr(scale)
     ep.residual_dtype = L.dtype_code(res)
     ep.B, ep.H, ep.W, ep.ws, ep.shift = B, H, W, ws, shift
+    if gated and scale is not None:
+        assert a.shape[0] % B == 0
+        _set_gate(ep, (scale, a.shape[0] // B))
     _launch(a, b, ep)
     return out
 
diff --git a/divergen_amd/layers/linear_ops.py b/divergen_amd/layers/linear_ops.py
--- a/divergen_amd/layers/linear_ops.py
+++ b/divergen_amd/layers/linear_ops.py
@@ -32,6 +32,10 @@
         arr[i].dy, arr[i].x, arr[i].gw = dy2.data_ptr(), x2.data_ptr(), g2.data_ptr()
         arr[i].gb = gb.data_ptr() if gb is not None else None
         arr[i].M, arr[i].Nn, arr[i].Kk = dy2.shape[0], dy2.shape[1], x2.shape[1]
+        gate = pr[4] if len(pr) > 4 else None
+        if gate is not None and gate[0] is not None:
+            assert gate[0].dtype == torch.float32 and gate[0].is_contiguous() and gate[0].numel() * int(gate[1]) <= dy2.shape[0]
+            arr[i].gate, arr[i].gate_rows, arr[i].gate_n = gate[0].data_ptr(), int(gate[1]), gate[0].numel()
     return arr
 
 
diff --git a/divergen_amd/layers/swin_block.py b/divergen_amd/layers/swin_block.py
--- a/divergen_amd/layers/swin_block.py
+++ b/divergen_amd/layers/swin_block.py
@@ -51,11 +51,11 @@
 
 
 def _launch(items):
-    members = [q for (g, d, x_, b, w), _ in items for q in ((w,) if b is None else (w, b))]
+    members = [q for (g, d, x_, b, w, gt), _ in items for q in ((w,) if b is None else (w, b))]
     slot = getattr(members[0], "_dgx_arena_slot", None)
     first = slot is not None and all(getattr(q, "_dgx_arena_slot", (None,))[0] is slot[0] for q in members) and slot[0].claim_first_write(members)
-    wgrad_grouped([(g, d, x_, b.grad if b is not None else None) for (g, d, x_, b, w), _ in items], beta=0.0 if first else 1.0)
-    for (g, d, x_, b, w), _ in items:
+    wgrad_grouped([(g, d, x_, b.grad if b is not None else None, gt) for (g, d, x_, b, w, gt), _ in items], beta=0.0 if first else 1.0)
+    for (g, d, x_, b, w, gt), _ in items:
         _ready(w) if b is None else _ready(w, b)
 
 
@@ -126,7 +126,7 @@
         return
     items = [[p, _tiles(p[0])] for p in _PENDING_LW]
     del _PENDING_LW[:]
-    if wgrad_group_form([(g, d, x_, b.grad if b is not None else None) for (g, d, x_, b, w), _ in items]):
+    if wgrad_group_form([(g, d, x_, b.grad if b is not None else None) for (g, d, x_, b, w, gt), _ in items]):
         _launch(items)
     else:
         _flush_all()
@@ -172,10 +172,10 @@
         _launch(items)
 
 
-def _linear_bwd(dy2, x2, weight, bias, wgrads, gelu_of=None):
-    wgrads.append((weight.grad.view(weight.shape[0], -1), dy2, x2, bias, weight))
+def _linear_bwd(dy2, x2, weight, bias, wgrads, gelu_of=None, gate=None):
+    wgrads.append((weight.grad.view(weight.shape[0], -1), dy2, x2, bias, weight, gate))
     wt = shadow_t(weight)
-    return G.gemm_gelu_grad(dy2, wt, gelu_of) if gelu_of is not None else G.gemm_nt(dy2, wt)
+    return G.gemm_gelu_grad(dy2, wt, gelu_of, gate=gate) if gelu_of is not None else G.gemm_nt(dy2, wt, gate=gate)
 
 
 _HANDOVER = [None]
@@ -219,25 +219,27 @@
         rstd1 = torch.empty(T, dtype=f32, device=dev)
         L.check(lib.dgx_layernorm_fwd(x.data_ptr(), n1w.data_ptr(), n1b.data_ptr(), xw.data_ptr(), mean1.data_ptr(),
                                       rstd1.data_ptr(), T, C, eps1, B, H, W, wsm, shift, code, st), "dgx_layernorm_fwd")
-        qkv = G.gemm_nt(xw[:Tr], shadow(qw), shadow(qb))
+        gate1, gate2 = (s1, Tr // B), (s2, H * W)
+        qkv = G.gemm_nt(xw[:Tr], shadow(qw), shadow(qb), gate=gate1)
         tbl = table.detach()
         o = torch.empty(Tr, C, dtype=BF16, device=dev)
         lse = torch.empty(B_, nH, N, dtype=f32, device=dev)
         if compact:
-            L.check(lib.dgx_window_attention_fwd_compact(qkv.data_ptr(), shadow(qb).data_ptr(), tbl.data_ptr(), tbl.stride(1), tbl.stride(0),
-                                                         L.ptr(region), o.data_ptr(), lse.data_ptr(), B, H, W, nH, ws, shift, scale, st),
-                    "dgx_window_attention_fwd_compact")
+            L.check(lib.dgx_window_attention_fwd_compact_gated(qkv.data_ptr(), shadow(qb).data_ptr(), tbl.data_ptr(), tbl.stride(1), tbl.stride(0),
+                                                               L.ptr(region), o.data_ptr(), lse.data_ptr(), B, H, W, nH, ws, shift, scale, st,
+                                                               L.ptr(s1)), "dgx_window_attention_fwd_compact_gated")
         else:
-            L.check(lib.dgx_window_attention_fwd(qkv.data_ptr(), tbl.data_ptr(), tbl.stride(1), tbl.stride(0), L.ptr(region),
-                                                 o.data_ptr(), lse.data_ptr(), B_, nW, nH, ws, scale, st), "dgx_window_attention_fwd")
-        x1 = G.gemm_bias_residual(o, shadow(pw), shadow(pb), x.view(B, H * W, C), s1, B, H, W, wsm, shift).view(x.shape)
+            L.check(lib.dgx_window_attention_fwd_gated(qkv.data_ptr(), tbl.data_ptr(), tbl.stride(1), tbl.stride(0), L.ptr(region),
+                                                       o.data_ptr(), lse.data_ptr(), B_, nW, nH, ws, scale, st, L.ptr(s1)),
+                    "dgx_window_attention_fwd_gated")
+        x1 = G.gemm_bias_residual(o, shadow(pw), shadow(pb), x.view(B, H * W, C), s1, B, H, W, wsm, shift, gated=True).view(x.shape)
         h2 = torch.empty(T, C, dtype=BF16, device=dev)
         mean2 = torch.empty(T, dtype=f32, device=dev)
         rstd2 = torch.empty(T, dtype=f32, device=dev)
         L.check(lib.dgx_layernorm_fwd(x1.data_ptr(), n2w.data_ptr(), n2b.data_ptr(), h2.data_ptr(), mean2.data_ptr(),
                                       rstd2.data_ptr(), T, C, eps2, 0, 0, 0, 0, 0, code, st), "dgx_layernorm_fwd")
-        f1, a = G.gemm_bias_gelu(h2, shadow(w1), shadow(b1))
-        out = G.gemm_bias_residual(a, shadow(w2), shadow(b2), x1.view(B, H * W, C), s2, B, H, W, 0, 0).view(x.shape)
+        f1, a = G.gemm_bias_gelu(h2, shadow(w1), shadow(b1), gate=gate2)
+        out = G.gemm_bias_residual(a, shadow(w2), shadow(b2), x1.view(B, H * W, C), s2, B, H, W, 0, 0, gated=True).view(x.shape)
         ctx.save_for_backward(x, mean1, rstd1, xw, qkv, region, o, lse, x1, mean2, rstd2, h2, f1, a, s1, s2)
         ctx.params = (n1w, n1b, qw, qb, table, pw, pb, n2w, n2b, w1, b1, w2, b2)
         ctx.cfg = cfg
@@ -264,8 +266,9 @@
                 df2 = torch.empty(T, C, dtype=BF16, device=dev)
                 L.check(lib.dgx_residual_bwd(g.data_ptr(), L.ptr(s2), df2.data_ptr(), B, H, W, C, 0, 0, code, st), "dgx_residual_bwd")
         wgrads = []
-        df1 = _linear_bwd(df2, a, w2, b2, wgrads, gelu_of=f1)
-        dh2 = _linear_bwd(df1, h2, w1, b1, wgrads)
+        gate2 = (s2, H * W)
+        df1 = _linear_bwd(df2, a, w2, b2, wgrads, gelu_of=f1, gate=gate2)
+        dh2 = _linear_bwd(df1, h2, w1, b1, wgrads, gate=gate2)
         nblk = lib.dgx_layernorm_bwd_blocks(T)
         part = torch.empty(2, nblk * 2 * C, dtype=torch.float32, device=dev)
         compact = compact_ok(H, W, ws, shift)
@@ -277,22 +280,24 @@
                                            g.data_ptr(), dx1.data_ptr(), None, None, part[0].data_ptr(),
                                            T, C, 0, 0, 0, 0, 0, code, dpr.data_ptr(), L.ptr(s1), B, H, W, wsm, shift, st),
                 "dgx_layernorm_bwd_emit")
-        do = _linear_bwd(dpr, o, pw, pb, wgrads)
+        gate1 = (s1, Tr // B)
+        do = _linear_bwd(dpr, o, pw, pb, wgrads, gate=gate1)
         dqkv = torch.empty(Tw, qkv.shape[1], dtype=BF16, device=dev)
         assert table.grad.stride() == table.stride()
         if compact:
-            L.check(lib.dgx_window_attention_bwd_compact(qkv.data_ptr(), shadow(qb).data_ptr(), table.data_ptr(), L.ptr(region), o.data_ptr(),
-                                                         lse.data_ptr(), do.data_ptr(), dqkv.data_ptr(), table.grad.data_ptr(), table.stride(1),
-                                                         table.stride(0), B, H, W, nH, ws, shift, scale, st), "dgx_window_attention_bwd_compact")
+            L.check(lib.dgx_window_attention_bwd_compact_gated(qkv.data_ptr(), shadow(qb).data_ptr(), table.data_ptr(), L.ptr(region), o.data_ptr(),
+                                                               lse.data_ptr(), do.data_ptr(), dqkv.data_ptr(), table.grad.data_ptr(), table.stride(1),
+                                                               table.stride(0), B, H, W, nH, ws, shift, scale, st, L.ptr(s1)),
+                    "dgx_window_attention_bwd_compact_gated")
             _ready(table)
-            wgrads.append((qw.grad.view(qw.shape[0], -1), dqkv, xw, qb, qw))
-            dxw = G.gemm_nt(dqkv[:T], shadow_t(qw))
+            wgrads.append((qw.grad.view(qw.shape[0], -1), dqkv, xw, qb, qw, gate1))
+            dxw = G.gemm_nt(dqkv[:T], shadow_t(qw), gate=gate1)
         else:
-            L.check(lib.dgx_window_attention_bwd(qkv.data_ptr(), table.data_ptr(), L.ptr(region), o.data_ptr(), lse.data_ptr(),
-                                                 do.data_ptr(), dqkv.data_ptr(), table.grad.data_ptr(), table.stride(1), table.stride(0),
-                                                 B_, nW, nH, ws, scale, st), "dgx_window_attention_bwd")
+            L.check(lib.dgx_window_attention_bwd_gated(qkv.data_ptr(), table.data_ptr(), L.ptr(region), o.data_ptr(), lse.data_ptr(),
+                                                       do.data_ptr(), dqkv.data_ptr(), table.grad.data_ptr(), table.stride(1), table.stride(0),
+                                                       B_, nW, nH, ws, scale, st, L.ptr(s1)), "dgx_window_attention_bwd_gated")
             _ready(table)
-            dxw = _linear_bwd(dqkv, xw, qw, qb, wgrads)
+            dxw = _linear_bwd(dqkv, xw, qw, qb, wgrads, gate=gate1)
         prev = ctx.prev_scale
         if prev and (prev[0] is not None or dx1.dtype != BF16):
             scaled = torch.empty(T, C, dtype=BF16, device=dev)
diff --git a/include/divergen_hip.h b/include/divergen_hip.h
--- a/include/divergen_hip.h
+++ b/include/divergen_hip.h
@@ -38,6 +38,21 @@
                                      const void* out, const float* lse, const void* dout, void* dqkv, float* dtable,
                                      int64_t dtable_stride_head, int64_t dtable_stride_index, int B, int H, int W, int nH,
                                      int ws, int shift, float scale, void* stream);
+
+int dgx_window_attention_fwd_gated(const void* qkv, const float* table, int64_t table_stride_head, int64_t table_stride_index,
+                                   const int8_t* region, void* out, float* lse, int B_, int nW, int nH, int ws, float scale,
+                                   void* stream, const float* gate);
+int dgx_window_attention_bwd_gated(const void* qkv, const float* table, const int8_t* region, const void* out, const float* lse,
+                                   const void* dout, void* dqkv, float* dtable, int64_t dtable_stride_head,
+                                   int64_t dtable_stride_index, int B_, int nW, int nH, int ws, float scale, void* stream,
+                                   const float* gate);
+int dgx_window_attention_fwd_compact_gated(const void* qkv, const void* qkv_bias, const float* table, int64_t table_stride_head,
+                                           int64_t table_stride_index, const int8_t* region, void* out, float* lse, int B, int H,
+                                           int W, int nH, int ws, int shift, float scale, void* stream, const float* gate);
+int dgx_window_attention_bwd_compact_gated(const void* qkv, const void* qkv_bias, const float* table, const int8_t* region,
+                                           const void* out, const float* lse, const void* dout, void* dqkv, float* dtable,
+                                           int64_t dtable_stride_head, int64_t dtable_stride_index, int B, int H, int W, int nH,
+                                           int ws, int shift, float scale, void* stream, const float* gate);
 
 int dgx_window_gather(const void* x, void* xw, int B, int H, int W, int C, int ws, int shift,
                       int dtype, void* stream);
@@ -228,6 +243,8 @@
     float* gw;
     int M, Nn, Kk;
     float* gb;
+    const float* gate;
+    int gate_rows, gate_n;
 } dgx_wgrad_problem;
 int64_t dgx_wgrad_grouped_workspace_bytes(const dgx_wgrad_problem* problems, int n);
 int dgx_linear_wgrad_grouped(const dgx_wgrad_problem* problems, int n, float beta, void* workspace,
@@ -332,6 +349,8 @@
     void* workspace;
     int64_t workspace_bytes;
     int relu;
+    const float* gate;
+    int gate_rows, gate_n;
 } dgx_gemm_epilogue;
 int dgx_gemm_bf16_nt(const void* A, const void* B, int M, int N, int K, int64_t lda, int64_t ldb,
                      const dgx_gemm_epilogue* epilogue, void* stream);
```

Measured after the change: 80.86 images/s (median of 6 runs). Within noise of the previous version (+0.5%).
